# Paleogenomics/pss-bam

Measured on AMD Instinct MI355X. Metric: aligned reads/s (whole node) + HBM GB/s fraction, 200M x 150bp BAM, higher is better.
Workload: dtype u64

## Files before the change

### pss-bam_amd/csrc/engine.hip

```cpp
#include "../../include/pssbam_hip.h"
#include "../../include/fasta-genome-io.h"

#include <hip/hip_runtime.h>

#include <algorithm>
#include <condition_variable>
#include <cstdarg>
#include <cstdio>
#include <cstdlib>
#include <cstring>
#include <ctime>
#include <map>
#include <string>
#include <thread>
#include <unordered_map>
#include <atomic>
#include <memory>
#include <mutex>
#include <vector>

#include "tally_kernels.h"

using namespace pssbam;

static thread_local char g_err[512] = "";
static double feed_now() {
    timespec ts;
    clock_gettime(CLOCK_MONOTONIC, &ts);
    return ts.tv_sec + ts.tv_nsec * 1e-9;
}

static int fail(int code, const char *fmt, ...) {
    va_list ap;
    va_start(ap, fmt);
    vsnprintf(g_err, sizeof g_err, fmt, ap);
    va_end(ap);
    return code;
}

#define HIP_TRY(expr)                                                                          \
    do {                                                                                       \
        hipError_t _e = (expr);                                                                \
        if (_e != hipSuccess)                                                                  \
            return fail(PSSBAM_EHIP, "%s failed: %s (%s:%d)", #expr, hipGetErrorString(_e), __FILE__, __LINE__); \
    } while (0)

extern "C" const char *pssbam_last_error(void) { return g_err; }

static bool device_is_gfx950(int dev) {
    hipDeviceProp_t pr;
    if (hipGetDeviceProperties(&pr, dev) != hipSuccess) return false;
    return strncmp(pr.gcnArchName, "gfx950", 6) == 0;
}

extern "C" int pssbam_device_count(void) {
    int n = 0;
    if (hipGetDeviceCount(&n) != hipSuccess) return 0;
    int ok = 0;
    for (int d = 0; d < n; d++) ok += device_is_gfx950(d) ? 1 : 0;
    return ok;
}

extern "C" int pssbam_warmup(int device) {
    HIP_TRY(hipSetDevice(device));
    HIP_TRY(hipFree(nullptr));
    return PSSBAM_OK;
}

struct Slot {
    uint8_t *d_recs = nullptr;
    size_t recs_cap = 0;
    uint32_t *d_offs = nullptr;
    size_t offs_cap = 0;
    hipEvent_t copy_begin = nullptr, copied = nullptr, consumed = nullptr;
    bool busy = false;
    bool timed = false;
    uint64_t ticket = 0;
};

static constexpr uint64_t FEED_OUT_TARGET = 4400ull << 20, FEED_COMP_CAP = 2ull << 30, FEED_OUT_SLACK = 160ull << 20,
                          FEED_OVERSHOOT = 64ull << 20,
                          FEED_GAP = 16ull << 20;
static constexpr int FEED_SLOTS_READY = 3, FEED_SLOTS_MAX = 40;

struct FeedAcc {
    uint8_t *d_comp = nullptr;
    size_t comp_cap = 0;
    uint64_t comp_used = 0;
    std::vector<pssbam_bgzf_block> blocks;
    std::vector<uint32_t> sub_first;
    uint64_t out_used = 0, sub_bytes = 0;
    void *d_blocks = nullptr;
    pssbam_bgzf_block *h_blocks = nullptr;
    size_t h_blocks_cap = 0;
    uint64_t *d_a = nullptr, *d_e = nullptr, *d_last = nullptr, *d_nexta = nullptr;
    uint32_t *d_n = nullptr, *d_counts = nullptr, *d_base = nullptr;
    size_t blocks_cap = 0;
    uint8_t *d_out = nullptr;
    size_t out_cap = 0;
    uint32_t *d_offs = nullptr;
    size_t offs_cap = 0;
    uint32_t *d_nrecs = nullptr;
    size_t nrecs_cap = 0;
    uint64_t *d_chain = nullptr;
    hipEvent_t consumed = nullptr, copies_done = nullptr, copies_done2 = nullptr, inflated = nullptr, inflate_done = nullptr;
    bool busy = false;
    bool held = false;
    uint64_t flush_seq = 0;
};

struct DeferredTally {
    int slot;
    uint64_t sub_base, sub_len, offs_at;
    uint32_t n_bound, k;
    uint64_t sample_off;
    bool last_of_slot;
};

namespace {
struct PinEntry { size_t len; int refs; };
std::map<const void *, PinEntry> g_pins;
std::mutex g_pins_mu;
bool pin_acquire(const void *p, size_t len) {
    std::lock_guard<std::mutex> lk(g_pins_mu);
    auto it = g_pins.find(p);
    if (it != g_pins.end()) { it->second.refs++; return true; }
    if (hipHostRegister((void *)p, len, hipHostRegisterPortable) != hipSuccess) { (void)hipGetLastError(); return false; }
    g_pins[p] = PinEntry{len, 1};
    return true;
}
void pin_release(const void *p) {
    std::lock_guard<std::mutex> lk(g_pins_mu);
    auto it = g_pins.find(p);
    if (it == g_pins.end()) return;
    if (--it->second.refs == 0) { (void)hipHostUnregister((void *)p); g_pins.erase(it); }
}
}

enum PrepSlot : int {
    PREP_TILED_PSS, PREP_TILED_PSS_LATER, PREP_TILED_PSS_KMER, PREP_TILED_PSS_KMER_LDS, PREP_TILED_KMER, PREP_TILED_KMER_LDS,
    PREP_COMPACT, PREP_COMPACT_KMER, PREP_COMPACT_KMER_LDS,
    PREP_COMPACT_ONCE, PREP_COMPACT_ONCE_KMER, PREP_COMPACT_ONCE_KMER_LDS, PREP_COMPACT_DECODE_TWICE,
    PREP_PLANES_RG, PREP_PLANES_RG_LATER, PREP_PLANES_LEN, PREP_PLANES_LEN_LATER, PREP_PLANES_REF, PREP_PLANES_REF_LATER,
    PREP_KPLANES_RG, PREP_KPLANES_RG_LDS, PREP_KPLANES_LEN, PREP_KPLANES_LEN_LDS, PREP_KPLANES_REF, PREP_KPLANES_REF_LDS,
    PREP_TILED_PSS_BQ, PREP_TILED_PSS_LATER_BQ, PREP_TILED_PSS_KMER_BQ, PREP_TILED_PSS_KMER_LDS_BQ,
    PREP_PLANES_RG_BQ, PREP_PLANES_RG_LATER_BQ, PREP_PLANES_LEN_BQ, PREP_PLANES_LEN_LATER_BQ, PREP_PLANES_REF_BQ, PREP_PLANES_REF_LATER_BQ,
    PREP_TILED_PSS_H, PREP_TILED_PSS_KMER_H, PREP_TILED_PSS_KMER_LDS_H, PREP_TILED_PSS_H_BQ, PREP_TILED_PSS_KMER_H_BQ, PREP_TILED_PSS_KMER_LDS_H_BQ,
    PREP_TILED_SITE, PREP_TILED_SITE_LATER, PREP_TILED_SITE_BQ, PREP_TILED_SITE_LATER_BQ,
    PREP_N
};

struct pssbam_engine {
    pssbam_config cfg{};
    std::string up_ctx, down_ctx, rg;
    bool has_rg = false;
    int device = 0;
    int n_cu = 0;
    hipStream_t stream = nullptr, copy_stream = nullptr, copy_stream2 = nullptr;
    hipStream_t inflate_stream[2] = {nullptr, nullptr};
    hipEvent_t feed_base_ev = nullptr;
    hipStream_t genome_stream = nullptr;
    std::thread late_thread;
    std::atomic<int> late_ready{0};
    std::mutex late_mu;
    hipStream_t late_copy1 = nullptr, late_copy2 = nullptr, late_genome = nullptr;
    bool late_adopted = false;
    hipEvent_t genome_ready = nullptr;
    bool genome_wait_pending = false;
    std::vector<const void *> genome_pins;
    std::vector<void *> retired;
    hipEvent_t copied2 = nullptr;
    bool own_stream = false;

    uint8_t *d_genome = nullptr;
    uint32_t *d_genome4 = nullptr;
    uint32_t acgt_ctx = 0;
    uint64_t genome_bytes = 0;
    std::vector<uint64_t> contig_start;
    std::vector<uint32_t> contig_len;
    std::vector<std::string> contig_ids;
    int32_t star_contig = -1;
    uint4 *d_ref_info = nullptr;
    uint4 *h_ref_info = nullptr;
    size_t h_ref_cap = 0;
    int32_t n_ref = 0;
    bool have_refs = false;
    uint8_t *d_rg = nullptr;
    PlaneSel planes = PLANES_NONE;
    uint32_t n_planes = 0, off_groups = 0, plane_words = 0;
    uint64_t kplane_words = 0;
    uint8_t *d_grp_ids = nullptr;
    uint32_t *d_grp_offs = nullptr, *d_grp_hash = nullptr;
    uint32_t grp_hash_mask = 0;
    std::vector<uint32_t> len_edges;
    std::unordered_map<std::string, uint32_t> ctg_plane;
    std::vector<std::string> ref_names;
    bool tallied = false;
    uint32_t min_bq = 0;
    uint32_t hist_max = 0, off_hist = 0;
    uint32_t site_mode = 0, off_site = 0;
    int env_hist_lds_bins = -1;
    std::unordered_map<std::string, std::vector<uint2>> regions;
    bool has_regions = false;
    uint32_t region_shift = 10;
    std::vector<uint4> ref_info_host;
    uint4 *d_region_info = nullptr;
    uint32_t *d_region_grid = nullptr;
    uint2 *d_region_iv = nullptr;
    unsigned long long *d_counters = nullptr;
    unsigned long long *d_counters_own = nullptr;
    size_t n_counters = 0;
    uint32_t rows = 0, off_rev = 0, off_k5 = 0, off_k3 = 0, off_stats = 0;
    uint64_t n_bins = 0;
    Slot slots[2];
    int next_slot = 0;
    uint64_t ticket_seq = 0;
    double h2d_ms = 0.0;
    uint64_t h2d_bytes = 0;
    std::vector<FeedAcc *> feed;
    int cur_feed = -1, spare_feed = -1;
    uint64_t flush_seq = 0;
    bool feed_opened = false;
    int32_t feed_n_ref = 0;
    uint64_t feed_mem_budget = 0;
    std::vector<DeferredTally> deferred;
    uint8_t *d_carry = nullptr;
    uint8_t *h_handoff = nullptr;
    hipEvent_t handoff_ev = nullptr;
    uint64_t feed_out_target = FEED_OUT_TARGET, feed_comp_cap = FEED_COMP_CAP;
    double feed_t_alloc = 0, feed_t_wait_busy = 0, feed_t_flush = 0;
    double feed_t0 = 0, feed_t_first_flush = -1;
    uint64_t feed_slots_allocated = 0, feed_deferred_launches = 0, feed_early_flushes = 0;
    uint64_t feed_blocks_launched = 0, feed_lanes_launched = 0;
    uint64_t feed_idle_min_blocks = 8192;
    uint64_t feed_block_target = 0;
    std::vector<std::pair<uint64_t, hipEvent_t>> feed_copies;
    std::vector<hipEvent_t> feed_event_pool;
    uint32_t *d_feed_flags = nullptr;
    uint64_t *d_feed_tail = nullptr;
    bool feed_fresh = true;
    uint32_t feed_skip = 0;
    double inflate_ms = 0.0;
    uint64_t inflated_bytes = 0;
    std::vector<std::pair<hipEvent_t, hipEvent_t>> inflate_events;
    hipEvent_t t_begin = nullptr, t_end = nullptr;
    std::vector<std::pair<hipEvent_t, hipEvent_t>> launch_events;
    std::vector<hipEvent_t> event_pool;
    double kernel_ms = 0.0;
    uint64_t kernel_launches = 0;
    int env_tile_reads = 0, env_grid_mult = 0, env_simple_blocks = 0, env_grid_wgs = 0, env_pieces = 0;
    int env_group_slots = 0;
    bool warned_ablate = false;
    bool compact_plan_once = false;
    uint32_t prep_lds[2 * PREP_N] = {0};
    int prep_occ[2 * PREP_N] = {0};
    bool use_compact = true;
    uint32_t *d_scratch = nullptr;
    size_t scratch_slots = 0;
    uint32_t dev_pieces = 0;
    uint64_t dev_pieces_avg = 0;
};

static void ctx_mask(const char *set, uint32_t (&m)[8]) {
    memset(m, 0, sizeof m);
    for (const unsigned char *p = (const unsigned char *)set;; p++) {
        const uint32_t st = enc_byte(*p);
        m[st >> 5] |= 1u << (st & 31);
        if (!*p) break;
    }
}

static int env_int(const char *name) {
    const char *v = getenv(name);
    return v ? atoi(v) : 0;
}

static void late_streams(pssbam_engine *e, bool wait) {
    std::lock_guard<std::mutex> lk(e->late_mu);
    if (e->late_adopted) return;
    if (!wait && !e->late_ready.load(std::memory_order_acquire)) return;
    if (e->late_thread.joinable()) e->late_thread.join();
    e->copy_stream = e->late_copy1;
    e->copy_stream2 = e->late_copy2;
    e->genome_stream = e->late_genome;
    e->late_adopted = true;
}

extern "C" int pssbam_engine_create(const pssbam_config *cfg, pssbam_engine **out) {
    if (!cfg || !out) return fail(PSSBAM_EINVAL, "null argument");
    *out = nullptr;
    if (cfg->abi_version != PSSBAM_ABI_VERSION)
        return fail(PSSBAM_EINVAL, "abi_version %u != %u", cfg->abi_version, PSSBAM_ABI_VERSION);
    if (!(cfg->tally_mask & (PSSBAM_TALLY_PSS | PSSBAM_TALLY_KMER)) ||
        (cfg->tally_mask & ~(PSSBAM_TALLY_PSS | PSSBAM_TALLY_KMER)))
        return fail(PSSBAM_EINVAL, "tally_mask must be a non-empty subset of PSS|KMER");
    if ((cfg->tally_mask & PSSBAM_TALLY_PSS)) {
        if (cfg->pss.region_len < 0 || cfg->pss.region_len > 1000000)
            return fail(PSSBAM_EINVAL, "region_len %d out of range", cfg->pss.region_len);
        if (!cfg->pss.up_ctx || !cfg->pss.down_ctx) return fail(PSSBAM_EINVAL, "up_ctx/down_ctx must be set");
    }
    if ((cfg->tally_mask & PSSBAM_TALLY_KMER) && (cfg->kmer.klen < 1 || cfg->kmer.klen > PSSBAM_MAX_KLEN))
        return fail(PSSBAM_EINVAL, "klen %d outside the device range 1..%d", cfg->kmer.klen, PSSBAM_MAX_KLEN);

    int n_dev = 0;
    if (hipGetDeviceCount(&n_dev) != hipSuccess || n_dev == 0)
        return fail(PSSBAM_ENODEV, "no HIP device available (this engine has no CPU path)");
    int dev = cfg->device;
    if (dev < 0) HIP_TRY(hipGetDevice(&dev));
    if (dev >= n_dev) return fail(PSSBAM_ENODEV, "device %d does not exist (%d present)", dev, n_dev);
    if (!device_is_gfx950(dev) && !getenv("PSSBAM_ALLOW_OTHER_ARCH"))
        return fail(PSSBAM_ENODEV, "device %d is not gfx950", dev);
    HIP_TRY(hipSetDevice(dev));

    pssbam_engine *e = new pssbam_engine();
    std::unique_ptr<pssbam_engine, void (*)(pssbam_engine *)> guard(e, pssbam_engine_destroy);
    e->cfg = *cfg;
    e->device = dev;
    if (cfg->tally_mask & PSSBAM_TALLY_PSS) {
        e->up_ctx = cfg->pss.up_ctx;
        e->down_ctx = cfg->pss.down_ctx;
    }
    if (cfg->read_group) {
        e->rg = cfg->read_group;
        e->has_rg = true;
    }
    e->cfg.pss.up_ctx = e->cfg.pss.down_ctx = e->cfg.read_group = nullptr;
    const bool tstat = getenv("PSSBAM_STATS") != nullptr;
    const double tc0 = tstat ? feed_now() : 0.0;
    hipDeviceProp_t pr;
    HIP_TRY(hipGetDeviceProperties(&pr, dev));
    e->n_cu = pr.multiProcessorCount;
    const double tc1 = tstat ? feed_now() : 0.0;
    HIP_TRY(hipStreamCreateWithFlags(&e->stream, hipStreamNonBlocking));
    if (getenv("PSSBAM_STREAMS_UP_FRONT")) {
        HIP_TRY(hipStreamCreateWithFlags(&e->copy_stream, hipStreamNonBlocking));
        HIP_TRY(hipStreamCreateWithFlags(&e->copy_stream2, hipStreamNonBlocking));
        HIP_TRY(hipStreamCreateWithFlags(&e->genome_stream, hipStreamNonBlocking));
        e->late_adopted = true;
    } else {
        e->late_thread = std::thread([e, dev]() {
            if (hipSetDevice(dev) == hipSuccess) {
                if (hipStreamCreateWithFlags(&e->late_copy1, hipStreamNonBlocking) != hipSuccess) e->late_copy1 = nullptr;
                if (hipStreamCreateWithFlags(&e->late_copy2, hipStreamNonBlocking) != hipSuccess) e->late_copy2 = nullptr;
                if (hipStreamCreateWithFlags(&e->late_genome, hipStreamNonBlocking) != hipSuccess) e->late_genome = nullptr;
            }
            (void)hipGetLastError();
            e->late_ready.store(1, std::memory_order_release);
        });
    }
    HIP_TRY(hipEventCreateWithFlags(&e->genome_ready, hipEventDisableTiming));
    HIP_TRY(hipEventCreateWithFlags(&e->copied2, hipEventDisableTiming));
    e->own_stream = true;
    HIP_TRY(hipEventCreate(&e->t_begin));
    HIP_TRY(hipEventCreate(&e->t_end));
    const double tc2 = tstat ? feed_now() : 0.0;

    e->rows = (cfg->tally_mask & PSSBAM_TALLY_PSS) ? (uint32_t)cfg->pss.region_len + 2u : 0u;
    e->n_bins = (cfg->tally_mask & PSSBAM_TALLY_KMER) ? (1ull << (2 * cfg->kmer.klen)) : 0ull;
    e->off_rev = e->rows * 16u;
    e->off_k5 = 2u * e->rows * 16u;
    e->off_k3 = (uint32_t)(e->off_k5 + e->n_bins);
    e->off_stats = (uint32_t)(e->off_k3 + e->n_bins);
    e->n_counters = (size_t)e->off_stats + PSSBAM_ST_N;
    e->plane_words = 2u * e->rows * 16u;
    e->off_groups = (uint32_t)e->n_counters;
    e->kplane_words = cfg->tally_mask == PSSBAM_TALLY_KMER ? 2ull * e->n_bins : 0ull;
    HIP_TRY(hipMalloc(&e->d_counters_own, e->n_counters * sizeof(unsigned long long)));
    e->d_counters = e->d_counters_own;
    HIP_TRY(hipMemsetAsync(e->d_counters, 0, e->n_counters * sizeof(unsigned long long), e->stream));
    if (e->has_rg) {
        HIP_TRY(hipMalloc(&e->d_rg, e->rg.size() + 16));
        HIP_TRY(hipMemcpy(e->d_rg, e->rg.data(), e->rg.size(), hipMemcpyHostToDevice));
    }
    for (Slot &s : e->slots) {
        HIP_TRY(hipEventCreate(&s.copy_begin));
        HIP_TRY(hipEventCreate(&s.copied));
        HIP_TRY(hipEventCreateWithFlags(&s.consumed, hipEventDisableTiming));
    }
    e->scratch_slots = (size_t)e->n_cu * 8;
    HIP_TRY(hipMalloc(&e->d_scratch, e->scratch_slots * SCRATCH_WORDS * sizeof(uint32_t)));
    e->env_tile_reads = env_int("PSSBAM_TILE_READS");
    e->env_grid_mult = env_int("PSSBAM_GRID_MULT");
    e->env_simple_blocks = env_int("PSSBAM_SIMPLE_BLOCKS");
    e->env_grid_wgs = env_int("PSSBAM_GRID_WGS");
    e->env_pieces = env_int("PSSBAM_PIECES");
    e->env_group_slots = env_int("PSSBAM_GROUP_SLOTS");
    if (getenv("PSSBAM_HIST_LDS_BINS")) e->env_hist_lds_bins = std::max(env_int("PSSBAM_HIST_LDS_BINS"), 0);
    if (const int g = env_int("PSSBAM_REGION_GRID_SHIFT")) e->region_shift = (uint32_t)std::min(std::max(g, 2), 20);
    if (getenv("PSSBAM_COMPACT")) e->use_compact = env_int("PSSBAM_COMPACT") != 0;
    if (getenv("PSSBAM_COMPACT_PLAN_ONCE")) e->compact_plan_once = env_int("PSSBAM_COMPACT_PLAN_ONCE") != 0;
    if (tstat)
        fprintf(stderr, "[pssbam] engine on device %d: device properties %.3f, its stream + events %.3f, counters + scratch (first allocations, first "
                        "enqueue) %.3f s\n", dev, tc1 - tc0, tc2 - tc1, feed_now() - tc2);
    *out = guard.release();
    return PSSBAM_OK;
}

extern "C" void pssbam_engine_destroy(pssbam_engine *e) {
    if (!e) return;
    (void)hipSetDevice(e->device);
    late_streams(e, true);
    for (hipStream_t is : e->inflate_stream)
        if (is) (void)hipStreamSynchronize(is);
    if (e->stream) (void)hipStreamSynchronize(e->stream);
    if (e->copy_stream) (void)hipStreamSynchronize(e->copy_stream);
    if (e->copy_stream2) (void)hipStreamSynchronize(e->copy_stream2);
    for (Slot &s : e->slots) {
        if (s.d_recs) (void)hipFree(s.d_recs);
        if (s.d_offs) (void)hipFree(s.d_offs);
        if (s.copied) (void)hipEventDestroy(s.copied);
        if (s.copy_begin) (void)hipEventDestroy(s.copy_begin);
        if (s.consumed) (void)hipEventDestroy(s.consumed);
    }
    if (e->genome_stream) (void)hipStreamSynchronize(e->genome_stream);
    for (const void *p : e->genome_pins) pin_release(p);
    e->genome_pins.clear();
    for (FeedAcc *sp : e->feed) {
        FeedAcc &s = *sp;
        void *ptrs[] = {s.d_comp, s.d_blocks, s.d_a, s.d_e, s.d_last, s.d_nexta, s.d_n, s.d_counts, s.d_base, s.d_out, s.d_offs, s.d_nrecs, s.d_chain};
        for (void *q : ptrs)
            if (q) (void)hipFree(q);
        if (s.h_blocks) (void)hipHostFree(s.h_blocks);
        if (s.consumed) (void)hipEventDestroy(s.consumed);
        if (s.copies_done) (void)hipEventDestroy(s.copies_done);
        if (s.copies_done2) (void)hipEventDestroy(s.copies_done2);
        if (s.inflated) (void)hipEventDestroy(s.inflated);
        if (s.inflate_done) (void)hipEventDestroy(s.inflate_done);
        delete sp;
    }
    e->feed.clear();
    if (e->d_carry) (void)hipFree(e->d_carry);
    if (e->h_handoff) (void)hipHostFree(e->h_handoff);
    if (e->handoff_ev) (void)hipEventDestroy(e->handoff_ev);
    for (void *q : e->retired) (void)hipFree(q);
    if (e->d_feed_tail) (void)hipFree(e->d_feed_tail);
    for (auto &p : e->feed_copies) (void)hipEventDestroy(p.second);
    for (hipEvent_t ev : e->feed_event_pool) (void)hipEventDestroy(ev);
    if (e->d_feed_flags) (void)hipFree(e->d_feed_flags);
    for (auto &p : e->inflate_events) { (void)hipEventDestroy(p.first); (void)hipEventDestroy(p.second); }
    for (auto &p : e->launch_events) { (void)hipEventDestroy(p.first); (void)hipEventDestroy(p.second); }
    for (hipEvent_t ev : e->event_pool) (void)hipEventDestroy(ev);
    if (e->t_begin) (void)hipEventDestroy(e->t_begin);
    if (e->t_end) (void)hipEventDestroy(e->t_end);
    if (e->d_scratch) (void)hipFree(e->d_scratch);
    if (e->d_genome) (void)hipFree(e->d_genome);
    if (e->d_genome4) (void)hipFree(e->d_genome4);
    if (e->d_ref_info) (void)hipFree(e->d_ref_info);
    if (e->h_ref_info) (void)hipHostFree(e->h_ref_info);
    if (e->d_rg) (void)hipFree(e->d_rg);
    for (void *q : {(void *)e->d_region_info, (void *)e->d_region_grid, (void *)e->d_region_iv})
        if (q) (void)hipFree(q);
    if (e->d_grp_ids) (void)hipFree(e->d_grp_ids);
    if (e->d_grp_offs) (void)hipFree(e->d_grp_offs);
    if (e->d_grp_hash) (void)hipFree(e->d_grp_hash);
    if (e->d_counters_own) (void)hipFree(e->d_counters_own);
    if (e->own_stream && e->stream) (void)hipStreamDestroy(e->stream);
    if (e->copy_stream) (void)hipStreamDestroy(e->copy_stream);
    if (e->copy_stream2) (void)hipStreamDestroy(e->copy_stream2);
    for (hipStream_t is : e->inflate_stream)
        if (is) (void)hipStreamDestroy(is);
    if (e->feed_base_ev) (void)hipEventDestroy(e->feed_base_ev);
    if (e->genome_stream) (void)hipStreamDestroy(e->genome_stream);
    if (e->genome_ready) (void)hipEventDestroy(e->genome_ready);
    if (e->copied2) (void)hipEventDestroy(e->copied2);
    delete e;
}

extern "C" int pssbam_engine_set_stream(pssbam_engine *e, void *hip_stream) {
    if (!e) return fail(PSSBAM_EINVAL, "null engine");
    HIP_TRY(hipSetDevice(e->device));
    HIP_TRY(hipStreamSynchronize(e->stream));
    if (e->own_stream) HIP_TRY(hipStreamDestroy(e->stream));
    e->stream = (hipStream_t)hip_stream;
    e->own_stream = false;
    return PSSBAM_OK;
}

static constexpr uint64_t CONTIG_ALIGN = 256, CONTIG_PAD = 256;

static hipEvent_t take_event(pssbam_engine *e);
static int feed_resume(pssbam_engine *e);

static int genome_settle(pssbam_engine *e) {
    if (e->genome_pins.empty()) return PSSBAM_OK;
    HIP_TRY(hipSetDevice(e->device));
    HIP_TRY(hipEventSynchronize(e->genome_ready));
    for (const void *p : e->genome_pins) pin_release(p);
    e->genome_pins.clear();
    return PSSBAM_OK;
}

static int genome_upload(pssbam_engine *e, size_t n, const char *const *ids, const uint8_t *const *seqs, const uint64_t *lens,
                         int seqs_on_device) {
    if (!e || (n && (!ids || !seqs || !lens))) return fail(PSSBAM_EINVAL, "null argument");
    HIP_TRY(hipSetDevice(e->device));
    int rc = genome_settle(e);
    if (rc) return rc;
    std::vector<size_t> order(n);
    for (size_t i = 0; i < n; i++) order[i] = i;
    std::stable_sort(order.begin(), order.end(), [&](size_t a, size_t b) { return strcmp(ids[a], ids[b]) < 0; });
    std::vector<uint64_t> start(n + 1, 0);
    std::vector<uint32_t> len(n + 1, 0);
    uint64_t total = CONTIG_PAD;
    for (size_t k = 0; k < n; k++) {
        if (lens[order[k]] > 0xFFFFFF00ull)
            return fail(PSSBAM_EINVAL, "contig %s has %llu bases; the engine addresses contigs below 4 Gi bases", ids[order[k]],
                        (unsigned long long)lens[order[k]]);
        start[k] = total;
        len[k] = (uint32_t)lens[order[k]];
        total += ((uint64_t)len[k] + CONTIG_PAD + CONTIG_ALIGN - 1) / CONTIG_ALIGN * CONTIG_ALIGN;
    }
    if (e->d_genome) {
        HIP_TRY(hipStreamSynchronize(e->stream));
        HIP_TRY(hipFree(e->d_genome));
        e->d_genome = nullptr;
        if (e->d_genome4) { HIP_TRY(hipFree(e->d_genome4)); e->d_genome4 = nullptr; }
    }
    HIP_TRY(hipMalloc(&e->d_genome, total));
    late_streams(e, true);
    if (!e->genome_stream) HIP_TRY(hipStreamCreateWithFlags(&e->genome_stream, hipStreamNonBlocking));
    hipStream_t gs = e->genome_stream;
    if (seqs_on_device) {
        hipEvent_t ev = take_event(e);
        if (!ev) return fail(PSSBAM_EHIP, "hipEventCreate failed");
        HIP_TRY(hipEventRecord(ev, e->stream));
        HIP_TRY(hipStreamWaitEvent(gs, ev, 0));
        e->event_pool.push_back(ev);
    }
    HIP_TRY(hipMemsetAsync(e->d_genome, 0, total, gs));
    const bool try_lock = !seqs_on_device && !getenv("PSSBAM_NO_PIN");
    for (size_t k = 0; k < n; k++) {
        if (!len[k]) continue;
        const void *src = seqs[order[k]];
        if (try_lock && len[k] >= (32u << 20) && pin_acquire(src, len[k])) e->genome_pins.push_back(src);
        HIP_TRY(hipMemcpyAsync(e->d_genome + start[k], src, len[k],
                               seqs_on_device ? hipMemcpyDeviceToDevice : hipMemcpyHostToDevice, gs));
    }
    hipLaunchKernelGGL(encode_genome_kernel, dim3(4096), dim3(256), 0, gs, e->d_genome, total / 16);
    HIP_TRY(hipGetLastError());
    {
        CtxSets sets;
        ctx_mask(e->up_ctx.c_str(), sets.up);
        ctx_mask(e->down_ctx.c_str(), sets.down);
        e->acgt_ctx = 0;
        for (uint32_t v = 0; v < 4; v++)
            e->acgt_ctx |= (((sets.up[0] >> v) & 1u) << (2 * v)) | (((sets.down[0] >> v) & 1u) << (2 * v + 1));
        const uint64_t n_out = total / 8, slack = 16;
        HIP_TRY(hipMalloc(&e->d_genome4, (n_out + slack) * sizeof(uint32_t)));
        HIP_TRY(hipMemsetAsync(e->d_genome4 + n_out, 0x44, slack * sizeof(uint32_t), gs));
        hipLaunchKernelGGL(pack_genome4_kernel, dim3(4096), dim3(256), 0, gs, e->d_genome, e->d_genome4, n_out, sets);
        HIP_TRY(hipGetLastError());
    }
    HIP_TRY(hipEventRecord(e->genome_ready, gs));
    e->genome_wait_pending = true;
    e->contig_start.assign(start.begin(), start.begin() + n);
    e->contig_len.assign(len.begin(), len.begin() + n);
    e->genome_bytes = total;
    e->contig_ids.clear();
    for (size_t k = 0; k < n; k++) e->contig_ids.emplace_back(ids[order[k]]);
    e->star_contig = -1;
    if (e->have_refs) e->have_refs = false;
    {
        auto it = std::lower_bound(e->contig_ids.begin(), e->contig_ids.end(), std::string("*"),
                                   [](const std::string &a, const std::string &b) { return strcmp(a.c_str(), b.c_str()) < 0; });
        if (it != e->contig_ids.end() && *it == "*") e->star_contig = (int32_t)(it - e->contig_ids.begin());
    }
    return PSSBAM_OK;
}

extern "C" int pssbam_engine_set_genome_arrays(pssbam_engine *e, size_t n, const char *const *ids,
                                               const uint8_t *const *seqs, const uint64_t *lens,
                                               int seqs_on_device) {
    int rc = genome_upload(e, n, ids, seqs, lens, seqs_on_device);
    if (rc) return rc;
    if (e->genome_stream) HIP_TRY(hipStreamSynchronize(e->genome_stream));
    return genome_settle(e);
}

static int genome_from_struct(pssbam_engine *e, const struct genome *g, bool wait) {
    if (!e || !g) return fail(PSSBAM_EINVAL, "null argument");
    std::vector<const char *> ids(g->n_seqs);
    std::vector<const uint8_t *> seqs(g->n_seqs);
    std::vector<uint64_t> lens(g->n_seqs);
    for (size_t i = 0; i < g->n_seqs; i++) {
        ids[i] = g->seqs[i]->id;
        seqs[i] = (const uint8_t *)g->seqs[i]->seq;
        lens[i] = g->seqs[i]->len;
    }
    return wait ? pssbam_engine_set_genome_arrays(e, g->n_seqs, ids.data(), seqs.data(), lens.data(), 0)
                : genome_upload(e, g->n_seqs, ids.data(), seqs.data(), lens.data(), 0);
}

extern "C" int pssbam_engine_set_genome(pssbam_engine *e, const struct genome *g) { return genome_from_struct(e, g, true); }

extern "C" int pssbam_engine_set_genome_async(pssbam_engine *e, const struct genome *g) { return genome_from_struct(e, g, false); }

extern "C" int pssbam_engine_genome_wait(pssbam_engine *e) {
    if (!e) return fail(PSSBAM_EINVAL, "null engine");
    HIP_TRY(hipSetDevice(e->device));
    if (e->genome_stream) HIP_TRY(hipStreamSynchronize(e->genome_stream));
    return genome_settle(e);
}

static int pack_regions(pssbam_engine *e, bool in_use) {
    if (!e->has_regions) return PSSBAM_OK;
    const size_t n_ent = (size_t)e->n_ref + 1;
    const uint32_t g = e->region_shift;
    std::vector<uint4> desc(n_ent, make_uint4(0, 0, 0, 0));
    uint64_t n_iv = 0, n_grid = 0;
    std::vector<const std::vector<uint2> *> src(n_ent, nullptr);
    for (size_t i = 0; i < n_ent; i++) {
        const uint4 ri = e->ref_info_host[i];
        if (!ri.w) continue;
        const auto it = e->regions.find(i < (size_t)e->n_ref ? e->ref_names[i] : std::string("*"));
        if (it == e->regions.end()) continue;
        uint64_t cnt = 0;
        for (const uint2 &v : it->second) cnt += v.x < ri.z ? 1u : 0u;
        if (!cnt) continue;
        src[i] = &it->second;
        desc[i] = make_uint4(0, (uint32_t)cnt, 0, 0);
        n_iv += cnt;
        n_grid += ((uint64_t)ri.z >> g) + 2;
    }
    if (n_iv >= (1ull << 32) || n_grid >= (1ull << 32)) return fail(PSSBAM_ENOMEM, "the region table has too many intervals or grid words for 32-bit indices");
    const uint64_t bytes = n_ent * sizeof(uint4) + (n_iv + 1) * sizeof(uint2) + (n_grid + 2) * sizeof(uint32_t);
    HIP_TRY(hipSetDevice(e->device));
    if (in_use && e->d_region_info) HIP_TRY(hipStreamSynchronize(e->stream));
    for (void **q : {(void **)&e->d_region_info, (void **)&e->d_region_grid, (void **)&e->d_region_iv})
        if (*q) { HIP_TRY(hipFree(*q)); *q = nullptr; }
    size_t free_b = 0, total_b = 0;
    HIP_TRY(hipMemGetInfo(&free_b, &total_b));
    if (bytes > (uint64_t)free_b)
        return fail(PSSBAM_ENOMEM, "the region table (%llu intervals, grid shift %u) needs %llu bytes; the device has %llu free",
                    (unsigned long long)n_iv, g, (unsigned long long)bytes, (unsigned long long)free_b);
    std::vector<uint2> iv((size_t)n_iv + 1, make_uint2(0, 0));
    std::vector<uint32_t> grid((size_t)n_grid + 2, 0u);
    uint64_t at_iv = 0, at_grid = 0;
    for (size_t i = 0; i < n_ent; i++) {
        if (!src[i]) continue;
        const uint32_t len = e->ref_info_host[i].z, cnt = desc[i].y;
        desc[i].x = (uint32_t)at_iv;
        desc[i].z = (uint32_t)at_grid;
        uint2 *out = iv.data() + at_iv;
        for (uint32_t k = 0; k < cnt; k++) out[k] = make_uint2((*src[i])[k].x, std::min((*src[i])[k].y, len));
        const uint64_t n_bins = ((uint64_t)len >> g) + 1;
        uint32_t j = 0;
        for (uint64_t b = 0; b < n_bins; b++) {
            while (j < cnt && (uint64_t)out[j].y <= (b << g)) j++;
            grid[at_grid + b] = j;
        }
        grid[at_grid + n_bins] = cnt;
        at_iv += cnt;
        at_grid += n_bins + 1;
    }
    HIP_TRY(hipMalloc(&e->d_region_info, n_ent * sizeof(uint4)));
    HIP_TRY(hipMalloc(&e->d_region_iv, iv.size() * sizeof(uint2)));
    HIP_TRY(hipMalloc(&e->d_region_grid, grid.size() * sizeof(uint32_t)));
    HIP_TRY(hipMemcpy(e->d_region_info, desc.data(), n_ent * sizeof(uint4), hipMemcpyHostToDevice));
    HIP_TRY(hipMemcpy(e->d_region_iv, iv.data(), iv.size() * sizeof(uint2), hipMemcpyHostToDevice));
    HIP_TRY(hipMemcpy(e->d_region_grid, grid.data(), grid.size() * sizeof(uint32_t), hipMemcpyHostToDevice));
    return PSSBAM_OK;
}

extern "C" int pssbam_engine_set_regions(pssbam_engine *e, int32_t n_names, const char *const *names, int64_t n_regions,
                                         const int32_t *name_of, const uint32_t *starts, const uint32_t *ends) {
    if (!e) return fail(PSSBAM_EINVAL, "null engine");
    if (n_names < 0 || n_regions < 0 || n_regions > PSSBAM_MAX_REGIONS) return fail(PSSBAM_EINVAL, "region count outside 0..%d", PSSBAM_MAX_REGIONS);
    if ((n_names && !names) || (n_regions && (!name_of || !starts || !ends))) return fail(PSSBAM_EINVAL, "null region list");
    if (e->tallied) return fail(PSSBAM_ESTATE, "records have been tallied already: set the regions after create or reset, before the first tally");
    std::unordered_map<std::string, std::vector<uint2>> map;
    for (int32_t k = 0; k < n_names; k++) {
        if (!names[k]) return fail(PSSBAM_EINVAL, "region contig name %d is NULL", k);
        if (n_regions) map[names[k]];
    }
    for (int64_t i = 0; i < n_regions; i++) {
        if (name_of[i] < 0 || name_of[i] >= n_names) return fail(PSSBAM_EINVAL, "region %lld: contig index %d outside 0..%d", (long long)i, name_of[i], n_names - 1);
        if (starts[i] > ends[i])
            return fail(PSSBAM_EINVAL, "region %lld on %s: start %u lies behind end %u", (long long)i, names[name_of[i]], starts[i], ends[i]);
        if (starts[i] < ends[i]) map[names[name_of[i]]].push_back(make_uint2(starts[i], ends[i]));
    }
    for (auto &kv : map) {
        std::vector<uint2> &v = kv.second;
        std::sort(v.begin(), v.end(), [](const uint2 &a, const uint2 &b) { return a.x != b.x ? a.x < b.x : a.y < b.y; });
        size_t n = 0;
        for (const uint2 &r : v) {
            if (n && r.x <= v[n - 1].y) v[n - 1].y = std::max(v[n - 1].y, r.y);
            else v[n++] = r;
        }
        v.resize(n);
    }
    HIP_TRY(hipSetDevice(e->device));
    e->regions.swap(map);
    e->has_regions = n_regions > 0;
// ... 123 lines not shown
static int launch_tiled(pssbam_engine *e, PrepSlot slot, TallyParams &P, uint32_t lds, uint32_t n_tiles) {
    if (P.region_info)
        return launch_flat(e, (PrepSlot)(slot + PREP_N), tally_tiled<DO_PSS, DO_KMER, LDS_KMER, LATER, MASKQ, true, HIST>, P, lds, n_tiles, LDS_KMER);
    return launch_flat(e, slot, tally_tiled<DO_PSS, DO_KMER, LDS_KMER, LATER, MASKQ, false, HIST>, P, lds, n_tiles, LDS_KMER);
}

template <bool LATER, bool MASKQ>
static int launch_tiled_site(pssbam_engine *e, TallyParams &P, uint32_t lds, uint32_t n_tiles) {
    constexpr PrepSlot slot = MASKQ ? (LATER ? PREP_TILED_SITE_LATER_BQ : PREP_TILED_SITE_BQ) : (LATER ? PREP_TILED_SITE_LATER : PREP_TILED_SITE);
    if (P.region_info)
        return launch_flat<true>(e, (PrepSlot)(slot + PREP_N), tally_tiled<true, false, false, LATER, MASKQ, true, false, true>, P, lds, n_tiles, false);
    return launch_flat<true>(e, slot, tally_tiled<true, false, false, LATER, MASKQ, false, false, true>, P, lds, n_tiles, false);
}

template <bool MASKQ>
static int launch_tiled_hist(pssbam_engine *e, TallyParams &P, bool do_kmer, bool kmer_lds, uint32_t lds, uint32_t n_tiles) {
    constexpr int bq = MASKQ ? PREP_TILED_PSS_H_BQ - PREP_TILED_PSS_H : 0;
    if (!do_kmer) return launch_tiled<true, false, false, false, MASKQ, true>(e, (PrepSlot)(PREP_TILED_PSS_H + bq), P, lds, n_tiles);
    return kmer_lds ? launch_tiled<true, true, true, false, MASKQ, true>(e, (PrepSlot)(PREP_TILED_PSS_KMER_LDS_H + bq), P, lds, n_tiles)
                    : launch_tiled<true, true, false, false, MASKQ, true>(e, (PrepSlot)(PREP_TILED_PSS_KMER_H + bq), P, lds, n_tiles);
}

template <PlaneSel SEL, bool LATER, bool MASKQ, bool REGIONS>
static int launch_planes(pssbam_engine *e, TallyParams &P, const PlaneParams &G, uint32_t lds, uint32_t n_tiles) {
    constexpr PrepSlot plain = SEL == PLANES_RG  ? (LATER ? PREP_PLANES_RG_LATER : PREP_PLANES_RG)
                             : SEL == PLANES_LEN ? (LATER ? PREP_PLANES_LEN_LATER : PREP_PLANES_LEN)
                                                 : (LATER ? PREP_PLANES_REF_LATER : PREP_PLANES_REF);
    constexpr PrepSlot unfiltered = MASKQ ? (PrepSlot)(PREP_PLANES_RG_BQ + (plain - PREP_PLANES_RG)) : plain;
    constexpr PrepSlot slot = (PrepSlot)(unfiltered + (REGIONS ? PREP_N : 0));
    uint32_t grid = 0;
    const int rc = tiled_grid(e, slot, tally_tiled_planes<SEL, LATER, MASKQ, REGIONS>, lds, n_tiles, G.scratch_words, &grid);
    if (rc != PSSBAM_OK) return rc;
    P.scratch = e->d_scratch;
    hipLaunchKernelGGL((tally_tiled_planes<SEL, LATER, MASKQ, REGIONS>), dim3(grid), dim3(TILED_THREADS), lds, e->stream, P, G);
    hipLaunchKernelGGL(reduce_partials_grouped, dim3((G.scratch_words * REDUCE_GROUPS + 255) / 256), dim3(256), 0, e->stream, P, G, grid);
    return PSSBAM_OK;
}

template <PlaneSel SEL, bool LDS_KMER, bool REGIONS>
static int launch_kmer_planes(pssbam_engine *e, TallyParams &P, const PlaneParams &G, uint32_t lds, uint32_t n_tiles) {
    constexpr PrepSlot unfiltered = SEL == PLANES_RG  ? (LDS_KMER ? PREP_KPLANES_RG_LDS : PREP_KPLANES_RG)
                                  : SEL == PLANES_LEN ? (LDS_KMER ? PREP_KPLANES_LEN_LDS : PREP_KPLANES_LEN)
                                                      : (LDS_KMER ? PREP_KPLANES_REF_LDS : PREP_KPLANES_REF);
    constexpr PrepSlot slot = (PrepSlot)(unfiltered + (REGIONS ? PREP_N : 0));
    uint32_t grid = 0;
    const int rc = tiled_grid(e, slot, tally_tiled_kmer_planes<SEL, LDS_KMER, REGIONS>, lds, n_tiles, G.scratch_words, &grid);
    if (rc != PSSBAM_OK) return rc;
    P.scratch = e->d_scratch;
    hipLaunchKernelGGL((tally_tiled_kmer_planes<SEL, LDS_KMER, REGIONS>), dim3(grid), dim3(TILED_THREADS), lds, e->stream, P, G);
    hipLaunchKernelGGL(reduce_partials_kmer_planes, dim3((G.scratch_words * REDUCE_GROUPS + 255) / 256), dim3(256), 0, e->stream, P, G, grid,
                       (uint32_t)(LDS_KMER ? 1 : 0));
    return PSSBAM_OK;
}

static uint64_t sample_prefix_need(const uint8_t *bytes, uint64_t nbytes, bool whole_record, int max_records = 4096) {
    uint64_t o = 0, need_max = 64;
    for (int n = 0; n < max_records && o + 36 <= nbytes; n++) {
        uint32_t bs, l_seq;
        memcpy(&bs, bytes + o, 4);
        if (bs < 32 || o + 4 + (uint64_t)bs > nbytes) break;
        const uint32_t l_name = bytes[o + 12];
        uint16_t n_cig;
        memcpy(&n_cig, bytes + o + 16, 2);
        memcpy(&l_seq, bytes + o + 20, 4);
        const uint64_t qual_off = 36ull + l_name + 4ull * n_cig + ((uint64_t)l_seq + 1) / 2;
        const uint64_t need = whole_record ? 4ull + bs : std::min<uint64_t>(qual_off + 1, 4ull + bs);
        need_max = std::max(need_max, need);
        o += 4 + (uint64_t)bs;
    }
    return need_max;
}

static bool whole_records(const pssbam_engine *e) { return e->has_rg || e->planes == PLANES_RG || e->min_bq > 0; }

static PlaneParams plane_params(const pssbam_engine *e) {
    PlaneParams G{};
    G.ids = e->d_grp_ids;
    G.id_offs = e->d_grp_offs;
    G.hash = e->d_grp_hash;
    G.hash_mask = e->grp_hash_mask;
    G.n_groups = e->n_planes;
    G.n_slots = e->n_planes + 1u;
    G.plane_words = e->plane_words;
    G.off_groups = e->off_groups;
    G.koff_planes = e->off_groups;
    G.kplane_words = e->kplane_words;
    G.n_edges = (uint32_t)e->len_edges.size();
    std::copy(e->len_edges.begin(), e->len_edges.end(), G.edges);
    return G;
}

static uint32_t pieces_for(uint64_t need_max) {
    uint64_t pieces = (need_max + 15 + 15) / 16;
    pieces |= 1;
    return (uint32_t)std::min<uint64_t>(std::max<uint64_t>(pieces, 5), 41);
}

static int launch_tally(pssbam_engine *e, const uint8_t *d_recs, uint64_t nbytes, const uint32_t *d_offs,
                        uint32_t n_records, const uint8_t *host_sample, uint64_t host_sample_bytes,
                        const uint32_t *d_n_recs = nullptr, uint64_t sample_off = 0, const uint32_t *host_offsets = nullptr) {
    if (!n_records) return PSSBAM_OK;
    e->tallied = true;
    const pssbam_config &c = e->cfg;
    TallyParams P{};
    P.recs = d_recs;
    P.offs = d_offs;
    P.n_recs = n_records;
    P.n_recs_dev = d_n_recs;
    P.recs_bytes = nbytes;
    P.tally_mask = c.tally_mask;
    P.genome = e->d_genome;
    P.genome4 = e->d_genome4;
    P.acgt_ctx = e->acgt_ctx;
    P.ref_info = e->d_ref_info;
    P.n_ref = e->n_ref;
    const bool do_pss = (c.tally_mask & PSSBAM_TALLY_PSS) != 0, do_kmer = (c.tally_mask & PSSBAM_TALLY_KMER) != 0;
    if (do_pss) {
        P.N = c.pss.region_len;
        P.pss_min_mq = (uint32_t)c.pss.min_mq;
        P.pss_len_never = c.pss.min_read_len > 0xFFFFFFFFull ? 1u : 0u;
        P.pss_min_len = (uint32_t)std::min<uint64_t>(c.pss.min_read_len, 0xFFFFFFFFull);
        P.pss_max_len = (uint32_t)std::min<uint64_t>(c.pss.max_read_len, 0xFFFFFFFFull);
        P.pss_merged_only = c.pss.merged_only ? 1u : 0u;
        ctx_mask(e->up_ctx.c_str(), P.up_mask);
        ctx_mask(e->down_ctx.c_str(), P.down_mask);
    }
    if (do_kmer) {
        P.K = c.kmer.klen;
        P.fk_min_mq = (uint32_t)c.kmer.min_mq;
        P.fk_len_never = c.kmer.min_read_len > 0xFFFFFFFFull ? 1u : 0u;
        P.fk_min_len = (uint32_t)std::min<uint64_t>(c.kmer.min_read_len, 0xFFFFFFFFull);
        P.fk_max_len = (uint32_t)std::min<uint64_t>(c.kmer.max_read_len, 0xFFFFFFFFull);
        P.fk_merged_only = c.kmer.merged_only ? 1u : 0u;
    }
    P.rg = e->has_rg ? e->d_rg : nullptr;
    P.rg_len = (uint32_t)e->rg.size();
    P.counters = e->d_counters;
    P.off_rev = e->off_rev;
    P.off_k5 = e->off_k5;
    P.off_k3 = e->off_k3;
    P.off_stats = e->off_stats;
    P.min_bq = do_pss ? e->min_bq : 0u;
    const bool maskq = P.min_bq > 0;
    const bool regions = e->has_regions;
    const bool hist = do_pss && e->hist_max > 0;
    if (hist) {
        P.hist_max = e->hist_max;
        P.off_hist = e->off_hist;
    }
    const bool site = do_pss && e->site_mode != PSSBAM_SITE_NONE;
    if (site) P.off_site = e->off_site;
    if (regions) {
        P.region_info = e->d_region_info;
        P.region_grid = e->d_region_grid;
        P.region_iv = e->d_region_iv;
        P.region_shift = e->region_shift;
    }
    PlaneParams G = plane_params(e);

    int kernel = c.kernel;
    if (d_n_recs && kernel == PSSBAM_KERNEL_SIMPLE) return fail(PSSBAM_EINVAL, "device-indexed blocks need the tiled kernels");
    const uint32_t n_passes = do_pss ? (e->rows + TILED_ROWS - 1) / TILED_ROWS : 1u;
    if (kernel == PSSBAM_KERNEL_AUTO) kernel = PSSBAM_KERNEL_TILED;

    if (e->genome_wait_pending) {
        HIP_TRY(hipStreamWaitEvent(e->stream, e->genome_ready, 0));
        e->genome_wait_pending = false;
    }
    hipEvent_t ev0 = take_event(e), ev1 = take_event(e);
    if (!ev0 || !ev1) return fail(PSSBAM_EHIP, "hipEventCreate failed");
    HIP_TRY(hipEventRecord(ev0, e->stream));

    if (kernel == PSSBAM_KERNEL_SIMPLE) {
        const uint32_t tab_bytes = do_pss ? 2u * e->rows * 16u * 4u : 0u;
        const bool lds_tab = do_pss && tab_bytes <= 60u * 1024u;
        uint32_t blocks = (uint32_t)std::min<uint64_t>(((uint64_t)n_records + 255) / 256, (uint64_t)e->n_cu * 8);
        if (e->env_simple_blocks > 0) blocks = (uint32_t)e->env_simple_blocks;
        if (e->planes != PLANES_NONE && !do_pss) {
            if (e->planes == PLANES_RG) hipLaunchKernelGGL(tally_simple_kmer_planes<PLANES_RG>, dim3(blocks), dim3(256), 0, e->stream, P, G);
            else if (e->planes == PLANES_LEN) hipLaunchKernelGGL(tally_simple_kmer_planes<PLANES_LEN>, dim3(blocks), dim3(256), 0, e->stream, P, G);
            else hipLaunchKernelGGL(tally_simple_kmer_planes<PLANES_REF>, dim3(blocks), dim3(256), 0, e->stream, P, G);
        } else if (e->planes == PLANES_RG) hipLaunchKernelGGL(tally_simple_planes<PLANES_RG>, dim3(blocks), dim3(256), 0, e->stream, P, G);
        else if (e->planes == PLANES_LEN) hipLaunchKernelGGL(tally_simple_planes<PLANES_LEN>, dim3(blocks), dim3(256), 0, e->stream, P, G);
        else if (e->planes == PLANES_REF) hipLaunchKernelGGL(tally_simple_planes<PLANES_REF>, dim3(blocks), dim3(256), 0, e->stream, P, G);
        else if (lds_tab) hipLaunchKernelGGL(tally_simple<true>, dim3(blocks), dim3(256), tab_bytes, e->stream, P);
        else hipLaunchKernelGGL(tally_simple<false>, dim3(blocks), dim3(256), 0, e->stream, P);
    } else {
        const uint64_t avg = std::max<uint64_t>(40, nbytes / n_records);
        uint32_t pieces;
        if (host_sample) {
            uint64_t need = sample_prefix_need(host_sample, host_sample_bytes, whole_records(e), 1400);
            if (host_offsets && n_records > 4200u) {
                const uint32_t mid = host_offsets[n_records / 2], late = host_offsets[n_records - 1400u];
                need = std::max(need, sample_prefix_need(host_sample + mid, host_sample_bytes - mid, whole_records(e), 1400));
                need = std::max(need, sample_prefix_need(host_sample + late, host_sample_bytes - late, whole_records(e), 1400));
            }
            pieces = pieces_for(need);
        } else {
            if (!e->dev_pieces || (!d_n_recs && (avg * 8 < e->dev_pieces_avg * 7 || avg * 7 > e->dev_pieces_avg * 8))) {
                sample_off = std::min<uint64_t>(sample_off, nbytes);
                std::vector<uint8_t> head((size_t)std::min<uint64_t>(nbytes - sample_off, 1024 * 1024));
                HIP_TRY(hipMemcpyAsync(head.data(), d_recs + sample_off, head.size(), hipMemcpyDeviceToHost, e->stream));
                HIP_TRY(hipStreamSynchronize(e->stream));
                uint64_t need = sample_prefix_need(head.data(), head.size(), whole_records(e));
                if (!d_n_recs && n_records > 8192u) {
                    uint32_t at[2] = {0, 0};
                    HIP_TRY(hipMemcpyAsync(&at[0], d_offs + n_records / 2, 4, hipMemcpyDeviceToHost, e->stream));
                    HIP_TRY(hipMemcpyAsync(&at[1], d_offs + (n_records - 2048u), 4, hipMemcpyDeviceToHost, e->stream));
                    HIP_TRY(hipStreamSynchronize(e->stream));
                    for (int k = 0; k < 2; k++) {
                        if ((uint64_t)at[k] >= nbytes) continue;
                        head.resize((size_t)std::min<uint64_t>(nbytes - at[k], 512 * 1024));
                        HIP_TRY(hipMemcpyAsync(head.data(), d_recs + at[k], head.size(), hipMemcpyDeviceToHost, e->stream));
                        HIP_TRY(hipStreamSynchronize(e->stream));
                        need = std::max(need, sample_prefix_need(head.data(), head.size(), whole_records(e), 2048));
                    }
                }
                e->dev_pieces = pieces_for(need);
                e->dev_pieces_avg = avg;
            }
            pieces = e->dev_pieces;
        }
        if (e->env_pieces > 0) pieces = (uint32_t)std::min(std::max(e->env_pieces, 4), 64);
        uint32_t T = TILED_MAX_T;
        if (e->env_tile_reads > 0) T = std::min<uint32_t>(TILED_MAX_T, (uint32_t)(e->env_tile_reads + 15) / 16 * 16);
        P.reads_per_tile = T;
        P.prefix_pieces = pieces;
        P.xcd_map = (uint32_t)env_int("PSSBAM_XCD_MAP");
        P.ablate = (uint32_t)env_int("PSSBAM_ABLATE");
        if (P.ablate && !e->warned_ablate) {
            fprintf(stderr, "[pssbam] PSSBAM_ABLATE=%u: kernel phases are switched off, the tables are WRONG (profiling only)\n", P.ablate);
            e->warned_ablate = true;
        }
        const bool kmer_lds = do_kmer && c.kmer.klen <= KMER_LDS_MAX_K;
        const uint32_t n_tiles = (n_records + T - 1) / T;
        const uint32_t lds = tiled_lds_bytes(T, pieces);
        int rc = PSSBAM_OK;
        P.row_base = 0;
        if (e->planes != PLANES_NONE && !do_pss) {
            using LaunchK = int (*)(pssbam_engine *, TallyParams &, const PlaneParams &, uint32_t, uint32_t);
            static constexpr LaunchK launch_kr[2][3][2] = {
                {{launch_kmer_planes<PLANES_RG, false, false>, launch_kmer_planes<PLANES_RG, true, false>},
                 {launch_kmer_planes<PLANES_LEN, false, false>, launch_kmer_planes<PLANES_LEN, true, false>},
                 {launch_kmer_planes<PLANES_REF, false, false>, launch_kmer_planes<PLANES_REF, true, false>}},
                {{launch_kmer_planes<PLANES_RG, false, true>, launch_kmer_planes<PLANES_RG, true, true>},
                 {launch_kmer_planes<PLANES_LEN, false, true>, launch_kmer_planes<PLANES_LEN, true, true>},
                 {launch_kmer_planes<PLANES_REF, false, true>, launch_kmer_planes<PLANES_REF, true, true>}}};
            const auto &launch_k = launch_kr[regions];
            const uint32_t n_planes = G.n_groups + 1u;
            if (kmer_lds) {
                const uint32_t hist = 2u * (1u << (2 * c.kmer.klen)) * 4u;
                const uint32_t fit = lds + 2u * hist <= KMER_PLANES_LDS_BUDGET ? (KMER_PLANES_LDS_BUDGET - lds) / hist - 1u : 1u;
                uint32_t per_pass = std::min(n_planes, fit);
                if (e->env_group_slots > 0) per_pass = std::min(per_pass, (uint32_t)e->env_group_slots);
                for (uint32_t plane0 = 0; plane0 < n_planes && rc == PSSBAM_OK; plane0 += per_pass) {
                    G.plane0 = plane0;
                    G.n_slots = std::min(per_pass, n_planes - plane0);
                    G.scratch_words = GROUP_SCRATCH_DELTA + G.n_slots * (hist / 4u);
                    rc = launch_k[e->planes - PLANES_RG][1](e, P, G, tiled_kmer_planes_lds_bytes(T, pieces, G.n_slots, c.kmer.klen, true), n_tiles);
                }
            } else {
                G.plane0 = 0;
                G.n_slots = n_planes;
                G.scratch_words = GROUP_SCRATCH_DELTA;
                rc = launch_k[e->planes - PLANES_RG][0](e, P, G, lds, n_tiles);
            }
        } else if (e->planes != PLANES_NONE) {
            using LaunchPlanes = int (*)(pssbam_engine *, TallyParams &, const PlaneParams &, uint32_t, uint32_t);
            static constexpr LaunchPlanes launch_pass_r[2][2][3][2] = {
                {{{launch_planes<PLANES_RG, false, false, false>, launch_planes<PLANES_RG, true, false, false>},
                  {launch_planes<PLANES_LEN, false, false, false>, launch_planes<PLANES_LEN, true, false, false>},
                  {launch_planes<PLANES_REF, false, false, false>, launch_planes<PLANES_REF, true, false, false>}},
                 {{launch_planes<PLANES_RG, false, true, false>, launch_planes<PLANES_RG, true, true, false>},
                  {launch_planes<PLANES_LEN, false, true, false>, launch_planes<PLANES_LEN, true, true, false>},
                  {launch_planes<PLANES_REF, false, true, false>, launch_planes<PLANES_REF, true, true, false>}}},
                {{{launch_planes<PLANES_RG, false, false, true>, launch_planes<PLANES_RG, true, false, true>},
                  {launch_planes<PLANES_LEN, false, false, true>, launch_planes<PLANES_LEN, true, false, true>},
                  {launch_planes<PLANES_REF, false, false, true>, launch_planes<PLANES_REF, true, false, true>}},
                 {{launch_planes<PLANES_RG, false, true, true>, launch_planes<PLANES_RG, true, true, true>},
                  {launch_planes<PLANES_LEN, false, true, true>, launch_planes<PLANES_LEN, true, true, true>},
                  {launch_planes<PLANES_REF, false, true, true>, launch_planes<PLANES_REF, true, true, true>}}}};
            const auto &launch_pass = launch_pass_r[regions];
            const uint32_t n_planes = G.n_groups + 1u;
            const uint32_t fit = lds + 2u * GROUP_PLANE_WORDS * 4u <= GROUPED_LDS_BUDGET
                                     ? (GROUPED_LDS_BUDGET - lds) / (GROUP_PLANE_WORDS * 4u) - 1u : 1u;
            uint32_t per_pass = std::min(n_planes, fit);
            if (e->env_group_slots > 0) per_pass = std::min(per_pass, (uint32_t)e->env_group_slots);
            for (uint32_t pass = 0; pass < n_passes && rc == PSSBAM_OK; pass++) {
                P.row_base = pass * TILED_ROWS;
                for (uint32_t plane0 = 0; plane0 < n_planes && rc == PSSBAM_OK; plane0 += per_pass) {
                    G.plane0 = plane0;
                    G.n_slots = std::min(per_pass, n_planes - plane0);
                    G.scratch_words = GROUP_SCRATCH_DELTA + G.n_slots * GROUP_PLANE_WORDS;
                    rc = launch_pass[maskq][e->planes - PLANES_RG][pass > 0](e, P, G, tiled_grouped_lds_bytes(T, pieces, G.n_slots), n_tiles);
                }
            }
        } else if (site) {
            rc = maskq ? launch_tiled_site<false, true>(e, P, lds, n_tiles) : launch_tiled_site<false, false>(e, P, lds, n_tiles);
            for (uint32_t pass = 1; pass < n_passes && rc == PSSBAM_OK; pass++) {
                P.row_base = pass * TILED_ROWS;
                rc = maskq ? launch_tiled_site<true, true>(e, P, lds, n_tiles) : launch_tiled_site<true, false>(e, P, lds, n_tiles);
            }
        } else if (do_pss && e->rows <= COMPACT_MAX_ROWS && e->use_compact && !e->has_rg && !maskq && !regions && !hist) {
            if (!do_kmer && getenv("PSSBAM_COMPACT_DECODE_TWICE"))
                rc = launch_flat(e, PREP_COMPACT_DECODE_TWICE, tally_compact_decode_twice, P, lds, n_tiles, false);
            else if (e->compact_plan_once)
                rc = !do_kmer  ? launch_flat(e, PREP_COMPACT_ONCE, tally_compact<false, false, true>, P, lds, n_tiles, false)
                     : kmer_lds ? launch_flat(e, PREP_COMPACT_ONCE_KMER_LDS, tally_compact<true, true, true>, P, lds, n_tiles, true)
                                : launch_flat(e, PREP_COMPACT_ONCE_KMER, tally_compact<true, false, true>, P, lds, n_tiles, false);
            else
                rc = !do_kmer  ? launch_flat(e, PREP_COMPACT, tally_compact<false, false, false>, P, lds, n_tiles, false)
                     : kmer_lds ? launch_flat(e, PREP_COMPACT_KMER_LDS, tally_compact<true, true, false>, P, lds, n_tiles, true)
                                : launch_flat(e, PREP_COMPACT_KMER, tally_compact<true, false, false>, P, lds, n_tiles, false);
        } else if (hist) {
            P.hist_lds_bins = std::min(e->hist_max + 2u, HIST_LDS_MAX_BINS);
            if (e->env_hist_lds_bins >= 0) P.hist_lds_bins = std::min(P.hist_lds_bins, (uint32_t)e->env_hist_lds_bins);
            const uint32_t lds_h = lds + hist_lds_bytes(P.hist_lds_bins);
            rc = maskq ? launch_tiled_hist<true>(e, P, do_kmer, kmer_lds, lds_h, n_tiles) : launch_tiled_hist<false>(e, P, do_kmer, kmer_lds, lds_h, n_tiles);
            for (uint32_t pass = 1; pass < n_passes && rc == PSSBAM_OK; pass++) {
                P.row_base = pass * TILED_ROWS;
                rc = maskq ? launch_tiled<true, false, false, true, true>(e, PREP_TILED_PSS_LATER_BQ, P, lds, n_tiles)
                           : launch_tiled<true, false, false, true, false>(e, PREP_TILED_PSS_LATER, P, lds, n_tiles);
            }
        } else if (maskq) {
            if (do_kmer)
                rc = kmer_lds ? launch_tiled<true, true, true, false, true>(e, PREP_TILED_PSS_KMER_LDS_BQ, P, lds, n_tiles)
                              : launch_tiled<true, true, false, false, true>(e, PREP_TILED_PSS_KMER_BQ, P, lds, n_tiles);
            else
                rc = launch_tiled<true, false, false, false, true>(e, PREP_TILED_PSS_BQ, P, lds, n_tiles);
            for (uint32_t pass = 1; pass < n_passes && rc == PSSBAM_OK; pass++) {
                P.row_base = pass * TILED_ROWS;
                rc = launch_tiled<true, false, false, true, true>(e, PREP_TILED_PSS_LATER_BQ, P, lds, n_tiles);
            }
        } else {
            if (do_pss && do_kmer)
                rc = kmer_lds ? launch_tiled<true, true, true, false, false>(e, PREP_TILED_PSS_KMER_LDS, P, lds, n_tiles)
                              : launch_tiled<true, true, false, false, false>(e, PREP_TILED_PSS_KMER, P, lds, n_tiles);
            else if (do_pss)
                rc = launch_tiled<true, false, false, false, false>(e, PREP_TILED_PSS, P, lds, n_tiles);
            else
                rc = kmer_lds ? launch_tiled<false, true, true, false, false>(e, PREP_TILED_KMER_LDS, P, lds, n_tiles)
                              : launch_tiled<false, true, false, false, false>(e, PREP_TILED_KMER, P, lds, n_tiles);
            for (uint32_t pass = 1; pass < n_passes && rc == PSSBAM_OK; pass++) {
                P.row_base = pass * TILED_ROWS;
                rc = launch_tiled<true, false, false, true, false>(e, PREP_TILED_PSS_LATER, P, lds, n_tiles);
            }
        }
        if (rc != PSSBAM_OK) return rc;
    }
    HIP_TRY(hipGetLastError());
    HIP_TRY(hipEventRecord(ev1, e->stream));
    e->launch_events.emplace_back(ev0, ev1);
    if (e->launch_events.size() > 4096) return resolve_launch_events(e);
    return PSSBAM_OK;
}

extern "C" int pssbam_engine_hint_records(pssbam_engine *e, const void *records, uint64_t nbytes) {
    if (!e || (!records && nbytes)) return fail(PSSBAM_EINVAL, "null argument");
    if (nbytes < 36) return PSSBAM_OK;
    e->dev_pieces = pieces_for(sample_prefix_need((const uint8_t *)records, nbytes, whole_records(e), 1 << 16));
    e->dev_pieces_avg = 40;
    return PSSBAM_OK;
}

static int check_ready(pssbam_engine *e) {
    if (!e) return fail(PSSBAM_EINVAL, "null engine");
    if (!e->d_genome) return fail(PSSBAM_ESTATE, "set_genome has not been called");
    if (!e->have_refs) return fail(PSSBAM_ESTATE, "set_references has not been called");
    return PSSBAM_OK;
}

extern "C" int pssbam_engine_submit_device(pssbam_engine *e, const void *d_records, uint64_t nbytes,
                                           const uint32_t *d_offsets, uint32_t n_records) {
    int rc = check_ready(e);
    if (rc) return rc;
    if (n_records && (!d_records || !d_offsets)) return fail(PSSBAM_EINVAL, "null buffer");
    if (nbytes >= (1ull << 32)) return fail(PSSBAM_EINVAL, "record block must be < 4 GiB (got %llu)", (unsigned long long)nbytes);
    if (((uintptr_t)d_records & 15u) || ((uintptr_t)d_offsets & 3u))
        return fail(PSSBAM_EINVAL, "d_records must be 16-byte aligned, d_offsets 4-byte aligned");
    HIP_TRY(hipSetDevice(e->device));
    return launch_tally(e, (const uint8_t *)d_records, nbytes, d_offsets, n_records, nullptr, 0);
}

static void book_copy_time(pssbam_engine *e, Slot &s) {
    if (!s.timed) return;
    float ms = 0.f;
    if (hipEventElapsedTime(&ms, s.copy_begin, s.copied) == hipSuccess) e->h2d_ms += ms;
    s.timed = false;
}

extern "C" int pssbam_engine_submit_async(pssbam_engine *e, const void *records, uint64_t nbytes, const uint32_t *offsets,
                                          uint32_t n_records, uint64_t *ticket) {
    int rc = check_ready(e);
    if (rc) return rc;
    if (ticket) *ticket = 0;
    if (!n_records) return PSSBAM_OK;
    if (!records || !offsets) return fail(PSSBAM_EINVAL, "null buffer");
    if (nbytes >= (1ull << 32)) return fail(PSSBAM_EINVAL, "record block must be < 4 GiB (got %llu)", (unsigned long long)nbytes);
    if (offsets[n_records] != nbytes) return fail(PSSBAM_EFORMAT, "offsets[n_records] must equal nbytes");
    HIP_TRY(hipSetDevice(e->device));
    Slot &s = e->slots[e->next_slot];
    e->next_slot ^= 1;
    if (s.busy) HIP_TRY(hipEventSynchronize(s.consumed));
    s.busy = false;
    book_copy_time(e, s);
    if (s.recs_cap < nbytes + 64) {
        if (s.d_recs) HIP_TRY(hipFree(s.d_recs));
        s.d_recs = nullptr;
        s.recs_cap = (size_t)(nbytes + nbytes / 4 + 4096);
        HIP_TRY(hipMalloc(&s.d_recs, s.recs_cap));
    }
    if (s.offs_cap < (size_t)n_records + 1) {
        if (s.d_offs) HIP_TRY(hipFree(s.d_offs));
        s.d_offs = nullptr;
        s.offs_cap = (size_t)n_records + n_records / 4 + 1024;
        HIP_TRY(hipMalloc(&s.d_offs, s.offs_cap * sizeof(uint32_t)));
    }
    late_streams(e, true);
    if (!e->copy_stream) HIP_TRY(hipStreamCreateWithFlags(&e->copy_stream, hipStreamNonBlocking));
    const uint64_t half = (nbytes >= (64ull << 20) && e->copy_stream2 && !getenv("PSSBAM_ONE_COPY_STREAM")) ? (nbytes / 2) & ~4095ull : 0;
    HIP_TRY(hipEventRecord(s.copy_begin, e->copy_stream));
    if (half) {
        HIP_TRY(hipStreamWaitEvent(e->copy_stream2, s.copy_begin, 0));
        HIP_TRY(hipMemcpyAsync(s.d_recs + half, (const uint8_t *)records + half, nbytes - half, hipMemcpyHostToDevice, e->copy_stream2));
        HIP_TRY(hipEventRecord(e->copied2, e->copy_stream2));
    }
    HIP_TRY(hipMemcpyAsync(s.d_recs, records, half ? half : nbytes, hipMemcpyHostToDevice, e->copy_stream));
    HIP_TRY(hipMemcpyAsync(s.d_offs, offsets, ((size_t)n_records + 1) * sizeof(uint32_t), hipMemcpyHostToDevice,
                           e->copy_stream));
    if (half) HIP_TRY(hipStreamWaitEvent(e->copy_stream, e->copied2, 0));
    HIP_TRY(hipEventRecord(s.copied, e->copy_stream));
    s.timed = true;
    e->h2d_bytes += nbytes + ((uint64_t)n_records + 1) * sizeof(uint32_t);
    HIP_TRY(hipStreamWaitEvent(e->stream, s.copied, 0));
    rc = launch_tally(e, s.d_recs, nbytes, s.d_offs, n_records, (const uint8_t *)records, nbytes, nullptr, 0, offsets);
    if (rc) return rc;
    HIP_TRY(hipEventRecord(s.consumed, e->stream));
    s.busy = true;
    s.ticket = ++e->ticket_seq;
    if (ticket) *ticket = s.ticket;
    return PSSBAM_OK;
}

extern "C" int pssbam_engine_copy_done(pssbam_engine *e, uint64_t ticket) {
    if (!e) return fail(PSSBAM_EINVAL, "null engine");
    if (!ticket) return 1;
    for (Slot &s : e->slots)
        if (s.ticket == ticket) {
            HIP_TRY(hipSetDevice(e->device));
            const hipError_t q = hipEventQuery(s.copied);
            if (q == hipSuccess) return 1;
            if (q == hipErrorNotReady) return 0;
            return fail(PSSBAM_EHIP, "hipEventQuery failed: %s", hipGetErrorString(q));
        }
    return 1;
}

extern "C" int pssbam_engine_wait_copied(pssbam_engine *e, uint64_t ticket) {
    if (!e) return fail(PSSBAM_EINVAL, "null engine");
    if (!ticket) return PSSBAM_OK;
    for (Slot &s : e->slots)
        if (s.ticket == ticket) {
            HIP_TRY(hipSetDevice(e->device));
            HIP_TRY(hipEventSynchronize(s.copied));
            return PSSBAM_OK;
        }
    return PSSBAM_OK;
}

extern "C" int pssbam_engine_submit(pssbam_engine *e, const void *records, uint64_t nbytes, const uint32_t *offsets,
                                    uint32_t n_records) {
    uint64_t ticket = 0;
    int rc = pssbam_engine_submit_async(e, records, nbytes, offsets, n_records, &ticket);
    if (rc) return rc;
    return pssbam_engine_wait_copied(e, ticket);
}

extern "C" int pssbam_engine_phase_times(pssbam_engine *e, double *h2d_ms, uint64_t *h2d_bytes, double *kernel_ms,
                                         uint64_t *n_launches) {
    if (!e) return fail(PSSBAM_EINVAL, "null engine");
    int rc = pssbam_engine_sync(e);
    if (rc) return rc;
    for (Slot &s : e->slots) book_copy_time(e, s);
    rc = resolve_launch_events(e);
    if (rc) return rc;
    if (h2d_ms) *h2d_ms = e->h2d_ms;
    if (h2d_bytes) *h2d_bytes = e->h2d_bytes;
    if (kernel_ms) *kernel_ms = e->kernel_ms;
    if (n_launches) *n_launches = e->kernel_launches;
    return PSSBAM_OK;
}

static int feed_flush(pssbam_engine *e);

extern "C" int pssbam_engine_sync(pssbam_engine *e) {
    if (!e) return fail(PSSBAM_EINVAL, "null engine");
    HIP_TRY(hipSetDevice(e->device));
    {
        const int rc = feed_flush(e);
        if (rc) return rc;
    }
    if (e->copy_stream2) HIP_TRY(hipStreamSynchronize(e->copy_stream2));
    if (e->copy_stream) HIP_TRY(hipStreamSynchronize(e->copy_stream));
    if (e->genome_stream) HIP_TRY(hipStreamSynchronize(e->genome_stream));
    for (hipStream_t q : e->inflate_stream)
        if (q) HIP_TRY(hipStreamSynchronize(q));
    HIP_TRY(hipStreamSynchronize(e->stream));
    const int rc = genome_settle(e);
    if (rc) return rc;
    if (!e->deferred.empty())
        return fail(PSSBAM_ESTATE, "compressed blocks were fed (pssbam_engine_feed_open) but set_genome / set_references never followed");
    return PSSBAM_OK;
}

extern "C" int pssbam_engine_finish(pssbam_engine *e, unsigned long *fwd, unsigned long *rev, uint64_t *k5,
                                    uint64_t *k3, uint64_t stats[PSSBAM_ST_N]) {
    int rc = pssbam_engine_sync(e);
    if (rc) return rc;
    std::vector<unsigned long long> h(e->n_counters);
    HIP_TRY(hipMemcpy(h.data(), e->d_counters, e->n_counters * sizeof(unsigned long long), hipMemcpyDeviceToHost));
    static_assert(sizeof(unsigned long) == 8, "LP64 expected");
    const size_t tab = (size_t)e->rows * 16;
    for (size_t g = 0; g < e->n_planes; g++)
        for (size_t i = 0; i < 2 * tab; i++) h[i] += h[e->off_groups + g * e->plane_words + i];
    for (size_t g = 0; g < e->n_planes && e->kplane_words; g++)
        for (uint64_t i = 0; i < e->kplane_words; i++) h[e->off_k5 + i] += h[(uint64_t)e->off_groups + g * e->kplane_words + i];
    if (fwd) for (size_t i = 0; i < tab; i++) fwd[i] = (unsigned long)h[i];
    if (rev) for (size_t i = 0; i < tab; i++) rev[i] = (unsigned long)h[e->off_rev + i];
    if (k5) for (uint64_t i = 0; i < e->n_bins; i++) k5[i] = h[e->off_k5 + i];
    if (k3) for (uint64_t i = 0; i < e->n_bins; i++) k3[i] = h[e->off_k3 + i];
    if (stats) for (int i = 0; i < PSSBAM_ST_N; i++) stats[i] = h[e->off_stats + i];
    return PSSBAM_OK;
}

extern "C" int pssbam_engine_finish_groups(pssbam_engine *e, int32_t group, unsigned long *fwd, unsigned long *rev) {
    if (!e) return fail(PSSBAM_EINVAL, "null engine");
    if (e->cfg.tally_mask == PSSBAM_TALLY_KMER) return fail(PSSBAM_EINVAL, "a k-mer engine's planes are read with pssbam_engine_finish_kmer_groups");
    const int32_t n_planes = (int32_t)e->n_planes;
    if (!n_planes) return fail(PSSBAM_ESTATE, "none of pssbam_engine_set_read_groups / _set_length_bins / _set_contig_sets has been called");
    if (group < -1 || group >= n_planes) return fail(PSSBAM_EINVAL, "group %d outside -1..%d", group, n_planes - 1);
    int rc = pssbam_engine_sync(e);
    if (rc) return rc;
    const size_t tab = (size_t)e->rows * 16;
    const size_t at = group < 0 ? 0 : e->off_groups + (size_t)group * e->plane_words;
    std::vector<unsigned long long> h(2 * tab);
    HIP_TRY(hipMemcpy(h.data(), e->d_counters + at, 2 * tab * sizeof(unsigned long long), hipMemcpyDeviceToHost));
    if (fwd) for (size_t i = 0; i < tab; i++) fwd[i] = (unsigned long)h[i];
    if (rev) for (size_t i = 0; i < tab; i++) rev[i] = (unsigned long)h[tab + i];
    return PSSBAM_OK;
}

extern "C" int pssbam_engine_finish_kmer_groups(pssbam_engine *e, int32_t group, uint64_t *k5, uint64_t *k3) {
    if (!e) return fail(PSSBAM_EINVAL, "null engine");
    if (e->cfg.tally_mask != PSSBAM_TALLY_KMER) return fail(PSSBAM_EINVAL, "only a k-mer engine (PSSBAM_TALLY_KMER alone) has k-mer planes");
    const int32_t n_planes = (int32_t)e->n_planes;
    if (!n_planes) return fail(PSSBAM_ESTATE, "none of pssbam_engine_set_read_groups / _set_length_bins / _set_contig_sets has been called");
    if (group < -1 || group >= n_planes) return fail(PSSBAM_EINVAL, "group %d outside -1..%d", group, n_planes - 1);
    int rc = pssbam_engine_sync(e);
    if (rc) return rc;
    const uint64_t at = group < 0 ? (uint64_t)e->off_k5 : (uint64_t)e->off_groups + (uint64_t)group * e->kplane_words;
    if (k5) HIP_TRY(hipMemcpy(k5, e->d_counters + at, e->n_bins * sizeof(uint64_t), hipMemcpyDeviceToHost));
    if (k3) HIP_TRY(hipMemcpy(k3, e->d_counters + at + e->n_bins, e->n_bins * sizeof(uint64_t), hipMemcpyDeviceToHost));
    return PSSBAM_OK;
}

static int set_planes(pssbam_engine *e, PlaneSel sel, uint32_t n_planes, const char *what) {
    if (e->hist_max) return fail(PSSBAM_EINVAL, "%s and the length histogram exclude each other", what);
    if (e->site_mode) return fail(PSSBAM_EINVAL, "%s and site context exclude each other", what);
    const bool kmer = e->cfg.tally_mask == PSSBAM_TALLY_KMER;
    if (e->cfg.tally_mask != PSSBAM_TALLY_PSS && !kmer)
        return fail(PSSBAM_EINVAL, "%s split the substitution tables or the k-mer tables, not both (PSSBAM_TALLY_PSS | PSSBAM_TALLY_KMER)", what);
    if (e->tallied) return fail(PSSBAM_ESTATE, "records have been tallied already: set %s after create or reset, before the first tally", what);
    if (e->d_counters != e->d_counters_own) return fail(PSSBAM_ESTATE, "a caller-bound counter block cannot grow: set %s before bind_counters", what);
    HIP_TRY(hipSetDevice(e->device));
    const uint64_t n_counters = (uint64_t)e->off_groups + (uint64_t)n_planes * (kmer ? e->kplane_words : (uint64_t)e->plane_words);
    if (kmer) {
        size_t free_b = 0, total_b = 0;
        HIP_TRY(hipMemGetInfo(&free_b, &total_b));
        if (n_counters * sizeof(unsigned long long) > (uint64_t)free_b)
            return fail(PSSBAM_ENOMEM, "k = %d with %u planes (plane 0 and %u %s) needs a counter block of %llu bytes; the device has %llu free",
                        e->cfg.kmer.klen, n_planes + 1u, n_planes, what, (unsigned long long)(n_counters * sizeof(unsigned long long)),
                        (unsigned long long)free_b);
    }
    unsigned long long *d_counters = nullptr;
    HIP_TRY(hipMalloc(&d_counters, n_counters * sizeof(unsigned long long)));
    HIP_TRY(hipMemsetAsync(d_counters, 0, n_counters * sizeof(unsigned long long), e->stream));
    if (e->d_counters_own) e->retired.push_back(e->d_counters_own);
    e->d_counters = e->d_counters_own = d_counters;
    e->n_counters = n_counters;
    e->planes = sel;
    e->n_planes = n_planes;
    return PSSBAM_OK;
}

extern "C" int pssbam_engine_set_read_groups(pssbam_engine *e, int32_t n, const char *const *ids) {
    if (!e) return fail(PSSBAM_EINVAL, "null engine");
    if (n < 1 || n > PSSBAM_MAX_READ_GROUPS || !ids) return fail(PSSBAM_EINVAL, "read group count %d outside 1..%d", n, PSSBAM_MAX_READ_GROUPS);
    if (e->has_rg) return fail(PSSBAM_EINVAL, "read groups and a -R read group filter exclude each other");
    if (e->planes == PLANES_LEN) return fail(PSSBAM_EINVAL, "read groups and length bins exclude each other");
    if (e->planes == PLANES_REF) return fail(PSSBAM_EINVAL, "read groups and contig sets exclude each other");
    for (int32_t i = 0; i < n; i++)
        if (!ids[i]) return fail(PSSBAM_EINVAL, "read group %d is NULL", i);
    std::vector<std::string> groups(ids, ids + n);
    std::string cat;
    std::vector<uint32_t> offs(1, 0u);
    for (const std::string &g : groups) {
        cat += g;
        offs.push_back((uint32_t)cat.size());
    }
    uint32_t hsize = 16;
    while (hsize < 2u * (uint32_t)n) hsize <<= 1;
    std::vector<uint32_t> hash(hsize, 0u);
    for (int32_t g = 0; g < n; g++) {
        uint32_t hv = FNV1A_SEED;
        for (unsigned char ch : groups[g]) hv = fnv1a_step(hv, ch);
        for (uint32_t k = 0;; k++) {
// ... 402 lines not shown
```

### pss-bam_amd/csrc/tally_kernels.h

```cpp
#pragma once

#include "record_decode.h"

namespace pssbam {

constexpr int TILED_THREADS = 256;
constexpr int TILED_WAVES = TILED_THREADS / 64;
constexpr int TILED_ROWS = 32;
constexpr int KMER_LDS_MAX_K = 4;
constexpr uint32_t STAGE_SLACK = 64;
constexpr uint32_t CODE_NONE = 32;
constexpr uint32_t TABLE_WORDS = 64 * 32;
constexpr uint32_t SCRATCH_KMER = 1024, SCRATCH_DELTA = 1536, SCRATCH_WORDS = 1552;
constexpr uint32_t SITE_WORDS = 16 * 32, SITE_SCRATCH_WORDS = SCRATCH_WORDS + SITE_WORDS;
constexpr uint32_t CODE_SITE = 64;
constexpr uint32_t REF_LDS_ENTRIES = 64;

struct LdsTableRowMajor {
    uint32_t *t;
    uint32_t rows;
    __device__ __forceinline__ void add(uint32_t table, uint32_t row, uint32_t cell) const {
        atomicAdd(&t[(table * rows + row) * 16u + cell], 1u);
    }
};
struct LdsTableColumnMajor {
    uint32_t *t;
    uint32_t row_base;
    __device__ __forceinline__ void add(uint32_t table, uint32_t row, uint32_t cell) const {
        const uint32_t r = row - row_base;
        if (r < 32u) atomicAdd(&t[(((cell << 1) | table) << 5) + r], 1u);
    }
};
struct GlobalTable {
    unsigned long long *c;
    uint32_t off_rev;
    __device__ __forceinline__ void add(uint32_t table, uint32_t row, uint32_t cell) const {
        atomicAdd(&c[(table ? off_rev : 0u) + row * 16u + cell], 1ull);
    }
};

struct NoSite {
    __device__ __forceinline__ void add(uint32_t, uint32_t, uint32_t) const {}
};
__device__ __forceinline__ uint32_t site_half_code(uint32_t table, uint32_t cell) {
    return ((cell >> 2) << 2) | (cell & 2u) | table;
}
struct LdsSiteColumnMajor {
    uint32_t *t;
    uint32_t row_base;
    __device__ __forceinline__ void add(uint32_t table, uint32_t row, uint32_t cell) const {
        const uint32_t r = row - row_base;
        if (r < 32u) atomicAdd(&t[(site_half_code(table, cell) << 5) + r], 1u);
    }
};
struct GlobalSite {
    unsigned long long *c;
    uint32_t off_rev;
    __device__ __forceinline__ void add(uint32_t table, uint32_t row, uint32_t cell) const {
        atomicAdd(&c[(table ? off_rev : 0u) + row * 16u + cell], 1ull);
    }
};
__device__ __forceinline__ bool site_in_cpg(const uint8_t *G, int64_t p) {
    const uint32_t b = G[p];
    return (b == 1u && G[p + 1] == 2u) || (b == 2u && G[p - 1] == 1u);
}

template <bool MASKQ, bool SITE, class Src, class Tab, class Site>
__device__ void tally_end(const Tab &tab, const Site &site, uint32_t table, const Src &src, const RecHdr &h, const uint8_t *G,
                          int64_t s, uint32_t L, int N, bool left, bool comp, uint32_t min_bq) {
    const uint32_t c0 = ref_code(left ? G[s - 2] : G[s + L + 1]);
    const uint32_t c1 = ref_code(left ? G[s - 1] : G[s + L]);
    if (c0 < 4u) tab.add(table, 0, comp ? 15u - 5u * c0 : 5u * c0);
    if (c1 < 4u) tab.add(table, 1, comp ? 15u - 5u * c1 : 5u * c1);
    for (int i = 0; i < N; i++) {
        const uint32_t ri = left ? (uint32_t)i : L - 1u - (uint32_t)i;
        if (MASKQ && ri < h.l_seq && src.u8(h.qual_off + ri) < min_bq) continue;
        const uint32_t rd = nib_code(read_nibble(src, h, ri));
        const uint32_t rf = ref_code(G[s + (int64_t)ri]);
        if (rd < 4u && rf < 4u) {
            const uint32_t cell = 4u * rd + rf;
            tab.add(table, (uint32_t)i + 2u, comp ? 15u - cell : cell);
            if constexpr (SITE) {
                if (site_in_cpg(G, s + (int64_t)ri)) site.add(table, (uint32_t)i + 2u, comp ? 15u - cell : cell);
            }
        }
    }
}

template <bool MASKQ = false, bool SITE = false, class Src, class Tab, class Site>
__device__ __forceinline__ void tally_pss_record(const TallyParams &P, const Tab &tab, const Site &site, const Src &src,
                                                 const RecHdr &h, const Plan &pl) {
    const uint32_t min_bq = MASKQ ? P.min_bq : 0u;
    const uint8_t *G = P.genome + pl.gbase;
    if (pl.pss_fwd) tally_end<MASKQ, SITE>(tab, site, 0u, src, h, G, pl.s, pl.L, P.N, !pl.rev, pl.rev, min_bq);
    if (pl.pss_rev) tally_end<MASKQ, SITE>(tab, site, 1u, src, h, G, pl.s, pl.L, P.N, pl.rev, pl.rev, min_bq);
}
template <bool MASKQ = false, class Src, class Tab>
__device__ __forceinline__ void tally_pss_record(const TallyParams &P, const Tab &tab, const Src &src,
                                                 const RecHdr &h, const Plan &pl) {
    tally_pss_record<MASKQ, false>(P, tab, NoSite{}, src, h, pl);
}

template <bool LDS_KMER>
__device__ __forceinline__ bool tally_one_kmer(const TallyParams &P, const Plan &pl, uint32_t which, uint32_t *lds_kmer) {
    const uint8_t *G = P.genome + pl.gbase;
    int64_t w5, w3;
    kmer_windows(pl, P.K, w5, w3);
    uint32_t bin;
    if (!kmer_bin(G, which ? w3 : w5, P.K, pl.rev, bin)) return false;
    if (LDS_KMER) atomicAdd(&lds_kmer[(which ? (1u << (2 * P.K)) : 0u) + bin], 1u);
    else atomicAdd(&P.counters[(which ? P.off_k3 : P.off_k5) + bin], 1ull);
    return true;
}

template <bool LDS_KMER>
__device__ __forceinline__ bool tally_kmer_record(const TallyParams &P, const Plan &pl, uint32_t *lds_kmer) {
    bool good = true;
    if (pl.fk5) good = tally_one_kmer<LDS_KMER>(P, pl, 0u, lds_kmer) && good;
    if (pl.fk3) good = tally_one_kmer<LDS_KMER>(P, pl, 1u, lds_kmer) && good;
    return !good;
}

constexpr uint32_t HIST_LDS_MAX_BINS = 1024;
__host__ __device__ inline uint32_t hist_lds_bytes(uint32_t lds_bins) { return 2u * lds_bins * 4u; }

__device__ __forceinline__ void hist_add(const TallyParams &P, uint32_t *hist_lds, uint32_t b, bool fwd, bool rev, uint32_t n) {
    if (b < P.hist_lds_bins) {
        if (fwd) atomicAdd(&hist_lds[b], n);
        if (rev) atomicAdd(&hist_lds[P.hist_lds_bins + b], n);
    } else {
        if (fwd) atomicAdd(&P.counters[P.off_hist + b], (unsigned long long)n);
        if (rev) atomicAdd(&P.counters[P.off_hist + P.hist_max + 2u + b], (unsigned long long)n);
    }
}
__device__ __forceinline__ uint32_t hist_bin(const TallyParams &P, uint32_t L) { return min(L, P.hist_max + 1u); }

__device__ __forceinline__ void hist_wave_add(const TallyParams &P, uint32_t *hist_lds, bool on, uint32_t L, bool fwd, bool rev) {
    const uint32_t b = hist_bin(P, L);
    const uint32_t key = (b << 2) | (fwd ? 2u : 0u) | (rev ? 1u : 0u);
    const uint32_t lane = threadIdx.x & 63u;
    bool pending = on && (fwd || rev);
    for (uint32_t round = 0; __any(pending); round++) {
        if (pending) {
            if (round >= 2u && b < P.hist_lds_bins) {
                hist_add(P, hist_lds, b, fwd, rev, 1u);
                pending = false;
            } else {
                const uint32_t v = __builtin_amdgcn_readfirstlane(key);
                const bool same = key == v;
                const unsigned long long m = __ballot(same);
                if (same) {
                    pending = false;
                    if (lane == (uint32_t)__ffsll((long long)m) - 1u) hist_add(P, hist_lds, b, fwd, rev, (uint32_t)__popcll(m));
                }
            }
        }
    }
}

template <bool LDS_TABLE>
__global__ void __launch_bounds__(256) tally_simple(const TallyParams P) {
    extern __shared__ __attribute__((aligned(16))) uint32_t dyn_lds[];
    __shared__ int32_t lds_delta[ST_USED];
    const uint32_t rows = (uint32_t)P.N + 2u;
    const uint32_t tab_words = LDS_TABLE ? 2u * rows * 16u : 0u;
    const bool do_pss = (P.tally_mask & 1u) != 0, do_kmer = (P.tally_mask & 2u) != 0;
    for (uint32_t i = threadIdx.x; i < tab_words; i += blockDim.x) dyn_lds[i] = 0u;
    if (threadIdx.x < ST_USED) lds_delta[threadIdx.x] = 0;
    __syncthreads();

    const uint32_t stride = gridDim.x * blockDim.x;
    for (uint32_t r = blockIdx.x * blockDim.x + threadIdx.x; r < P.n_recs; r += stride) {
        const uint32_t o0 = P.offs[r], o1 = P.offs[r + 1];
        GlobalBytes src{P.recs + o0};
        const RecHdr h = decode_hdr(src, o1 - o0);
        Plan pl = make_plan<true, true>(P, src, h);
        if (!do_pss) pl.pss_fwd = pl.pss_rev = false;
        if (!do_kmer) pl.fk5 = pl.fk3 = false;
        if (pl.pss_fwd || pl.pss_rev) {
            if (P.off_site) {
                const GlobalSite site{P.counters + P.off_site, rows * 16u};
                if (LDS_TABLE) tally_pss_record<true, true>(P, LdsTableRowMajor{dyn_lds, rows}, site, src, h, pl);
                else tally_pss_record<true, true>(P, GlobalTable{P.counters, P.off_rev}, site, src, h, pl);
            } else if (LDS_TABLE) tally_pss_record<true>(P, LdsTableRowMajor{dyn_lds, rows}, src, h, pl);
            else tally_pss_record<true>(P, GlobalTable{P.counters, P.off_rev}, src, h, pl);
            if (P.hist_max) hist_add(P, nullptr, hist_bin(P, pl.L), pl.pss_fwd, pl.pss_rev, 1u);
        }
        bool kfail = false;
        if (pl.fk5 || pl.fk3) kfail = tally_kmer_record<false>(P, pl, nullptr);
        book_events(do_pss, do_kmer, record_events(do_pss, do_kmer, pl, kfail), lds_delta);
    }
    __syncthreads();
    if (LDS_TABLE) {
        for (uint32_t i = threadIdx.x; i < tab_words; i += blockDim.x) {
            const uint32_t v = dyn_lds[i];
            if (v) {
                const uint32_t table = i / (rows * 16u), rest = i % (rows * 16u);
                atomicAdd(&P.counters[(table ? P.off_rev : 0u) + rest], (unsigned long long)v);
            }
        }
    }
    flush_events(do_pss, do_kmer, P, lds_delta);
}

__host__ __device__ inline uint32_t tiled_lds_bytes(uint32_t T, uint32_t pieces) { return T * pieces * 16u + STAGE_SLACK; }

struct __attribute__((packed, aligned(4))) Quad { uint32_t v[4]; };
struct __attribute__((packed, aligned(4))) Tri { uint32_t v[3]; };

constexpr uint32_t TILED_MAX_T = 128;
static_assert(TILED_MAX_T * 2 == TILED_THREADS, "CODES maps one (read, end) pair to each thread");

__device__ __forceinline__ void stage_tile_dma(const uint8_t *recs, uint64_t recs_limit, const uint32_t *tile_offs,
                                               uint32_t count, uint32_t pieces, uint8_t *stage, uint32_t tid) {
    const uint32_t n_pieces = count * pieces;
    const uint32_t lds0 = (uint32_t)(uintptr_t)stage;
    const uint32_t magic = ((1u << 20) + pieces - 1u) / pieces;
    for (uint32_t q0 = (tid & ~63u); q0 < n_pieces; q0 += TILED_THREADS) {
        const uint32_t q = q0 + (tid & 63u);
        const uint32_t jq = (q * magic) >> 20;
        const uint32_t j = min(jq, count - 1u), pc = q - jq * pieces;
        const uint64_t a = (uint64_t)(tile_offs[j] & ~15u) + 16u * pc;
        if (q < n_pieces && a + 16u <= recs_limit) {
            const uint8_t *src = recs + a;
            const uint32_t m0v = __builtin_amdgcn_readfirstlane(lds0 + (q0 << 4));
            uint32_t keep;
            asm volatile("s_mov_b32 %0, m0\n\ts_mov_b32 m0, %2\n\ts_nop 0\n\tglobal_load_lds_dwordx4 %1, off nt\n\ts_mov_b32 m0, %0"
                         : "=&s"(keep) : "v"(src), "s"(m0v) : "memory");
        }
    }
}

template <bool DO_PSS, bool DO_KMER, bool LDS_KMER, bool MASKQ = false, bool REGIONS = false, bool HIST = false, bool SITE = false>
__device__ __attribute__((noinline)) uint32_t tally_overflow_record(const TallyParams *kernarg, uint32_t o0,
                                                                    uint32_t o1, uint32_t *table, uint32_t *lds_kmer,
                                                                    uint32_t *hist_lds = nullptr, uint32_t *site_lds = nullptr) {
    const TallyParams &P = *kernarg;
    GlobalBytes gsrc{P.recs + o0};
    const RecHdr gh = decode_hdr(gsrc, o1 - o0);
    const Plan gpl = make_plan<DO_PSS, DO_KMER, REGIONS>(P, gsrc, gh);
    if constexpr (SITE) {
        if (gpl.pss_fwd || gpl.pss_rev)
            tally_pss_record<MASKQ, true>(P, LdsTableColumnMajor{table, P.row_base}, LdsSiteColumnMajor{site_lds, P.row_base}, gsrc, gh, gpl);
    } else if (DO_PSS && (gpl.pss_fwd || gpl.pss_rev)) tally_pss_record<MASKQ>(P, LdsTableColumnMajor{table, P.row_base}, gsrc, gh, gpl);
    if constexpr (HIST) {
        if (gpl.pss_fwd || gpl.pss_rev) hist_add(P, hist_lds, hist_bin(P, gpl.L), gpl.pss_fwd, gpl.pss_rev, 1u);
    }
    bool kfail = false;
    if (DO_KMER && (gpl.fk5 || gpl.fk3)) kfail = tally_kmer_record<LDS_KMER>(P, gpl, lds_kmer);
    return record_events(DO_PSS, DO_KMER, gpl, kfail);
}

enum PlaneSel { PLANES_NONE = 0, PLANES_RG, PLANES_LEN, PLANES_REF };

template <PlaneSel PLANES, bool KMER = false, class Src>
__device__ __forceinline__ uint32_t record_plane(const Src &src, const RecHdr &h, const Plan &pl, const PlaneParams &G) {
    if constexpr (PLANES == PLANES_RG) return read_group_plane(src, h, G);
    else if constexpr (PLANES == PLANES_REF) return pl.ref_plane;
    else return length_bin_plane(G, KMER ? pl.Lk : pl.L);
}

__device__ __forceinline__ uint64_t kmer_plane_base(const TallyParams &P, const PlaneParams &G, uint32_t plane) {
    return plane ? G.koff_planes + (uint64_t)(plane - 1u) * G.kplane_words : (uint64_t)P.off_k5;
}
template <bool LDS_KMER>
__device__ __forceinline__ void kmer_plane_add(const TallyParams &P, const PlaneParams &G, uint32_t plane, uint32_t which,
                                               uint32_t bin, uint32_t *lds_kmer) {
    const uint32_t nb = 1u << (2 * P.K);
    if (LDS_KMER) {
        const uint32_t slot = min(plane - G.plane0, G.n_slots);
        atomicAdd(&lds_kmer[slot * 2u * nb + (which ? nb : 0u) + bin], 1u);
    } else {
        atomicAdd(&P.counters[kmer_plane_base(P, G, plane) + (which ? nb : 0u) + bin], 1ull);
    }
}
template <bool LDS_KMER>
__device__ __forceinline__ bool tally_kmer_record_plane(const TallyParams &P, const PlaneParams &G, const Plan &pl, uint32_t plane,
                                                        uint32_t *lds_kmer) {
    const uint8_t *Gn = P.genome + pl.gbase;
    int64_t w5, w3;
    kmer_windows(pl, P.K, w5, w3);
    bool good = true;
    for (uint32_t which = 0; which < 2u; which++) {
        if (!(which ? pl.fk3 : pl.fk5)) continue;
        uint32_t bin;
        if (kmer_bin(Gn, which ? w3 : w5, P.K, pl.rev, bin)) kmer_plane_add<LDS_KMER>(P, G, plane, which, bin, lds_kmer);
        else good = false;
    }
    return !good;
}
template <PlaneSel PLANES, bool LDS_KMER, bool REGIONS = false>
__device__ __attribute__((noinline)) uint32_t tally_overflow_record_kmer_planes(const TallyParams *kernarg, const PlaneParams *gk,
                                                                                uint32_t o0, uint32_t o1, uint32_t *lds_kmer) {
    const TallyParams &P = *kernarg;
    GlobalBytes gsrc{P.recs + o0};
    const RecHdr gh = decode_hdr(gsrc, o1 - o0);
    const Plan gpl = make_plan<false, true, REGIONS>(P, gsrc, gh);
    bool kfail = false;
    if (gpl.fk5 || gpl.fk3) kfail = tally_kmer_record_plane<LDS_KMER>(P, *gk, gpl, record_plane<PLANES, true>(gsrc, gh, gpl, *gk), lds_kmer);
    return record_events(false, true, gpl, kfail);
}

template <PlaneSel PLANES, bool MASKQ = false, bool REGIONS = false>
__device__ __attribute__((noinline)) uint32_t tally_overflow_record_planes(const TallyParams *kernarg, const PlaneParams *gk,
                                                                           uint32_t o0, uint32_t o1, uint32_t *table) {
    const TallyParams &P = *kernarg;
    GlobalBytes gsrc{P.recs + o0};
    const RecHdr gh = decode_hdr(gsrc, o1 - o0);
    const Plan gpl = make_plan<true, false, REGIONS>(P, gsrc, gh);
    if (gpl.pss_fwd || gpl.pss_rev) {
        const uint32_t slot = record_plane<PLANES>(gsrc, gh, gpl, *gk) - gk->plane0;
        if (slot < gk->n_slots) tally_pss_record<MASKQ>(P, LdsTableColumnMajor{table + slot * GROUP_PLANE_WORDS, P.row_base}, gsrc, gh, gpl);
    }
    return record_events(true, false, gpl, false);
}

__device__ __forceinline__ uint32_t base_quality_mask(uint32_t x, uint32_t q4) {
    const uint32_t lt = ~((x | 0x80808080u) - q4) & ~x & 0x80808080u;
    return (lt - (lt >> 7)) | lt;
}

template <bool DO_PSS, bool DO_KMER, bool LDS_KMER, bool LATER_PASS, PlaneSel PLANES = PLANES_NONE, bool MASKQ = false,
          bool REGIONS = false, bool HIST = false, bool SITE = false>
__device__ __forceinline__ void tally_tiled_body(const TallyParams &P, const TallyParams *kernarg,
                                                 uint8_t *__restrict__ stage, uint8_t *__restrict__ sheet,
                                                 uint32_t *__restrict__ table,
                                                 uint32_t *__restrict__ toffs,
                                                 uint32_t *__restrict__ lds_kmer,
                                                 int32_t *__restrict__ lds_delta, uint4 *__restrict__ refs_lds,
                                                 const PlaneParams *gk = nullptr, uint32_t *__restrict__ grp_lds = nullptr,
                                                 uint32_t *__restrict__ hist_lds = nullptr, uint32_t *__restrict__ site_lds = nullptr) {
    constexpr bool GROUPED = PLANES != PLANES_NONE;
    static_assert(!SITE || (DO_PSS && !DO_KMER && PLANES == PLANES_NONE && !HIST), "site context belongs to the one-plane substitution tally without the length histogram");
    static_assert(!HIST || (DO_PSS && !LATER_PASS && PLANES == PLANES_NONE), "the length histogram belongs to pass 0 of the one-plane substitution tally");
    constexpr bool KPLANES = GROUPED && DO_KMER;
    static_assert(!KPLANES || !DO_PSS, "planes split either the substitution tables or the k-mer tables");
    static_assert(!MASKQ || DO_PSS, "base qualities mask the substitution tables only");
    const uint32_t T = P.reads_per_tile;
    const uint32_t n_recs = P.n_recs_dev ? *P.n_recs_dev : P.n_recs;
    const uint32_t pieces = P.prefix_pieces;
    const uint64_t recs_limit = (P.recs_bytes + 15ull) & ~15ull;
    const uint32_t ablate = P.ablate;

    const uint32_t tid = threadIdx.x;
    const uint32_t lane = tid & 63u, wave = tid >> 6;
    const int N = P.N;
    const uint32_t n_pos = (uint32_t)N + 2u;
    const uint32_t row_base = LATER_PASS ? P.row_base : 0u;
    const bool pass0 = !LATER_PASS;
    const uint32_t n_live = n_pos > row_base ? min(n_pos - row_base, 32u) : 0u;

    const uint32_t table_words = KPLANES ? 0u : GROUPED ? (gk->n_slots + 1u) * GROUP_PLANE_WORDS : TABLE_WORDS;
    for (uint32_t i = tid; i < table_words; i += TILED_THREADS) table[i] = 0u;
    uint32_t kmer_words = 2u * (1u << (2 * P.K));
    if constexpr (KPLANES) kmer_words *= gk->n_slots + 1u;
    if (LDS_KMER)
        for (uint32_t i = tid; i < kmer_words; i += TILED_THREADS) lds_kmer[i] = 0u;
    if (tid < ST_USED) lds_delta[tid] = 0;
    if constexpr (HIST)
        for (uint32_t i = tid; i < 2u * P.hist_lds_bins; i += TILED_THREADS) hist_lds[i] = 0u;
    if constexpr (SITE)
        for (uint32_t i = tid; i < SITE_WORDS; i += TILED_THREADS) site_lds[i] = 0u;
    const uint32_t n_ref_cached = min((uint32_t)P.n_ref, REF_LDS_ENTRIES);
    if (tid < n_ref_cached) refs_lds[tid] = P.ref_info[tid];
    if (tid == n_ref_cached) refs_lds[tid] = P.ref_info[P.n_ref];
    const uint32_t all_tiles = (n_recs + T - 1u) / T;
    uint32_t tile0 = blockIdx.x, tstride = gridDim.x, n_tiles = all_tiles;
    if (P.xcd_map && (gridDim.x & 7u) == 0u && all_tiles >= 64u) {
        const uint32_t per = (all_tiles + 7u) >> 3, xcd = blockIdx.x & 7u;
        tile0 = xcd * per + (blockIdx.x >> 3);
        tstride = gridDim.x >> 3;
        n_tiles = min(all_tiles, (xcd + 1u) * per);
    }
    uint32_t tile = tile0;
    uint32_t off_a = 0;
    const uint32_t TOFF = TILED_MAX_T + 4u;
    auto load_offsets = [&](uint32_t t) {
        const uint32_t r0 = t * T;
        if (tid <= T && r0 + tid <= n_recs) off_a = P.offs[r0 + tid];
    };
    auto tile_count = [&](uint32_t t) { return min(T, n_recs - t * T); };
    __syncthreads();
    if (tile < n_tiles) {
        load_offsets(tile);
        if (tid <= T) toffs[tid] = off_a;
        __syncthreads();
        stage_tile_dma(P.recs, recs_limit, toffs, tile_count(tile), pieces, stage, tid);
        if (tile + tstride < n_tiles) load_offsets(tile + tstride);
    }

    for (uint32_t it = 0; tile < n_tiles; tile += tstride, it++) {
        const uint32_t par = it & 1u;
        const uint32_t *cur_offs = toffs + par * TOFF;
        const uint32_t r0 = tile * T;
        const uint32_t count = min(T, n_recs - r0);
        const uint32_t next = tile + tstride;

        asm volatile("s_waitcnt vmcnt(0)" ::: "memory");
        if (next < n_tiles && tid <= T) toffs[(par ^ 1u) * TOFF + tid] = off_a;
        __syncthreads();

        const uint32_t j = tid >> 1, e = tid & 1u;
        const bool lane_on = tid < 2u * T && !(ablate & 4u);
        const bool in_tile = lane_on && j < count;
        uint32_t o0 = 0, o1 = 0;
        if (in_tile) { o0 = cur_offs[j]; o1 = cur_offs[j + 1]; }
        const uint32_t avail = pieces * 16u - (o0 & 15u);
        const bool hdr_ok = in_tile && o1 - o0 >= 36u && avail >= 48u;
        LdsBytes src{stage, hdr_ok ? j * pieces * 16u + (o0 & 15u) : 0u};
        const RecHdr h = decode_hdr_lds(src, hdr_ok ? o1 - o0 : 0u);
        const uint32_t needed = (PLANES == PLANES_RG || P.rg) ? o1 - o0 : MASKQ ? h.aux_off : h.qual_off + 1u;
        const bool in_stage = hdr_ok && needed <= avail;
        Plan pl = plan_head<DO_PSS, DO_KMER>(P, src, h, RefsLdsCached{refs_lds, P.ref_info, n_ref_cached, (uint32_t)P.n_ref});
        if (!in_stage) { pl.status = RS_LIVE; pl.live = pl.pss_cand = pl.fk5 = pl.fk3 = false; }
        const bool cand = DO_PSS && pl.pss_cand;
        const bool rcand = REGIONS && (pl.pss_cand || pl.fk5 || pl.fk3);
        uint4 rdesc = make_uint4(0u, 0u, 0u, 0u);
        if constexpr (REGIONS) {
            if (rcand) rdesc = P.region_info[region_ref_index(P, h)];
        }
        uint32_t gq[5] = {0u, 0u, 0u, 0u, 0u};
        uint32_t gsh = 0u;
        uint32_t nb_front = 4u, nb_behind = 4u;
        if (cand) {
            const uint64_t ga = pl.gbase + (uint64_t)pl.s + (e ? (uint64_t)pl.L - 30ull - row_base : (uint64_t)row_base - 2ull);
            const uint32_t *pg = P.genome4 + (ga >> 3);
            if (!(ablate & 128u)) {
                const Quad q0 = *(const Quad *)pg;
#pragma unroll
                for (int k = 0; k < 4; k++) gq[k] = q0.v[k];
                gq[4] = pg[4];
                if constexpr (SITE) nb_front = P.genome4[(ga - 1ull) >> 3] >> (4u * (uint32_t)((ga - 1ull) & 7ull));
            }
            gsh = 4u * (uint32_t)(ga & 7ull);
        }
        uint32_t cx = 0u;
        if (cand && !pass0) {
            const uint64_t pc = pl.gbase + (uint64_t)pl.s + (e ? (uint64_t)pl.L : (uint64_t)-1ll);
            cx = (P.genome4[pc >> 3] >> (4u * (uint32_t)(pc & 7ull))) & 15u;
        }
        const int32_t n0 = e ? (int32_t)pl.L - 30 - (int32_t)row_base : (int32_t)row_base - 2;
        uint32_t rr[6];
#pragma unroll
        for (int k = 0; k < 6; k++) rr[k] = 0u;
        uint32_t ssh = 0u;
        if (cand) {
            const int32_t n0a = min(n0, (int32_t)h.l_seq);
            const uint32_t sa = src.off + (uint32_t)((int32_t)h.seq_off + (n0a >> 1));
            const uint32_t *qs = (const uint32_t *)(stage + (sa & ~3u));
            ssh = sa & 3u;
#pragma unroll
            for (int k = 0; k < 6; k++) rr[k] = qs[k];
        }
        uint32_t qq[MASKQ ? 9 : 1];
        uint32_t qsh = 0u;
        if constexpr (MASKQ) {
#pragma unroll
            for (int k = 0; k < 9; k++) qq[k] = 0u;
            if (cand) {
                const int32_t n0q = min(n0, (int32_t)h.l_seq);
                const uint32_t qa = src.off + (uint32_t)((int32_t)h.qual_off + n0q);
                const uint32_t *qp = (const uint32_t *)(stage + (qa & ~3u));
                qsh = qa & 3u;
#pragma unroll
                for (int k = 0; k < 9; k++) qq[k] = qp[k];
            }
        }
        const uint32_t kwhich = e ^ (pl.rev ? 1u : 0u);
        bool kmer_try = DO_KMER && (kwhich ? pl.fk3 : pl.fk5) && !(ablate & 16u);
        uint32_t kw[3] = {0u, 0u, 0u};
        uint32_t ksh = 0u;
        if (kmer_try) {
            int64_t w5, w3;
            kmer_windows(pl, P.K, w5, w3);
            const uint64_t ka = pl.gbase + (uint64_t)(kwhich ? w3 : w5);
            const Tri kq = *(const Tri *)(P.genome4 + (ka >> 3));
#pragma unroll
            for (int k = 0; k < 3; k++) kw[k] = kq.v[k];
            ksh = 4u * (uint32_t)(ka & 7ull);
        }
        RegionQuery rq{};
        if constexpr (REGIONS) {
            if (rcand) region_grid_load(P, h, rdesc, rq);
        }
        uint32_t kplane = 0u;
        if constexpr (KPLANES) {
            if (e == 0u && (pl.fk5 || pl.fk3)) kplane = record_plane<PLANES, true>(src, h, pl, *gk);
            const uint32_t left = (uint32_t)__shfl_xor((int)kplane, 1);
            if (e) kplane = left;
        }
        if constexpr (GROUPED && !KPLANES) {
            if (in_tile && e == 0u) {
                const uint32_t slot = cand ? record_plane<PLANES>(src, h, pl, *gk) - gk->plane0 : gk->n_slots;
                grp_lds[j] = slot < gk->n_slots ? slot : gk->n_slots;
            }
        }
        uint32_t ev_over = 0u;
        if (in_tile && !in_stage && e == 0u) {
            if constexpr (KPLANES) ev_over = tally_overflow_record_kmer_planes<PLANES, LDS_KMER, REGIONS>(kernarg, gk, o0, o1, lds_kmer);
            else if constexpr (GROUPED) ev_over = tally_overflow_record_planes<PLANES, MASKQ, REGIONS>(kernarg, gk, o0, o1, table);
            else ev_over = tally_overflow_record<DO_PSS, DO_KMER, LDS_KMER, MASKQ, REGIONS, HIST, SITE>(kernarg, o0, o1, table, lds_kmer, hist_lds, site_lds);
            if (pass0) atomicAdd(&lds_delta[ST_SLOW_PATH], 1);
        }
        uint32_t W[4];
#pragma unroll
        for (int m = 0; m < 4; m++) W[m] = __builtin_amdgcn_alignbit(gq[m + 1], gq[m], gsh);
#pragma unroll
        for (int k = 0; k < 2; k++) kw[k] = __builtin_amdgcn_alignbit(kw[k + 1], kw[k], ksh);
#pragma unroll
        for (int m = 0; m < 4; m++) asm volatile("" : "+v"(W[m]));
        asm volatile("" : "+v"(cx));
        if constexpr (SITE) {
            nb_front &= 15u;
            nb_behind = (gq[4] >> gsh) & 15u;
            asm volatile("" : "+v"(nb_front));
            asm volatile("" : "+v"(nb_behind));
        }
        if (DO_KMER) {
#pragma unroll
            for (int k = 0; k < 2; k++) asm volatile("" : "+v"(kw[k]));
        }
        if constexpr (MASKQ) {
#pragma unroll
            for (int k = 0; k < 9; k++) asm volatile("" : "+v"(qq[k]));
        }
        if constexpr (REGIONS) {
            if (rcand && !region_resolve(P, rq)) {
                pl.pss_cand = pl.fk5 = pl.fk3 = false;
                kmer_try = false;
            }
        }
        __syncthreads();

        if (next < n_tiles) {
            stage_tile_dma(P.recs, recs_limit, toffs + (par ^ 1u) * TOFF, tile_count(next), pieces, stage, tid);
            if (next + tstride < n_tiles) load_offsets(next + tstride);
        }

        {
            const uint32_t own1 = !pass0 ? cx : e ? (W[3] >> 24) & 15u : (W[0] >> 4) & 15u;
            const uint32_t other1 = (uint32_t)__shfl_xor((int)own1, 1);
            if (DO_PSS) plan_finish_pss_packed(P.acgt_ctx, pl, e ? other1 : own1, e ? own1 : other1);
            uint32_t code_w[8];
#pragma unroll
            for (int k = 0; k < 8; k++) code_w[k] = CODE_NONE * 0x01010101u;
            const uint32_t tsel = e ^ (pl.rev ? 1u : 0u);
            if (cand && (tsel ? pl.pss_rev : pl.pss_fwd) && !(ablate & 2u)) {
                uint32_t S[5];
#pragma unroll
                for (int k = 0; k < 5; k++) S[k] = __builtin_amdgcn_alignbyte(rr[k + 1], rr[k], ssh);
                const bool odd = (n0 & 1) != 0;
                const uint32_t M = 0x0F0F0F0Fu;
                const uint32_t sx = pl.rev ? 0u : 0x1E1E1E1Eu;
                const uint32_t tsel4 = tsel * 0x01010101u;
                uint32_t RE[4], RO[4], GE[4], GO[4];
#pragma unroll
                for (int m = 0; m < 4; m++) {
                    const uint32_t S1 = __builtin_amdgcn_alignbyte(S[m + 1], S[m], 1);
                    const uint32_t A = odd ? S1 : S[m];
                    const uint32_t hiA = (A >> 4) & M, loS = S[m] & M;
                    const uint32_t E = odd ? loS : hiA, O = odd ? hiA : loS;
                    RE[m] = __builtin_amdgcn_perm(0xFF1098FFu, 0xFFFFFF08u, E ^ 0x04040404u);
                    RO[m] = __builtin_amdgcn_perm(0xFF1098FFu, 0xFFFFFF08u, O ^ 0x04040404u);
                    GE[m] = __builtin_amdgcn_perm(0xFFFFFFFFu, 0x00020406u, W[m] & M);
                    GO[m] = __builtin_amdgcn_perm(0xFFFFFFFFu, 0x00020406u, (W[m] >> 4) & M);
                }
                if constexpr (MASKQ) {
                    const uint32_t q4 = P.min_bq * 0x01010101u;
                    uint32_t Qb[8];
#pragma unroll
                    for (int k = 0; k < 8; k++) Qb[k] = __builtin_amdgcn_alignbyte(qq[k + 1], qq[k], qsh);
#pragma unroll
                    for (int m = 0; m < 4; m++) {
                        RE[m] |= base_quality_mask(__builtin_amdgcn_perm(Qb[2 * m + 1], Qb[2 * m], 0x06040200u), q4);
                        RO[m] |= base_quality_mask(__builtin_amdgcn_perm(Qb[2 * m + 1], Qb[2 * m], 0x07050301u), q4);
                    }
                }
                const int32_t have_s = (int32_t)h.l_seq - n0;
                const uint32_t have = have_s <= 0 ? 0u : have_s >= 32 ? 32u : (uint32_t)have_s;
                if (__any(have < (e && pass0 ? 30u : 32u))) {
#pragma unroll
                    for (int m = 0; m < 4; m++) {
                        const uint32_t left = have > 8u * m ? have - 8u * m : 0u;
                        const uint32_t ne = min((left + 1u) >> 1, 4u), no = min(left >> 1, 4u);
                        RE[m] |= ne >= 4u ? 0u : ~((1u << (8u * ne)) - 1u);
                        RO[m] |= no >= 4u ? 0u : ~((1u << (8u * no)) - 1u);
                    }
                }
                {
                    const uint32_t ml = (e || !pass0) ? 0u : 0x000000FFu, mr = (e && pass0) ? 0xFF000000u : 0u;
                    RE[0] = (RE[0] & ~ml) | ((GE[0] << 2) & ml & 0x18181818u);
                    RO[0] = (RO[0] & ~ml) | ((GO[0] << 2) & ml & 0x18181818u);
                    RE[3] = (RE[3] & ~mr) | ((GE[3] << 2) & mr & 0x18181818u);
                    RO[3] = (RO[3] & ~mr) | ((GO[3] << 2) & mr & 0x18181818u);
                }
#pragma unroll
                for (int m = 0; m < 4; m++) {
                    code_w[2 * m] = ((RE[m] | GE[m] | tsel4) ^ sx) & 0x3F3F3F3Fu;
                    code_w[2 * m + 1] = ((RO[m] | GO[m] | tsel4) ^ sx) & 0x3F3F3F3Fu;
                }
                if constexpr (SITE) {
                    const uint32_t B = 0x02020202u;
                    uint32_t cE[4], gE[5], cO[5], gO[4];
                    cO[0] = nb_front == 1u ? 0x02000000u : 0u;
                    gE[4] = nb_behind == 2u ? 0x00000002u : 0u;
#pragma unroll
                    for (int m = 0; m < 4; m++) {
                        const uint32_t yE = GE[m] & 0x06060606u, yO = GO[m] & 0x06060606u;
                        cE[m] = (yE >> 1) & ~yE & B;
                        gE[m] = yE & ~(yE >> 1) & B;
                        cO[m + 1] = (yO >> 1) & ~yO & B;
                        gO[m] = yO & ~(yO >> 1) & B;
                    }
                    const uint32_t ml = (e || !pass0) ? 0u : 0x000000FFu, mr = (e && pass0) ? 0xFF000000u : 0u;
#pragma unroll
                    for (int m = 0; m < 4; m++) {
                        const uint32_t keep = ~((m == 0 ? ml : 0u) | (m == 3 ? mr : 0u));
                        const uint32_t inE = (cE[m] & gO[m]) | (gE[m] & __builtin_amdgcn_alignbyte(cO[m + 1], cO[m], 3));
                        const uint32_t inO = (cO[m + 1] & __builtin_amdgcn_alignbyte(gE[m + 1], gE[m], 1)) | (gO[m] & cE[m]);
                        code_w[2 * m] |= (inE << 5) & keep;
                        code_w[2 * m + 1] |= (inO << 5) & keep;
                    }
                }
            }
            bool kmer_ok = true;
            if (kmer_try) {
                uint32_t bin = 0u, bad = 0u;
#pragma unroll
                for (int t = 0; t < 16; t++) {
                    if (t < P.K) {
                        const uint32_t c = (kw[t >> 3] >> (4 * (t & 7))) & 0xFu;
                        bad |= c & ~3u;
                        bin = pl.rev ? (bin | ((3u - (c & 3u)) << (2 * t))) : ((bin << 2) | (c & 3u));
                    }
                }
                kmer_ok = bad == 0u;
                if (kmer_ok && !(ablate & 8u)) {
                    if constexpr (KPLANES) kmer_plane_add<LDS_KMER>(P, *gk, kplane, kwhich, bin, lds_kmer);
                    else if (LDS_KMER) atomicAdd(&lds_kmer[(kwhich ? (1u << (2 * P.K)) : 0u) + bin], 1u);
                    else atomicAdd(&P.counters[(kwhich ? P.off_k3 : P.off_k5) + bin], 1ull);
                }
            }
            if (lane_on && !KPLANES) {
                uint4 *dst = (uint4 *)(sheet + j * 64u + e * 32u);
                dst[0] = make_uint4(code_w[0], code_w[1], code_w[2], code_w[3]);
                dst[1] = make_uint4(code_w[4], code_w[5], code_w[6], code_w[7]);
            }
            bool kfail = false;
            if (DO_KMER) {
                const int bad = (kmer_try && !kmer_ok) ? 1 : 0;
                const int bad_other = __shfl_xor(bad, 1);
                kfail = (bad | bad_other) != 0;
            }
            if (e == 0u && pass0) book_events(DO_PSS, DO_KMER, in_stage ? record_events(DO_PSS, DO_KMER, pl, kfail) : ev_over, lds_delta);
            if constexpr (HIST) hist_wave_add(P, hist_lds, e == 0u, pl.L, pl.pss_fwd, pl.pss_rev);
        }

        if (DO_PSS && !(ablate & 1u)) {
            const uint32_t e = lane >> 5, b = lane & 31u;
            const uint32_t wpos = (b & 24u) + 2u * (b & 3u) + ((b >> 2) & 1u);
            const uint32_t row = e ? 31u - wpos : wpos;
            const uint32_t j0 = min(count, wave * 32u), j1 = min(count, j0 + 32u);
            if (GROUPED && row < n_live) {
                const uint32_t trash_off = (gk->n_slots - 1u) * GROUP_PLANE_WORDS;
                uint32_t j = j0;
                for (; j + 8u <= j1; j += 8u) {
                    uint32_t c[8], po[8];
#pragma unroll
                    for (int u = 0; u < 8; u++) {
                        c[u] = sheet[(j + u) * 64u + lane];
                        po[u] = __builtin_amdgcn_readfirstlane(grp_lds[j + u]) * GROUP_PLANE_WORDS;
                    }
#pragma unroll
                    for (int u = 0; u < 8; u++) atomicAdd(&table[(c[u] << 5) + row + (c[u] < 32u ? po[u] : trash_off)], 1u);
                }
                for (; j < j1; j++) {
                    const uint32_t c = sheet[j * 64u + lane];
                    const uint32_t po = __builtin_amdgcn_readfirstlane(grp_lds[j]) * GROUP_PLANE_WORDS;
                    atomicAdd(&table[(c << 5) + row + (c < 32u ? po : trash_off)], 1u);
                }
            } else if (SITE && row < n_live) {
                auto add = [&](uint32_t c) {
                    atomicAdd(&table[((c & 63u) << 5) + row], 1u);
                    if ((c & (CODE_SITE | CODE_NONE)) == CODE_SITE) atomicAdd(&site_lds[((((c >> 1) & 14u) | (c & 1u)) << 5) + row], 1u);
                };
                uint32_t j = j0;
                for (; j + 8u <= j1; j += 8u) {
                    uint32_t c[8];
#pragma unroll
                    for (int u = 0; u < 8; u++) c[u] = sheet[(j + u) * 64u + lane];
#pragma unroll
                    for (int u = 0; u < 8; u++) add(c[u]);
                }
                for (; j < j1; j++) add(sheet[j * 64u + lane]);
            } else if (row < n_live) {
                uint32_t j = j0;
                for (; j + 8u <= j1; j += 8u) {
                    uint32_t c[8];
#pragma unroll
                    for (int u = 0; u < 8; u++) c[u] = sheet[(j + u) * 64u + lane];
#pragma unroll
                    for (int u = 0; u < 8; u++) atomicAdd(&table[(c[u] << 5) + row], 1u);
                }
                for (; j < j1; j++) atomicAdd(&table[((uint32_t)sheet[j * 64u + lane] << 5) + row], 1u);
            }
        }
    }

    __syncthreads();
    if constexpr (KPLANES) {
        uint32_t *mine = P.scratch + (size_t)blockIdx.x * gk->scratch_words;
        const uint32_t n_words = LDS_KMER ? gk->n_slots * 2u * (1u << (2 * P.K)) : 0u;
        for (uint32_t i = tid; i < n_words; i += TILED_THREADS) mine[GROUP_SCRATCH_DELTA + i] = lds_kmer[i];
        if (tid < 16u) mine[tid] = tid < (uint32_t)ST_USED ? (uint32_t)lds_delta[tid] : 0u;
    } else if constexpr (GROUPED) {
        uint32_t *mine = P.scratch + (size_t)blockIdx.x * gk->scratch_words;
        const uint32_t n_words = gk->n_slots * GROUP_PLANE_WORDS;
        for (uint32_t i = tid; i < n_words; i += TILED_THREADS) mine[GROUP_SCRATCH_DELTA + i] = table[i];
        if (tid < 16u) mine[tid] = tid < (uint32_t)ST_USED ? (uint32_t)lds_delta[tid] : 0u;
    } else {
    uint32_t *mine = P.scratch + (size_t)blockIdx.x * (SITE ? SITE_SCRATCH_WORDS : SCRATCH_WORDS);
    if constexpr (SITE)
        for (uint32_t i = tid; i < SITE_WORDS; i += TILED_THREADS) mine[SCRATCH_WORDS + i] = site_lds[i];
    for (uint32_t i = tid; i < 32u * 32u; i += TILED_THREADS) mine[i] = DO_PSS ? table[i] : 0u;
    for (uint32_t i = tid; i < 512u; i += TILED_THREADS)
        mine[SCRATCH_KMER + i] = (LDS_KMER && i < 2u * (1u << (2 * P.K))) ? lds_kmer[i] : 0u;
    if (tid < 16u) mine[SCRATCH_DELTA + tid] = tid < (uint32_t)ST_USED ? (uint32_t)lds_delta[tid] : 0u;
    }
    if constexpr (HIST) {
        for (uint32_t i = tid; i < 2u * P.hist_lds_bins; i += TILED_THREADS) {
            const uint32_t v = hist_lds[i];
            if (v) atomicAdd(&P.counters[P.off_hist + (i < P.hist_lds_bins ? i : P.hist_max + 2u + (i - P.hist_lds_bins))], (unsigned long long)v);
        }
    }
}


constexpr uint32_t COMPACT_MAX_ROWS = 18;
constexpr uint32_t CTX_REP = 16;
constexpr uint32_t CTX_WORDS = 16 * CTX_REP;
constexpr uint32_t COMPACT_TABLE_WORDS = 33 * 32;

__device__ __forceinline__ void stage_tile_dma32(const uint8_t *recs, uint32_t recs_limit32, const uint32_t *tile_offs,
                                                 uint32_t count, uint32_t pieces, uint8_t *stage, uint32_t tid) {
    const uint32_t n_pieces = count * pieces;
    const uint32_t lds0 = (uint32_t)(uintptr_t)stage;
    const uint32_t magic = ((1u << 20) + pieces - 1u) / pieces;
    for (uint32_t q0 = (tid & ~63u); q0 < n_pieces; q0 += TILED_THREADS) {
        const uint32_t q = q0 + (tid & 63u);
        const uint32_t jq = (q * magic) >> 20;
        const uint32_t j = min(jq, count - 1u), pc = q - jq * pieces;
        const uint32_t a = (tile_offs[j] & ~15u) + 16u * pc;
        if (q < n_pieces && a <= recs_limit32) {
            const uint32_t m0v = __builtin_amdgcn_readfirstlane(lds0 + (q0 << 4));
            uint32_t keep;
            asm volatile("s_mov_b32 %0, m0\n\ts_mov_b32 m0, %3\n\ts_nop 0\n\tglobal_load_lds_dwordx4 %1, %2\n\ts_mov_b32 m0, %0"
                         : "=&s"(keep) : "v"(a), "s"(recs), "s"(m0v) : "memory");
        }
    }
}

struct LdsTableCompact {
    uint32_t *t;
    uint32_t *ctx;
    __device__ __forceinline__ void add(uint32_t table, uint32_t row, uint32_t cell) const {
        if (row >= 2u) { if (row < COMPACT_MAX_ROWS) atomicAdd(&t[(((cell << 1) | table) << 5) + (row - 2u)], 1u); }
        else atomicAdd(&ctx[((table * 2u + row) * 4u + cell / 5u) * CTX_REP], 1u);
    }
};

template <bool DO_KMER, bool LDS_KMER>
__device__ __attribute__((noinline)) uint32_t tally_overflow_record_compact(const TallyParams *kernarg, uint32_t o0, uint32_t o1,
                                                                            uint32_t *table, uint32_t *ctx, uint32_t *lds_kmer) {
    const TallyParams &P = *kernarg;
    GlobalBytes gsrc{P.recs + o0};
    const RecHdr gh = decode_hdr(gsrc, o1 - o0);
    const Plan gpl = make_plan<true, DO_KMER, false>(P, gsrc, gh);
    if (gpl.pss_fwd || gpl.pss_rev) tally_pss_record(P, LdsTableCompact{table, ctx}, gsrc, gh, gpl);
    bool kfail = false;
    if (DO_KMER && (gpl.fk5 || gpl.fk3)) kfail = tally_kmer_record<LDS_KMER>(P, gpl, lds_kmer);
    return record_events(true, DO_KMER, gpl, kfail);
}

template <bool DO_KMER, bool LDS_KMER, int DECODE_REPS = 1, bool PLAN_ONCE = false>
__device__ __forceinline__ void tally_compact_body(const TallyParams &P, const TallyParams *kernarg,
                                                   uint8_t *__restrict__ stage, uint8_t *__restrict__ sheet,
                                                   uint32_t *__restrict__ table, uint32_t *__restrict__ toffs,
                                                   uint32_t *__restrict__ lds_kmer, int32_t *__restrict__ lds_delta,
                                                   uint4 *__restrict__ refs_lds, uint32_t *__restrict__ ctx_rep,
                                                   uint32_t *__restrict__ ovf_list, uint32_t *__restrict__ ovf_n) {
    const uint32_t T = P.reads_per_tile;
    const uint32_t n_recs = P.n_recs_dev ? *P.n_recs_dev : P.n_recs;
    const uint32_t pieces = P.prefix_pieces;
    const uint32_t recs_limit32 = (uint32_t)(((P.recs_bytes + 15ull) & ~15ull) - 16ull);
    const uint32_t tid = threadIdx.x;
    const uint32_t lane = tid & 63u, wave = tid >> 6;

    uint32_t up_tab = 0u, dn_tab = 0u;
#pragma unroll
    for (uint32_t n = 0; n < 8u; n++) {
        const uint32_t c = n < 4u ? 3u - n : n;
        const uint32_t u = n < 4u ? (P.acgt_ctx >> (2u * n)) & 1u : n & 1u, uc = c < 4u ? (P.acgt_ctx >> (2u * c)) & 1u : c & 1u;
        const uint32_t d = n < 4u ? (P.acgt_ctx >> (2u * n + 1u)) & 1u : (n >> 1) & 1u, dc = c < 4u ? (P.acgt_ctx >> (2u * c + 1u)) & 1u : (c >> 1) & 1u;
        up_tab |= (u << n) | (uc << (16u + n));
        dn_tab |= (d << n) | (dc << (16u + n));
    }

    for (uint32_t i = tid; i < COMPACT_TABLE_WORDS; i += TILED_THREADS) table[i] = 0u;
    if (tid < CTX_WORDS) ctx_rep[tid] = 0u;
    if (LDS_KMER)
        for (uint32_t i = tid; i < 2u * (1u << (2 * P.K)); i += TILED_THREADS) lds_kmer[i] = 0u;
    if (tid < ST_USED) lds_delta[tid] = 0;
    if (tid == 0u) *ovf_n = 0u;
    const uint32_t n_ref_cached = min((uint32_t)P.n_ref, REF_LDS_ENTRIES);
    if (tid < n_ref_cached) refs_lds[tid] = P.ref_info[tid];
    if (tid == n_ref_cached) refs_lds[tid] = P.ref_info[P.n_ref];
    const uint32_t all_tiles = (n_recs + T - 1u) / T;
    uint32_t tile = blockIdx.x;
    const uint32_t tstride = gridDim.x, n_tiles = all_tiles;
    uint32_t off_a = 0;
    const uint32_t TOFF = TILED_MAX_T + 4u;
    auto load_offsets = [&](uint32_t t) {
        const uint32_t r0 = t * T;
        if (tid <= T && r0 + tid <= n_recs) off_a = P.offs[r0 + tid];
    };
    auto tile_count = [&](uint32_t t) { return min(T, n_recs - t * T); };
    __syncthreads();
    if (tile < n_tiles) {
        load_offsets(tile);
        if (tid <= T) toffs[tid] = off_a;
        __syncthreads();
        stage_tile_dma32(P.recs, recs_limit32, toffs, tile_count(tile), pieces, stage, tid);
        if (tile + tstride < n_tiles) load_offsets(tile + tstride);
    }

    for (uint32_t it = 0; tile < n_tiles; tile += tstride, it++) {
        const uint32_t par = it & 1u;
        const uint32_t *cur_offs = toffs + par * TOFF;
        const uint32_t r0 = tile * T;
        const uint32_t count = min(T, n_recs - r0);
        const uint32_t next = tile + tstride;

        asm volatile("s_waitcnt vmcnt(0)" ::: "memory");
        if (next < n_tiles && tid <= T) toffs[(par ^ 1u) * TOFF + tid] = off_a;
        __syncthreads();

        const uint32_t j = tid >> 1, e = tid & 1u;
        const bool lane_on = tid < 2u * T;
        Plan pl;
        uint32_t l_seq = 0, soff = 0;
        bool in_stage = false;
        if constexpr (PLAN_ONCE) {
            uint4 *plan_lds = (uint4 *)sheet;
            if (tid < T) {
                const bool in_t = tid < count;
                uint32_t o0 = 0, o1 = 0;
                if (in_t) { o0 = cur_offs[tid]; o1 = cur_offs[tid + 1]; }
                const uint32_t avail = pieces * 16u - (o0 & 15u);
                const bool hdr_ok = in_t && o1 - o0 >= 36u && avail >= 48u;
                LdsBytes src{stage, hdr_ok ? tid * pieces * 16u + (o0 & 15u) : 0u};
                const RecHdr h = decode_hdr_lds32(src, hdr_ok ? o1 - o0 : 0u);
                const bool staged = hdr_ok && h.qual_off + 1u <= avail;
                Plan p1 = plan_head<true, DO_KMER, false>(P, src, h, RefsLdsCached{refs_lds, P.ref_info, n_ref_cached, (uint32_t)P.n_ref});
                if (!staged) { p1.status = RS_LIVE; p1.live = p1.pss_cand = p1.fk5 = p1.fk3 = false; }
                if (in_t && !staged) ovf_list[atomicAdd(ovf_n, 1u)] = tid;
                const uint32_t bits = (p1.flag & 0xFFFFu) | (p1.status << 16) | (p1.live ? 1u << 18 : 0u) | (p1.pss_cand ? 1u << 19 : 0u) |
                                      (p1.fk5 ? 1u << 20 : 0u) | (p1.fk3 ? 1u << 21 : 0u) | (staged ? 1u << 22 : 0u);
                plan_lds[2u * tid] = make_uint4((uint32_t)p1.gbase, (uint32_t)(p1.gbase >> 32), (uint32_t)p1.s, p1.L);
                plan_lds[2u * tid + 1u] = make_uint4(h.l_seq, src.off + h.seq_off, bits, p1.Lk);
            }
            __syncthreads();
            const uint4 qa = plan_lds[2u * j], qb = plan_lds[2u * j + 1u];
            pl.gbase = (uint64_t)qa.x | ((uint64_t)qa.y << 32);
            pl.s = (int32_t)qa.z;
            pl.L = qa.w;
            l_seq = qb.x;
            soff = qb.y;
            pl.flag = qb.z & 0xFFFFu;
            pl.status = (qb.z >> 16) & 3u;
            pl.live = lane_on && ((qb.z >> 18) & 1u);
            pl.pss_cand = lane_on && ((qb.z >> 19) & 1u);
            pl.fk5 = lane_on && ((qb.z >> 20) & 1u);
            pl.fk3 = lane_on && ((qb.z >> 21) & 1u);
            in_stage = lane_on && ((qb.z >> 22) & 1u);
            pl.Lk = qb.w;
            pl.rev = (pl.flag & FL_REVERSE) != 0;
            pl.pss_fwd = pl.pss_rev = false;
        } else {
        const bool in_tile = lane_on && j < count;
        uint32_t o0 = 0, o1 = 0;
        if (in_tile) { o0 = cur_offs[j]; o1 = cur_offs[j + 1]; }
        const uint32_t avail = pieces * 16u - (o0 & 15u);
        const bool hdr_ok = in_tile && o1 - o0 >= 36u && avail >= 48u;
        LdsBytes src{stage, hdr_ok ? j * pieces * 16u + (o0 & 15u) : 0u};
        const RecHdr h = decode_hdr_lds32(src, hdr_ok ? o1 - o0 : 0u);
        const uint32_t needed = h.qual_off + 1u;
        in_stage = hdr_ok && needed <= avail;
        pl = plan_head<true, DO_KMER, false>(P, src, h, RefsLdsCached{refs_lds, P.ref_info, n_ref_cached, (uint32_t)P.n_ref});
        if constexpr (DECODE_REPS > 1) {
            uint32_t off2 = src.off;
            asm volatile("" : "+v"(off2));
            const LdsBytes src2{stage, off2};
            const RecHdr h2 = decode_hdr_lds32(src2, hdr_ok ? o1 - o0 : 0u);
            const Plan p2 = plan_head<true, DO_KMER, false>(P, src2, h2, RefsLdsCached{refs_lds, P.ref_info, n_ref_cached, (uint32_t)P.n_ref});
            const uint32_t sink = (uint32_t)p2.s ^ p2.L ^ p2.flag ^ (uint32_t)p2.gbase ^ (uint32_t)(p2.gbase >> 32) ^ p2.status ^ (p2.pss_cand ? 1u : 0u) ^
                                  (p2.rev ? 2u : 0u) ^ (p2.fk5 ? 4u : 0u) ^ (p2.fk3 ? 8u : 0u) ^ h2.seq_off ^ h2.qual_off;
            asm volatile("" ::"v"(sink));
        }
        if (!in_stage) { pl.status = RS_LIVE; pl.live = pl.pss_cand = pl.fk5 = pl.fk3 = false; }
        l_seq = h.l_seq;
        soff = src.off + h.seq_off;
        if (in_tile && !in_stage && e == 0u) ovf_list[atomicAdd(ovf_n, 1u)] = j;
        }
        const bool cand = pl.pss_cand;
        uint32_t gq[4] = {0u, 0u, 0u, 0u};
        uint32_t gsh = 0u;
        if (cand) {
            const uint64_t ga = pl.gbase + (uint64_t)(int64_t)((int32_t)pl.s + (e ? (int32_t)pl.L - 16 : -2));
            const Quad q0 = *(const Quad *)(P.genome4 + (ga >> 3));
#pragma unroll
            for (int k = 0; k < 4; k++) gq[k] = q0.v[k];
            gsh = 4u * (uint32_t)(ga & 7ull);
        }
        const int32_t n0 = e ? (int32_t)pl.L - 16 : 0;
        uint32_t rr[3] = {0u, 0u, 0u};
        uint32_t ssh = 0u;
        if (cand) {
            const int32_t n0a = min(n0, (int32_t)l_seq);
            const uint32_t sa = soff + (uint32_t)(n0a >> 1);
            const uint32_t *qs = (const uint32_t *)(stage + (sa & ~3u));
            ssh = sa & 3u;
#pragma unroll
            for (int k = 0; k < 3; k++) rr[k] = qs[k];
        }
        const uint32_t kwhich = e ^ (pl.rev ? 1u : 0u);
        const bool kmer_try = DO_KMER && (kwhich ? pl.fk3 : pl.fk5);
        uint32_t kw[3] = {0u, 0u, 0u};
        uint32_t ksh = 0u;
        if (kmer_try) {
            int64_t w5, w3;
            kmer_windows(pl, P.K, w5, w3);
            const uint64_t ka = pl.gbase + (uint64_t)(kwhich ? w3 : w5);
            const Tri kq = *(const Tri *)(P.genome4 + (ka >> 3));
#pragma unroll
            for (int k = 0; k < 3; k++) kw[k] = kq.v[k];
            ksh = 4u * (uint32_t)(ka & 7ull);
        }
        uint32_t A[3];
#pragma unroll
        for (int m = 0; m < 3; m++) A[m] = __builtin_amdgcn_alignbit(gq[m + 1], gq[m], gsh);
#pragma unroll
        for (int k = 0; k < 2; k++) kw[k] = __builtin_amdgcn_alignbit(kw[k + 1], kw[k], ksh);
#pragma unroll
        for (int m = 0; m < 3; m++) asm volatile("" : "+v"(A[m]));
        if (DO_KMER) {
#pragma unroll
            for (int k = 0; k < 2; k++) asm volatile("" : "+v"(kw[k]));
        }
        __syncthreads();

        if (next < n_tiles) {
            stage_tile_dma32(P.recs, recs_limit32, toffs + (par ^ 1u) * TOFF, tile_count(next), pieces, stage, tid);
            if (next + tstride < n_tiles) load_offsets(next + tstride);
        }

        {
            const uint32_t cx = e ? A[2] : A[0];
            const uint32_t c_lo = cx & 15u, c_hi = (cx >> 4) & 15u;
            const uint32_t own1 = e ? c_lo : c_hi, own2 = e ? c_hi : c_lo;
            const uint32_t other1 = (uint32_t)__shfl_xor((int)own1, 1);
            {
                const uint32_t left1 = e ? other1 : own1, right1 = e ? own1 : other1;
                const uint32_t rsh = pl.rev ? 16u : 0u;
                const bool up_ok = ((up_tab >> ((pl.rev ? right1 : left1) + rsh)) & 1u) != 0;
                const bool dn_ok = ((dn_tab >> ((pl.rev ? left1 : right1) + rsh)) & 1u) != 0;
                const bool paired = (pl.flag & FL_PAIRED) != 0;
                const bool r1 = (pl.flag & FL_READ1) != 0, r2 = (pl.flag & FL_READ2) != 0;
                pl.pss_fwd = pl.pss_cand && (paired ? (r1 && up_ok) : (up_ok && dn_ok));
                pl.pss_rev = pl.pss_cand && (paired ? (!(r1 && up_ok) && r2 && dn_ok) : (up_ok && dn_ok));
            }
            const uint32_t G0 = e ? A[0] : __builtin_amdgcn_alignbit(A[1], A[0], 8);
            const uint32_t G1 = e ? A[1] : __builtin_amdgcn_alignbit(A[2], A[1], 8);
            uint32_t code_w[4];
#pragma unroll
            for (int k = 0; k < 4; k++) code_w[k] = CODE_NONE * 0x01010101u;
            const uint32_t tsel = e ^ (pl.rev ? 1u : 0u);
            const bool tallied = cand && (tsel ? pl.pss_rev : pl.pss_fwd);
            if (tallied) {
                uint32_t S[3];
                S[0] = __builtin_amdgcn_alignbyte(rr[1], rr[0], ssh);
                S[1] = __builtin_amdgcn_alignbyte(rr[2], rr[1], ssh);
                S[2] = __builtin_amdgcn_alignbyte(0u, rr[2], ssh);
                const bool odd = (n0 & 1) != 0;
                const uint32_t M = 0x0F0F0F0Fu;
                const uint32_t sx = pl.rev ? 0u : 0x1E1E1E1Eu;
                const uint32_t tsel4 = tsel * 0x01010101u;
                const uint32_t Gw[2] = {G0, G1};
                uint32_t RE[2], RO[2], GE[2], GO[2];
#pragma unroll
                for (int m = 0; m < 2; m++) {
                    const uint32_t S1 = __builtin_amdgcn_alignbyte(S[m + 1], S[m], 1);
                    const uint32_t Ax = odd ? S1 : S[m];
                    const uint32_t hiA = (Ax >> 4) & M, loS = S[m] & M;
                    const uint32_t E = odd ? loS : hiA, O = odd ? hiA : loS;
                    RE[m] = __builtin_amdgcn_perm(0xFF1098FFu, 0xFFFFFF08u, E ^ 0x04040404u);
                    RO[m] = __builtin_amdgcn_perm(0xFF1098FFu, 0xFFFFFF08u, O ^ 0x04040404u);
                    GE[m] = __builtin_amdgcn_perm(0xFFFFFFFFu, 0x00020406u, Gw[m] & M);
                    GO[m] = __builtin_amdgcn_perm(0xFFFFFFFFu, 0x00020406u, (Gw[m] >> 4) & M);
                }
                const int32_t have_s = (int32_t)l_seq - n0;
                const uint32_t have = have_s <= 0 ? 0u : have_s >= 16 ? 16u : (uint32_t)have_s;
                if (__any(have < 16u)) {
#pragma unroll
                    for (int m = 0; m < 2; m++) {
                        const uint32_t left = have > 8u * m ? have - 8u * m : 0u;
                        const uint32_t ne = min((left + 1u) >> 1, 4u), no = min(left >> 1, 4u);
                        RE[m] |= ne >= 4u ? 0u : ~((1u << (8u * ne)) - 1u);
                        RO[m] |= no >= 4u ? 0u : ~((1u << (8u * no)) - 1u);
                    }
                }
#pragma unroll
                for (int m = 0; m < 2; m++) {
                    code_w[2 * m] = ((RE[m] | GE[m] | tsel4) ^ sx) & 0x3F3F3F3Fu;
                    code_w[2 * m + 1] = ((RO[m] | GO[m] | tsel4) ^ sx) & 0x3F3F3F3Fu;
                }
                const uint32_t rep = lane & (CTX_REP - 1u);
                const uint32_t b1 = pl.rev ? 3u - own1 : own1, b2 = pl.rev ? 3u - own2 : own2;
                if (own1 < 4u) atomicAdd(&ctx_rep[((tsel * 2u + 1u) * 4u + b1) * CTX_REP + rep], 1u);
                if (own2 < 4u) atomicAdd(&ctx_rep[((tsel * 2u + 0u) * 4u + b2) * CTX_REP + rep], 1u);
            }
            bool kmer_ok = true;
            if (kmer_try) {
                uint32_t bin = 0u, bad = 0u;
#pragma unroll
                for (int t = 0; t < 16; t++) {
                    if (t < P.K) {
                        const uint32_t c = (kw[t >> 3] >> (4 * (t & 7))) & 0xFu;
                        bad |= c & ~3u;
                        bin = pl.rev ? (bin | ((3u - (c & 3u)) << (2 * t))) : ((bin << 2) | (c & 3u));
                    }
                }
                kmer_ok = bad == 0u;
                if (kmer_ok) {
                    if (LDS_KMER) atomicAdd(&lds_kmer[(kwhich ? (1u << (2 * P.K)) : 0u) + bin], 1u);
                    else atomicAdd(&P.counters[(kwhich ? P.off_k3 : P.off_k5) + bin], 1ull);
                }
            }
            if (lane_on)
                *(uint4 *)(sheet + j * 32u + e * 16u) = make_uint4(code_w[0], code_w[1], code_w[2], code_w[3]);
            bool kfail = false;
            if (DO_KMER) {
                const int bad = (kmer_try && !kmer_ok) ? 1 : 0;
                const int bad_other = __shfl_xor(bad, 1);
                kfail = (bad | bad_other) != 0;
            }
            if (e == 0u && in_stage) book_events(true, DO_KMER, record_events(true, DO_KMER, pl, kfail), lds_delta);
        }

        {
            const uint32_t ee = (lane >> 4) & 1u, b = lane & 15u;
            const uint32_t w = (b & 8u) + 2u * (b & 3u) + ((b >> 2) & 1u);
            const uint32_t posn = ee ? 15u - w : w;
            const uint32_t slot = ee * 16u + posn;
            const uint32_t j0 = min(count, wave * 32u), j1 = min(count, j0 + 32u);
            if (posn < (uint32_t)P.N) {
                const uint32_t rd = lane >> 5;
                uint32_t jj = j0;
                for (; jj + 16u <= j1; jj += 16u) {
                    uint32_t c[8];
#pragma unroll
                    for (int u = 0; u < 8; u++) c[u] = sheet[(jj + 2u * u) * 32u + lane];
#pragma unroll
                    for (int u = 0; u < 8; u++) atomicAdd(&table[(min(c[u], 32u) << 5) + slot], 1u);
                }
                for (; jj < j1; jj += 2u)
                    if (jj + rd < j1) atomicAdd(&table[(min((uint32_t)sheet[jj * 32u + lane], 32u) << 5) + slot], 1u);
            }
        }
        const uint32_t n_ovf = *ovf_n;
        if (n_ovf) {
            for (uint32_t i = tid; i < n_ovf; i += TILED_THREADS) {
                const uint32_t jo = ovf_list[i];
                const uint32_t ev = tally_overflow_record_compact<DO_KMER, LDS_KMER>(kernarg, cur_offs[jo], cur_offs[jo + 1u], table,
                                                                                    ctx_rep, lds_kmer);
                book_events(true, DO_KMER, ev, lds_delta);
                atomicAdd(&lds_delta[ST_SLOW_PATH], 1);
            }
            __syncthreads();
            if (tid == 0u) *ovf_n = 0u;
        }
    }

    __syncthreads();
    uint32_t *mine = P.scratch + (size_t)blockIdx.x * SCRATCH_WORDS;
    for (uint32_t i = tid; i < 32u * 32u; i += TILED_THREADS) {
        const uint32_t ct = i >> 5, row = i & 31u;
        uint32_t v = 0u;
        if (row >= 2u && row < COMPACT_MAX_ROWS) v = table[(ct << 5) + (row - 2u)] + table[(ct << 5) + 16u + (row - 2u)];
        else if (row < 2u) {
            const uint32_t t = ct & 1u, cell = ct >> 1;
            if (cell % 5u == 0u) {
                const uint32_t *rp = ctx_rep + ((t * 2u + row) * 4u + cell / 5u) * CTX_REP;
                for (uint32_t k = 0; k < CTX_REP; k++) v += rp[k];
            }
        }
        mine[i] = v;
    }
    for (uint32_t i = tid; i < 512u; i += TILED_THREADS)
        mine[SCRATCH_KMER + i] = (LDS_KMER && i < 2u * (1u << (2 * P.K))) ? lds_kmer[i] : 0u;
    if (tid < 16u) mine[SCRATCH_DELTA + tid] = tid < (uint32_t)ST_USED ? (uint32_t)lds_delta[tid] : 0u;
}

template <bool DO_KMER, bool LDS_KMER, bool PLAN_ONCE = false>
__global__ void __launch_bounds__(TILED_THREADS) tally_compact(const TallyParams P) {
    extern __shared__ __attribute__((aligned(16))) uint8_t stage[];
    __shared__ __attribute__((aligned(16))) uint8_t sheet[TILED_MAX_T * 32u];
    __shared__ uint32_t table[COMPACT_TABLE_WORDS];
    __shared__ uint32_t toffs[2u * (TILED_MAX_T + 4u)];
    __shared__ uint32_t lds_kmer[LDS_KMER ? 2u * (1u << (2 * KMER_LDS_MAX_K)) : 1u];
    __shared__ int32_t lds_delta[ST_USED];
    __shared__ uint4 refs_lds[REF_LDS_ENTRIES + 1];
    __shared__ uint32_t ctx_rep[CTX_WORDS];
    __shared__ uint32_t ovf_list[TILED_MAX_T + 1];
    const TallyParams *kernarg = (const TallyParams *)__builtin_amdgcn_kernarg_segment_ptr();
    tally_compact_body<DO_KMER, LDS_KMER, 1, PLAN_ONCE>(P, kernarg, stage, sheet, table, toffs, lds_kmer, lds_delta, refs_lds, ctx_rep, ovf_list,
                                                        ovf_list + TILED_MAX_T);
}

__global__ void __launch_bounds__(TILED_THREADS) tally_compact_decode_twice(const TallyParams P) {
    extern __shared__ __attribute__((aligned(16))) uint8_t stage[];
    __shared__ __attribute__((aligned(16))) uint8_t sheet[TILED_MAX_T * 32u];
    __shared__ uint32_t table[COMPACT_TABLE_WORDS];
    __shared__ uint32_t toffs[2u * (TILED_MAX_T + 4u)];
    __shared__ uint32_t lds_kmer[1u];
    __shared__ int32_t lds_delta[ST_USED];
    __shared__ uint4 refs_lds[REF_LDS_ENTRIES + 1];
    __shared__ uint32_t ctx_rep[CTX_WORDS];
    __shared__ uint32_t ovf_list[TILED_MAX_T + 1];
    const TallyParams *kernarg = (const TallyParams *)__builtin_amdgcn_kernarg_segment_ptr();
    tally_compact_body<false, false, 2>(P, kernarg, stage, sheet, table, toffs, lds_kmer, lds_delta, refs_lds, ctx_rep, ovf_list,
                                        ovf_list + TILED_MAX_T);
}

constexpr uint32_t REDUCE_GROUPS = 32;
template <bool SITE = false>
__global__ void __launch_bounds__(256) reduce_partials(const TallyParams P, uint32_t n_slots, uint32_t lds_kmer_on) {
    constexpr uint32_t SLOT_WORDS = SITE ? SITE_SCRATCH_WORDS : SCRATCH_WORDS;
    const uint32_t gid = blockIdx.x * blockDim.x + threadIdx.x;
    const uint32_t i = gid % SLOT_WORDS, g = gid / SLOT_WORDS;
    if (g >= REDUCE_GROUPS) return;
    const bool do_pss = (P.tally_mask & 1u) != 0, do_kmer = (P.tally_mask & 2u) != 0;
    const uint32_t n_pos = (uint32_t)P.N + 2u;
    unsigned long long *dst = nullptr;
    bool is_delta = false;
    if (i < 1024u) {
        const uint32_t row = P.row_base + (i & 31u), ct = i >> 5, t = ct & 1u, cell = ct >> 1;
        if (do_pss && row < n_pos) dst = &P.counters[(t ? P.off_rev : 0u) + row * 16u + cell];
    } else if (i < SCRATCH_DELTA) {
        const uint32_t k = i - SCRATCH_KMER, nb = do_kmer ? 1u << (2 * P.K) : 0u;
        if (lds_kmer_on && k < 2u * nb) dst = &P.counters[k < nb ? P.off_k5 + k : P.off_k3 + (k - nb)];
    } else if (SITE && i >= SCRATCH_WORDS) {
        const uint32_t k = i - SCRATCH_WORDS, row = P.row_base + (k & 31u), hc = k >> 5;
        const uint32_t cell = ((hc >> 2) << 2) | ((hc & 2u) ? 2u : 1u);
        if (row >= 2u && row < n_pos) dst = &P.counters[P.off_site + ((hc & 1u) ? n_pos * 16u : 0u) + row * 16u + cell];
    } else {
        const uint32_t k = i - SCRATCH_DELTA;
        if (k < (uint32_t)ST_USED && P.row_base == 0u) { dst = &P.counters[P.off_stats + k]; is_delta = true; }
    }
    if (!dst) return;
    long long sum = 0;
    const uint32_t *p = P.scratch + i;
#pragma unroll 8
    for (uint32_t b = g; b < n_slots; b += REDUCE_GROUPS) {
        const uint32_t v = p[(size_t)b * SLOT_WORDS];
        sum += is_delta ? (long long)(int32_t)v : (long long)v;
    }
    if (is_delta && g == 0u) {
        const uint32_t k = i - SCRATCH_DELTA;
        if (k == ST_RECORDS || (do_pss && k == ST_PSS_OK) || (do_kmer && k == ST_KMER_OK)) sum += P.n_recs_dev ? *P.n_recs_dev : P.n_recs;
    }
    if (sum) atomicAdd(dst, (unsigned long long)sum);
}

template <bool DO_PSS, bool DO_KMER, bool LDS_KMER, bool LATER_PASS = false, bool MASKQ = false, bool REGIONS = false, bool HIST = false,
          bool SITE = false>
__global__ void __launch_bounds__(TILED_THREADS) tally_tiled(const TallyParams P) {
    extern __shared__ __attribute__((aligned(16))) uint8_t stage[];
    __shared__ __attribute__((aligned(16))) uint8_t sheet[TILED_MAX_T * 64u];
    __shared__ uint32_t table[TABLE_WORDS];
    __shared__ uint32_t toffs[2u * (TILED_MAX_T + 4u)];
    __shared__ uint32_t lds_kmer[LDS_KMER ? 2u * (1u << (2 * KMER_LDS_MAX_K)) : 1u];
    __shared__ int32_t lds_delta[ST_USED];
    __shared__ uint4 refs_lds[REF_LDS_ENTRIES + 1];
    const TallyParams *kernarg = (const TallyParams *)__builtin_amdgcn_kernarg_segment_ptr();
    uint32_t *hist_lds = HIST ? (uint32_t *)(stage + tiled_lds_bytes(P.reads_per_tile, P.prefix_pieces)) : nullptr;
    if constexpr (SITE) {
        __shared__ uint32_t site_lds[SITE_WORDS];
        tally_tiled_body<DO_PSS, DO_KMER, LDS_KMER, LATER_PASS, PLANES_NONE, MASKQ, REGIONS, HIST, true>(P, kernarg, stage, sheet, table, toffs, lds_kmer,
                                                                                                      lds_delta, refs_lds, nullptr, nullptr, hist_lds, site_lds);
    } else
    tally_tiled_body<DO_PSS, DO_KMER, LDS_KMER, LATER_PASS, PLANES_NONE, MASKQ, REGIONS, HIST>(P, kernarg, stage, sheet, table, toffs, lds_kmer,
                                                                                            lds_delta, refs_lds, nullptr, nullptr, hist_lds);
}

constexpr size_t PLANE_KERNARG_OFFSET = (sizeof(TallyParams) + alignof(PlaneParams) - 1) & ~(alignof(PlaneParams) - 1);

template <PlaneSel PLANES, bool LATER_PASS, bool MASKQ = false, bool REGIONS = false>
__global__ void __launch_bounds__(TILED_THREADS) tally_tiled_planes(const TallyParams P, const PlaneParams G) {
    extern __shared__ __attribute__((aligned(16))) uint8_t stage[];
    __shared__ __attribute__((aligned(16))) uint8_t sheet[TILED_MAX_T * 64u];
    __shared__ uint32_t toffs[2u * (TILED_MAX_T + 4u)];
    __shared__ uint32_t grp_lds[TILED_MAX_T];
    __shared__ uint32_t lds_kmer[1];
    __shared__ int32_t lds_delta[ST_USED];
    __shared__ uint4 refs_lds[REF_LDS_ENTRIES + 1];
    const TallyParams *kernarg = (const TallyParams *)__builtin_amdgcn_kernarg_segment_ptr();
    const PlaneParams *gk = (const PlaneParams *)((const uint8_t *)kernarg + PLANE_KERNARG_OFFSET);
    uint32_t *table = (uint32_t *)(stage + tiled_lds_bytes(P.reads_per_tile, P.prefix_pieces));
    tally_tiled_body<true, false, false, LATER_PASS, PLANES, MASKQ, REGIONS>(P, kernarg, stage, sheet, table, toffs, lds_kmer, lds_delta,
                                                                             refs_lds, gk, grp_lds);
}
constexpr uint32_t GROUPED_LDS_BUDGET = 148u * 1024u;
__host__ __device__ inline uint32_t tiled_grouped_lds_bytes(uint32_t T, uint32_t pieces, uint32_t n_slots) {
    return tiled_lds_bytes(T, pieces) + (n_slots + 1u) * GROUP_PLANE_WORDS * 4u;
}

__global__ void __launch_bounds__(256) reduce_partials_grouped(const TallyParams P, const PlaneParams G, uint32_t n_slots) {
    const uint32_t sw = G.scratch_words;
    const uint32_t gid = blockIdx.x * blockDim.x + threadIdx.x;
    const uint32_t i = gid % sw, g = gid / sw;
    if (g >= REDUCE_GROUPS) return;
    const uint32_t n_pos = (uint32_t)P.N + 2u;
    unsigned long long *dst = nullptr;
    bool is_delta = false;
    if (i < GROUP_SCRATCH_DELTA) {
        if (i < (uint32_t)ST_USED && P.row_base == 0u && G.plane0 == 0u) { dst = &P.counters[P.off_stats + i]; is_delta = true; }
    } else {
        const uint32_t w = (i - GROUP_SCRATCH_DELTA) & (GROUP_PLANE_WORDS - 1u), plane = G.plane0 + (i - GROUP_SCRATCH_DELTA) / GROUP_PLANE_WORDS;
        const uint32_t row = P.row_base + (w & 31u), ct = w >> 5, t = ct & 1u, cell = ct >> 1;
        const uint32_t base = plane ? G.off_groups + (plane - 1u) * G.plane_words : 0u;
        if (plane <= G.n_groups && row < n_pos) dst = &P.counters[base + (t ? P.off_rev : 0u) + row * 16u + cell];
    }
    if (!dst) return;
    long long sum = 0;
    const uint32_t *p = P.scratch + i;
#pragma unroll 8
    for (uint32_t b = g; b < n_slots; b += REDUCE_GROUPS) {
        const uint32_t v = p[(size_t)b * sw];
        sum += is_delta ? (long long)(int32_t)v : (long long)v;
    }
    if (is_delta && g == 0u && (i == ST_RECORDS || i == ST_PSS_OK)) sum += P.n_recs_dev ? *P.n_recs_dev : P.n_recs;
    if (sum) atomicAdd(dst, (unsigned long long)sum);
}

template <PlaneSel PLANES>
__global__ void __launch_bounds__(256) tally_simple_planes(const TallyParams P, const PlaneParams G) {
    __shared__ int32_t lds_delta[ST_USED];
    if (threadIdx.x < ST_USED) lds_delta[threadIdx.x] = 0;
    __syncthreads();
    const uint32_t stride = gridDim.x * blockDim.x;
    for (uint32_t r = blockIdx.x * blockDim.x + threadIdx.x; r < P.n_recs; r += stride) {
        const uint32_t o0 = P.offs[r], o1 = P.offs[r + 1];
        GlobalBytes src{P.recs + o0};
        const RecHdr h = decode_hdr(src, o1 - o0);
        const Plan pl = make_plan<true, false>(P, src, h);
        if (pl.pss_fwd || pl.pss_rev) {
            const uint32_t plane = record_plane<PLANES>(src, h, pl, G);
            unsigned long long *base = P.counters + (plane ? G.off_groups + (plane - 1u) * G.plane_words : 0u);
            tally_pss_record<true>(P, GlobalTable{base, P.off_rev}, src, h, pl);
        }
        book_events(true, false, record_events(true, false, pl, false), lds_delta);
    }
    __syncthreads();
    flush_events(true, false, P, lds_delta);
}

template <PlaneSel PLANES, bool LDS_KMER, bool REGIONS = false>
__global__ void __launch_bounds__(TILED_THREADS) tally_tiled_kmer_planes(const TallyParams P, const PlaneParams G) {
    extern __shared__ __attribute__((aligned(16))) uint8_t stage[];
    __shared__ uint32_t toffs[2u * (TILED_MAX_T + 4u)];
    __shared__ int32_t lds_delta[ST_USED];
    __shared__ uint4 refs_lds[REF_LDS_ENTRIES + 1];
    const TallyParams *kernarg = (const TallyParams *)__builtin_amdgcn_kernarg_segment_ptr();
    const PlaneParams *gk = (const PlaneParams *)((const uint8_t *)kernarg + PLANE_KERNARG_OFFSET);
    uint32_t *lds_kmer = (uint32_t *)(stage + tiled_lds_bytes(P.reads_per_tile, P.prefix_pieces));
    tally_tiled_body<false, true, LDS_KMER, false, PLANES, false, REGIONS>(P, kernarg, stage, nullptr, nullptr, toffs, lds_kmer, lds_delta,
                                                                           refs_lds, gk);
}
constexpr uint32_t KMER_PLANES_LDS_BUDGET = 156u * 1024u;
__host__ __device__ inline uint32_t tiled_kmer_planes_lds_bytes(uint32_t T, uint32_t pieces, uint32_t n_slots, int K, bool lds_kmer) {
    return tiled_lds_bytes(T, pieces) + (lds_kmer ? (n_slots + 1u) * 2u * (1u << (2 * K)) * 4u : 0u);
}

__global__ void __launch_bounds__(256) reduce_partials_kmer_planes(const TallyParams P, const PlaneParams G, uint32_t n_slots,
                                                                   uint32_t lds_kmer_on) {
    const uint32_t sw = G.scratch_words;
    const uint32_t gid = blockIdx.x * blockDim.x + threadIdx.x;
    const uint32_t i = gid % sw, g = gid / sw;
    if (g >= REDUCE_GROUPS) return;
    unsigned long long *dst = nullptr;
    bool is_delta = false;
    if (i < GROUP_SCRATCH_DELTA) {
        if (i < (uint32_t)ST_USED && G.plane0 == 0u) { dst = &P.counters[P.off_stats + i]; is_delta = true; }
    } else if (lds_kmer_on) {
        const uint32_t kw = 2u * (1u << (2 * P.K));
        const uint32_t w = (i - GROUP_SCRATCH_DELTA) % kw, plane = G.plane0 + (i - GROUP_SCRATCH_DELTA) / kw;
        if (plane <= G.n_groups) dst = &P.counters[kmer_plane_base(P, G, plane) + w];
    }
    if (!dst) return;
    long long sum = 0;
    const uint32_t *p = P.scratch + i;
#pragma unroll 8
    for (uint32_t b = g; b < n_slots; b += REDUCE_GROUPS) {
        const uint32_t v = p[(size_t)b * sw];
        sum += is_delta ? (long long)(int32_t)v : (long long)v;
    }
    if (is_delta && g == 0u && (i == ST_RECORDS || i == ST_KMER_OK)) sum += P.n_recs_dev ? *P.n_recs_dev : P.n_recs;
    if (sum) atomicAdd(dst, (unsigned long long)sum);
}

template <PlaneSel PLANES>
__global__ void __launch_bounds__(256) tally_simple_kmer_planes(const TallyParams P, const PlaneParams G) {
    __shared__ int32_t lds_delta[ST_USED];
    if (threadIdx.x < ST_USED) lds_delta[threadIdx.x] = 0;
    __syncthreads();
    const uint32_t stride = gridDim.x * blockDim.x;
    for (uint32_t r = blockIdx.x * blockDim.x + threadIdx.x; r < P.n_recs; r += stride) {
        const uint32_t o0 = P.offs[r], o1 = P.offs[r + 1];
        GlobalBytes src{P.recs + o0};
        const RecHdr h = decode_hdr(src, o1 - o0);
        const Plan pl = make_plan<false, true>(P, src, h);
        bool kfail = false;
        if (pl.fk5 || pl.fk3) kfail = tally_kmer_record_plane<false>(P, G, pl, record_plane<PLANES, true>(src, h, pl, G), nullptr);
        book_events(false, true, record_events(false, true, pl, kfail), lds_delta);
    }
    __syncthreads();
    flush_events(false, true, P, lds_delta);
}

constexpr uint32_t GKC_SPAN = 256;
template <bool LDS_BINS>
__global__ void __launch_bounds__(256) genome_kmer_kernel(const uint8_t *genome, uint64_t n, int K,
                                                          unsigned long long *bins) {
    __shared__ uint32_t lds_bins[LDS_BINS ? 4096 : 1];
    const uint32_t nb = 1u << (2 * K), mask = nb - 1u;
    if (LDS_BINS) {
        for (uint32_t i = threadIdx.x; i < nb; i += blockDim.x) lds_bins[i] = 0u;
        __syncthreads();
    }
    const uint64_t n_spans = (n + GKC_SPAN - 1) / GKC_SPAN;
    for (uint64_t sp = (uint64_t)blockIdx.x * blockDim.x + threadIdx.x; sp < n_spans; sp += (uint64_t)gridDim.x * blockDim.x) {
        const uint64_t p0 = sp * GKC_SPAN, p1 = min(n, p0 + GKC_SPAN);
        uint32_t code = 0u, run = 0u;
        for (uint64_t p = p0 >= (uint64_t)(K - 1) ? p0 - (uint64_t)(K - 1) : 0; p < p0; p++) {
            const uint32_t c = genome[p];
            run = c < 4u ? run + 1u : 0u;
            code = ((code << 2) | (c & 3u)) & mask;
        }
        for (uint64_t p = p0; p < p1; p += 4) {
            const uint32_t w = *(const uint32_t *)(genome + p);
#pragma unroll
            for (int b = 0; b < 4; b++) {
                if (p + b < p1) {
                    const uint32_t c = (w >> (8 * b)) & 0xFFu;
                    run = c < 4u ? run + 1u : 0u;
                    code = ((code << 2) | (c & 3u)) & mask;
                    if (run >= (uint32_t)K) {
                        if (LDS_BINS) atomicAdd(&lds_bins[code], 1u);
                        else atomicAdd(&bins[code], 1ull);
                    }
                }
            }
        }
    }
    if (LDS_BINS) {
        __syncthreads();
        for (uint32_t i = threadIdx.x; i < nb; i += blockDim.x)
            if (lds_bins[i]) atomicAdd(&bins[i], (unsigned long long)lds_bins[i]);
    }
}

constexpr uint32_t GKC4_SPAN = 256;
__global__ void __launch_bounds__(512) genome_kmer_packed_kernel(const uint32_t *g4, uint64_t n_pos, int K, uint32_t bin_lo,
                                                                 uint32_t n_bins, uint32_t rep_log2,
                                                                 unsigned long long *bins) {
    extern __shared__ uint32_t lds_hist[];
    const uint32_t rep = 1u << rep_log2;
    for (uint32_t i = threadIdx.x; i < (n_bins << rep_log2); i += blockDim.x) lds_hist[i] = 0u;
    __syncthreads();
    const uint32_t mask = (1u << (2 * K)) - 1u;
    const uint32_t copy = threadIdx.x & (rep - 1u);
    const uint64_t n_spans = (n_pos + GKC4_SPAN - 1) / GKC4_SPAN;
    for (uint64_t sp = (uint64_t)blockIdx.x * blockDim.x + threadIdx.x; sp < n_spans; sp += (uint64_t)gridDim.x * blockDim.x) {
        const uint64_t p0 = sp * GKC4_SPAN;
        const uint4 *src = (const uint4 *)(g4 + p0 / 8);
        uint32_t code = 0u, run = 0u;
        if (p0) {
            const uint32_t w = g4[p0 / 8 - 1];
#pragma unroll
            for (int b = 1; b < 8; b++) {
                const uint32_t c = (w >> (4 * b)) & 15u;
                run = c < 4u ? run + 1u : 0u;
                code = (code << 2) | (c & 3u);
            }
            run = min(run, (uint32_t)(K - 1));
        }
#pragma unroll 2
        for (int q = 0; q < (int)(GKC4_SPAN / 32); q++) {
            if (p0 + 32ull * q >= n_pos) break;
            const uint4 v = src[q];
            const uint32_t w4[4] = {v.x, v.y, v.z, v.w};
#pragma unroll
            for (int d = 0; d < 4; d++) {
#pragma unroll
                for (int b = 0; b < 8; b++) {
                    const uint32_t c = (w4[d] >> (4 * b)) & 15u;
                    run = c < 4u ? run + 1u : 0u;
                    code = ((code << 2) | (c & 3u)) & mask;
                    const uint32_t slot = code - bin_lo;
                    if (run >= (uint32_t)K && slot < n_bins && p0 + 32ull * q + 8u * d + b < n_pos)
                        atomicAdd(&lds_hist[(slot << rep_log2) + copy], 1u);
                }
            }
        }
    }
    __syncthreads();
    for (uint32_t i = threadIdx.x; i < n_bins; i += blockDim.x) {
        uint32_t sum = 0u;
        for (uint32_t r = 0; r < rep; r++) sum += lds_hist[(i << rep_log2) + r];
        if (sum) atomicAdd(&bins[bin_lo + i], (unsigned long long)sum);
    }
}

__global__ void copy_table_kernel(uint4 *dst, const uint4 *src, uint32_t n) {
    for (uint32_t i = threadIdx.x; i < n; i += blockDim.x) dst[i] = src[i];
}

__global__ void encode_genome_kernel(uint8_t *p, uint64_t n16) {
    const uint64_t stride = (uint64_t)gridDim.x * blockDim.x;
    uint4 *q = (uint4 *)p;
    for (uint64_t i = (uint64_t)blockIdx.x * blockDim.x + threadIdx.x; i < n16; i += stride) {
        uint4 v = q[i];
        uint32_t w[4] = {v.x, v.y, v.z, v.w};
#pragma unroll
// ... 33 lines not shown
```

Baseline: 23.71 billion.

## Decode each read once per thread and share header via lane permutes

```diff
diff --git a/pss-bam_amd/csrc/engine.hip b/pss-bam_amd/csrc/engine.hip
--- a/pss-bam_amd/csrc/engine.hip
+++ b/pss-bam_amd/csrc/engine.hip
@@ -140,7 +140,6 @@
 enum PrepSlot : int {
     PREP_TILED_PSS, PREP_TILED_PSS_LATER, PREP_TILED_PSS_KMER, PREP_TILED_PSS_KMER_LDS, PREP_TILED_KMER, PREP_TILED_KMER_LDS,
     PREP_COMPACT, PREP_COMPACT_KMER, PREP_COMPACT_KMER_LDS,
-    PREP_COMPACT_ONCE, PREP_COMPACT_ONCE_KMER, PREP_COMPACT_ONCE_KMER_LDS, PREP_COMPACT_DECODE_TWICE,
     PREP_PLANES_RG, PREP_PLANES_RG_LATER, PREP_PLANES_LEN, PREP_PLANES_LEN_LATER, PREP_PLANES_REF, PREP_PLANES_REF_LATER,
     PREP_KPLANES_RG, PREP_KPLANES_RG_LDS, PREP_KPLANES_LEN, PREP_KPLANES_LEN_LDS, PREP_KPLANES_REF, PREP_KPLANES_REF_LDS,
     PREP_TILED_PSS_BQ, PREP_TILED_PSS_LATER_BQ, PREP_TILED_PSS_KMER_BQ, PREP_TILED_PSS_KMER_LDS_BQ,
@@ -251,7 +250,6 @@
     int env_tile_reads = 0, env_grid_mult = 0, env_simple_blocks = 0, env_grid_wgs = 0, env_pieces = 0;
     int env_group_slots = 0;
     bool warned_ablate = false;
-    bool compact_plan_once = false;
     uint32_t prep_lds[2 * PREP_N] = {0};
     int prep_occ[2 * PREP_N] = {0};
     bool use_compact = true;
@@ -388,7 +386,6 @@
     if (getenv("PSSBAM_HIST_LDS_BINS")) e->env_hist_lds_bins = std::max(env_int("PSSBAM_HIST_LDS_BINS"), 0);
     if (const int g = env_int("PSSBAM_REGION_GRID_SHIFT")) e->region_shift = (uint32_t)std::min(std::max(g, 2), 20);
     if (getenv("PSSBAM_COMPACT")) e->use_compact = env_int("PSSBAM_COMPACT") != 0;
-    if (getenv("PSSBAM_COMPACT_PLAN_ONCE")) e->compact_plan_once = env_int("PSSBAM_COMPACT_PLAN_ONCE") != 0;
     if (tstat)
         fprintf(stderr, "[pssbam] engine on device %d: device properties %.3f, its stream + events %.3f, counters + scratch (first allocations, first "
                         "enqueue) %.3f s\n", dev, tc1 - tc0, tc2 - tc1, feed_now() - tc2);
@@ -1118,16 +1115,9 @@
                 rc = maskq ? launch_tiled_site<true, true>(e, P, lds, n_tiles) : launch_tiled_site<true, false>(e, P, lds, n_tiles);
             }
         } else if (do_pss && e->rows <= COMPACT_MAX_ROWS && e->use_compact && !e->has_rg && !maskq && !regions && !hist) {
-            if (!do_kmer && getenv("PSSBAM_COMPACT_DECODE_TWICE"))
-                rc = launch_flat(e, PREP_COMPACT_DECODE_TWICE, tally_compact_decode_twice, P, lds, n_tiles, false);
-            else if (e->compact_plan_once)
-                rc = !do_kmer  ? launch_flat(e, PREP_COMPACT_ONCE, tally_compact<false, false, true>, P, lds, n_tiles, false)
-                     : kmer_lds ? launch_flat(e, PREP_COMPACT_ONCE_KMER_LDS, tally_compact<true, true, true>, P, lds, n_tiles, true)
-                                : launch_flat(e, PREP_COMPACT_ONCE_KMER, tally_compact<true, false, true>, P, lds, n_tiles, false);
-            else
-                rc = !do_kmer  ? launch_flat(e, PREP_COMPACT, tally_compact<false, false, false>, P, lds, n_tiles, false)
-                     : kmer_lds ? launch_flat(e, PREP_COMPACT_KMER_LDS, tally_compact<true, true, false>, P, lds, n_tiles, true)
-                                : launch_flat(e, PREP_COMPACT_KMER, tally_compact<true, false, false>, P, lds, n_tiles, false);
+            rc = !do_kmer  ? launch_flat(e, PREP_COMPACT, tally_compact<false, false>, P, lds, n_tiles, false)
+                 : kmer_lds ? launch_flat(e, PREP_COMPACT_KMER_LDS, tally_compact<true, true>, P, lds, n_tiles, true)
+                            : launch_flat(e, PREP_COMPACT_KMER, tally_compact<true, false>, P, lds, n_tiles, false);
         } else if (hist) {
             P.hist_lds_bins = std::min(e->hist_max + 2u, HIST_LDS_MAX_BINS);
             if (e->env_hist_lds_bins >= 0) P.hist_lds_bins = std::min(P.hist_lds_bins, (uint32_t)e->env_hist_lds_bins);
diff --git a/pss-bam_amd/csrc/tally_kernels.h b/pss-bam_amd/csrc/tally_kernels.h
--- a/pss-bam_amd/csrc/tally_kernels.h
+++ b/pss-bam_amd/csrc/tally_kernels.h
@@ -4,8 +4,7 @@
 
 namespace pssbam {
 
-constexpr int TILED_THREADS = 256;
-constexpr int TILED_WAVES = TILED_THREADS / 64;
+constexpr int TILED_THREADS = 128;
 constexpr int TILED_ROWS = 32;
 constexpr int KMER_LDS_MAX_K = 4;
 constexpr uint32_t STAGE_SLACK = 64;
@@ -209,7 +208,7 @@
 struct __attribute__((packed, aligned(4))) Tri { uint32_t v[3]; };
 
 constexpr uint32_t TILED_MAX_T = 128;
-static_assert(TILED_MAX_T * 2 == TILED_THREADS, "CODES maps one (read, end) pair to each thread");
+static_assert(TILED_MAX_T == TILED_THREADS, "the decode round maps one read to each thread");
 
 __device__ __forceinline__ void stage_tile_dma(const uint8_t *recs, uint64_t recs_limit, const uint32_t *tile_offs,
                                                uint32_t count, uint32_t pieces, uint8_t *stage, uint32_t tid) {
@@ -249,6 +248,15 @@
     bool kfail = false;
     if (DO_KMER && (gpl.fk5 || gpl.fk3)) kfail = tally_kmer_record<LDS_KMER>(P, gpl, lds_kmer);
     return record_events(DO_PSS, DO_KMER, gpl, kfail);
+}
+
+__device__ __forceinline__ uint32_t lane_fetch(uint32_t v, uint32_t byte_addr) {
+    return (uint32_t)__builtin_amdgcn_ds_bpermute((int)byte_addr, (int)v);
+}
+__device__ __forceinline__ int64_t kmer_window_rel(bool rev, uint32_t Lk, int K, uint32_t which) {
+    const int64_t ok = K / 2, ik = K - K / 2;
+    if (!rev) return which ? (int64_t)Lk - ik : -ok;
+    return which ? -ok + (ik - ok) : (int64_t)Lk - ok;
 }
 
 enum PlaneSel { PLANES_NONE = 0, PLANES_RG, PLANES_LEN, PLANES_REF };
@@ -343,7 +351,7 @@
     const uint32_t ablate = P.ablate;
 
     const uint32_t tid = threadIdx.x;
-    const uint32_t lane = tid & 63u, wave = tid >> 6;
+    const uint32_t lane = tid & 63u, wave = __builtin_amdgcn_readfirstlane(tid >> 6);
     const int N = P.N;
     const uint32_t n_pos = (uint32_t)N + 2u;
     const uint32_t row_base = LATER_PASS ? P.row_base : 0u;
@@ -373,17 +381,22 @@
         n_tiles = min(all_tiles, (xcd + 1u) * per);
     }
     uint32_t tile = tile0;
-    uint32_t off_a = 0;
+    uint32_t off_a = 0, off_b = 0;
     const uint32_t TOFF = TILED_MAX_T + 4u;
     auto load_offsets = [&](uint32_t t) {
         const uint32_t r0 = t * T;
         if (tid <= T && r0 + tid <= n_recs) off_a = P.offs[r0 + tid];
+        if (tid + TILED_THREADS <= T && r0 + tid + TILED_THREADS <= n_recs) off_b = P.offs[r0 + tid + TILED_THREADS];
+    };
+    auto store_offsets = [&](uint32_t *dst) {
+        if (tid <= T) dst[tid] = off_a;
+        if (tid + TILED_THREADS <= T) dst[tid + TILED_THREADS] = off_b;
     };
     auto tile_count = [&](uint32_t t) { return min(T, n_recs - t * T); };
     __syncthreads();
     if (tile < n_tiles) {
         load_offsets(tile);
-        if (tid <= T) toffs[tid] = off_a;
+        store_offsets(toffs);
         __syncthreads();
         stage_tile_dma(P.recs, recs_limit, toffs, tile_count(tile), pieces, stage, tid);
         if (tile + tstride < n_tiles) load_offsets(tile + tstride);
@@ -397,137 +410,167 @@
         const uint32_t next = tile + tstride;
 
         asm volatile("s_waitcnt vmcnt(0)" ::: "memory");
-        if (next < n_tiles && tid <= T) toffs[(par ^ 1u) * TOFF + tid] = off_a;
+        if (next < n_tiles) store_offsets(toffs + (par ^ 1u) * TOFF);
         __syncthreads();
 
-        const uint32_t j = tid >> 1, e = tid & 1u;
-        const bool lane_on = tid < 2u * T && !(ablate & 4u);
-        const bool in_tile = lane_on && j < count;
+        const uint32_t jd = wave * 64u + lane;
+        const bool in_tile = jd < count && !(ablate & 4u);
         uint32_t o0 = 0, o1 = 0;
-        if (in_tile) { o0 = cur_offs[j]; o1 = cur_offs[j + 1]; }
+        if (in_tile) { o0 = cur_offs[jd]; o1 = cur_offs[jd + 1]; }
         const uint32_t avail = pieces * 16u - (o0 & 15u);
         const bool hdr_ok = in_tile && o1 - o0 >= 36u && avail >= 48u;
-        LdsBytes src{stage, hdr_ok ? j * pieces * 16u + (o0 & 15u) : 0u};
+        LdsBytes src{stage, hdr_ok ? jd * pieces * 16u + (o0 & 15u) : 0u};
         const RecHdr h = decode_hdr_lds(src, hdr_ok ? o1 - o0 : 0u);
         const uint32_t needed = (PLANES == PLANES_RG || P.rg) ? o1 - o0 : MASKQ ? h.aux_off : h.qual_off + 1u;
         const bool in_stage = hdr_ok && needed <= avail;
-        Plan pl = plan_head<DO_PSS, DO_KMER>(P, src, h, RefsLdsCached{refs_lds, P.ref_info, n_ref_cached, (uint32_t)P.n_ref});
-        if (!in_stage) { pl.status = RS_LIVE; pl.live = pl.pss_cand = pl.fk5 = pl.fk3 = false; }
-        const bool cand = DO_PSS && pl.pss_cand;
-        const bool rcand = REGIONS && (pl.pss_cand || pl.fk5 || pl.fk3);
-        uint4 rdesc = make_uint4(0u, 0u, 0u, 0u);
+        Plan pd = plan_head<DO_PSS, DO_KMER>(P, src, h, RefsLdsCached{refs_lds, P.ref_info, n_ref_cached, (uint32_t)P.n_ref});
+        if (!in_stage) { pd.status = RS_LIVE; pd.live = pd.pss_cand = pd.fk5 = pd.fk3 = false; }
         if constexpr (REGIONS) {
-            if (rcand) rdesc = P.region_info[region_ref_index(P, h)];
-        }
-        uint32_t gq[5] = {0u, 0u, 0u, 0u, 0u};
-        uint32_t gsh = 0u;
-        uint32_t nb_front = 4u, nb_behind = 4u;
-        if (cand) {
-            const uint64_t ga = pl.gbase + (uint64_t)pl.s + (e ? (uint64_t)pl.L - 30ull - row_base : (uint64_t)row_base - 2ull);
-            const uint32_t *pg = P.genome4 + (ga >> 3);
-            if (!(ablate & 128u)) {
-                const Quad q0 = *(const Quad *)pg;
-#pragma unroll
-                for (int k = 0; k < 4; k++) gq[k] = q0.v[k];
-                gq[4] = pg[4];
-                if constexpr (SITE) nb_front = P.genome4[(ga - 1ull) >> 3] >> (4u * (uint32_t)((ga - 1ull) & 7ull));
-            }
-            gsh = 4u * (uint32_t)(ga & 7ull);
-        }
-        uint32_t cx = 0u;
-        if (cand && !pass0) {
-            const uint64_t pc = pl.gbase + (uint64_t)pl.s + (e ? (uint64_t)pl.L : (uint64_t)-1ll);
-            cx = (P.genome4[pc >> 3] >> (4u * (uint32_t)(pc & 7ull))) & 15u;
-        }
-        const int32_t n0 = e ? (int32_t)pl.L - 30 - (int32_t)row_base : (int32_t)row_base - 2;
-        uint32_t rr[6];
-#pragma unroll
-        for (int k = 0; k < 6; k++) rr[k] = 0u;
-        uint32_t ssh = 0u;
-        if (cand) {
-            const int32_t n0a = min(n0, (int32_t)h.l_seq);
-            const uint32_t sa = src.off + (uint32_t)((int32_t)h.seq_off + (n0a >> 1));
-            const uint32_t *qs = (const uint32_t *)(stage + (sa & ~3u));
-            ssh = sa & 3u;
-#pragma unroll
-            for (int k = 0; k < 6; k++) rr[k] = qs[k];
-        }
-        uint32_t qq[MASKQ ? 9 : 1];
-        uint32_t qsh = 0u;
-        if constexpr (MASKQ) {
-#pragma unroll
-            for (int k = 0; k < 9; k++) qq[k] = 0u;
-            if (cand) {
-                const int32_t n0q = min(n0, (int32_t)h.l_seq);
-                const uint32_t qa = src.off + (uint32_t)((int32_t)h.qual_off + n0q);
-                const uint32_t *qp = (const uint32_t *)(stage + (qa & ~3u));
-                qsh = qa & 3u;
-#pragma unroll
-                for (int k = 0; k < 9; k++) qq[k] = qp[k];
-            }
-        }
-        const uint32_t kwhich = e ^ (pl.rev ? 1u : 0u);
-        bool kmer_try = DO_KMER && (kwhich ? pl.fk3 : pl.fk5) && !(ablate & 16u);
-        uint32_t kw[3] = {0u, 0u, 0u};
-        uint32_t ksh = 0u;
-        if (kmer_try) {
-            int64_t w5, w3;
-            kmer_windows(pl, P.K, w5, w3);
-            const uint64_t ka = pl.gbase + (uint64_t)(kwhich ? w3 : w5);
-            const Tri kq = *(const Tri *)(P.genome4 + (ka >> 3));
-#pragma unroll
-            for (int k = 0; k < 3; k++) kw[k] = kq.v[k];
-            ksh = 4u * (uint32_t)(ka & 7ull);
-        }
-        RegionQuery rq{};
-        if constexpr (REGIONS) {
-            if (rcand) region_grid_load(P, h, rdesc, rq);
-        }
-        uint32_t kplane = 0u;
+            if (pd.pss_cand || pd.fk5 || pd.fk3) {
+                RegionQuery rq;
+                region_grid_load(P, h, P.region_info[region_ref_index(P, h)], rq);
+                if (!region_resolve(P, rq)) pd.pss_cand = pd.fk5 = pd.fk3 = false;
+            }
+        }
+        uint32_t kplane_d = 0u;
         if constexpr (KPLANES) {
-            if (e == 0u && (pl.fk5 || pl.fk3)) kplane = record_plane<PLANES, true>(src, h, pl, *gk);
-            const uint32_t left = (uint32_t)__shfl_xor((int)kplane, 1);
-            if (e) kplane = left;
+            if (pd.fk5 || pd.fk3) kplane_d = record_plane<PLANES, true>(src, h, pd, *gk);
         }
         if constexpr (GROUPED && !KPLANES) {
-            if (in_tile && e == 0u) {
-                const uint32_t slot = cand ? record_plane<PLANES>(src, h, pl, *gk) - gk->plane0 : gk->n_slots;
-                grp_lds[j] = slot < gk->n_slots ? slot : gk->n_slots;
-            }
-        }
-        uint32_t ev_over = 0u;
-        if (in_tile && !in_stage && e == 0u) {
+            if (in_tile) {
+                const uint32_t slot = pd.pss_cand ? record_plane<PLANES>(src, h, pd, *gk) - gk->plane0 : gk->n_slots;
+                grp_lds[jd] = slot < gk->n_slots ? slot : gk->n_slots;
+            }
+        }
+        if (in_tile && !in_stage) {
+            uint32_t ev_over;
             if constexpr (KPLANES) ev_over = tally_overflow_record_kmer_planes<PLANES, LDS_KMER, REGIONS>(kernarg, gk, o0, o1, lds_kmer);
             else if constexpr (GROUPED) ev_over = tally_overflow_record_planes<PLANES, MASKQ, REGIONS>(kernarg, gk, o0, o1, table);
             else ev_over = tally_overflow_record<DO_PSS, DO_KMER, LDS_KMER, MASKQ, REGIONS, HIST, SITE>(kernarg, o0, o1, table, lds_kmer, hist_lds, site_lds);
-            if (pass0) atomicAdd(&lds_delta[ST_SLOW_PATH], 1);
-        }
-        uint32_t W[4];
-#pragma unroll
-        for (int m = 0; m < 4; m++) W[m] = __builtin_amdgcn_alignbit(gq[m + 1], gq[m], gsh);
-#pragma unroll
-        for (int k = 0; k < 2; k++) kw[k] = __builtin_amdgcn_alignbit(kw[k + 1], kw[k], ksh);
-#pragma unroll
-        for (int m = 0; m < 4; m++) asm volatile("" : "+v"(W[m]));
-        asm volatile("" : "+v"(cx));
-        if constexpr (SITE) {
-            nb_front &= 15u;
-            nb_behind = (gq[4] >> gsh) & 15u;
-            asm volatile("" : "+v"(nb_front));
-            asm volatile("" : "+v"(nb_behind));
-        }
-        if (DO_KMER) {
-#pragma unroll
-            for (int k = 0; k < 2; k++) asm volatile("" : "+v"(kw[k]));
-        }
-        if constexpr (MASKQ) {
-#pragma unroll
-            for (int k = 0; k < 9; k++) asm volatile("" : "+v"(qq[k]));
-        }
-        if constexpr (REGIONS) {
-            if (rcand && !region_resolve(P, rq)) {
-                pl.pss_cand = pl.fk5 = pl.fk3 = false;
-                kmer_try = false;
+            if (pass0) {
+                book_events(DO_PSS, DO_KMER, ev_over, lds_delta);
+                atomicAdd(&lds_delta[ST_SLOW_PATH], 1);
+            }
+        }
+        const uint64_t gs_d = pd.gbase + (uint64_t)pd.s;
+        const uint32_t meta_d = ((pd.pss_cand ? src.off + h.seq_off : 0u) & 0x3FFFFu) | ((pd.flag & 0xD1u) << 18) | (pd.status << 26) |
+                                (pd.pss_cand ? 1u << 28 : 0u) | (pd.fk5 ? 1u << 29 : 0u) | (pd.fk3 ? 1u << 30 : 0u) | (in_stage ? 1u << 31 : 0u);
+
+        const uint32_t e = lane & 1u;
+        struct Round {
+            uint32_t W[4], cx, nb_front, nb_behind;
+            uint32_t rr[6], ssh;
+            uint32_t qq[MASKQ ? 9 : 1], qsh;
+            uint32_t kw[2], kwhich, kplane;
+            uint32_t L, l_seq, meta;
+            int32_t n0;
+            bool on, cand, kmer_try;
+        } R[2];
+#pragma unroll
+        for (int hh = 0; hh < 2; hh++) {
+            Round &r = R[hh];
+            r.on = wave * 64u + (uint32_t)hh * 32u < count && !(ablate & 4u);
+            r.cand = r.kmer_try = false;
+            if (!r.on) continue;
+            const uint32_t sl = ((uint32_t)hh * 32u + (lane >> 1)) << 2;
+            const uint64_t gs = (uint64_t)lane_fetch((uint32_t)gs_d, sl) | ((uint64_t)lane_fetch((uint32_t)(gs_d >> 32), sl) << 32);
+            r.L = lane_fetch(pd.L, sl);
+            r.l_seq = lane_fetch(h.l_seq, sl);
+            r.meta = lane_fetch(meta_d, sl);
+            const bool rev = (r.meta & (FL_REVERSE << 18)) != 0;
+            const bool cand = DO_PSS && ((r.meta >> 28) & 1u);
+            r.cand = cand;
+            uint32_t gq[5] = {0u, 0u, 0u, 0u, 0u};
+            uint32_t gsh = 0u;
+            r.nb_front = r.nb_behind = 4u;
+            if (cand) {
+                const uint64_t ga = gs + (e ? (uint64_t)r.L - 30ull - row_base : (uint64_t)row_base - 2ull);
+                const uint32_t *pg = P.genome4 + (ga >> 3);
+                if (!(ablate & 128u)) {
+                    const Quad q0 = *(const Quad *)pg;
+#pragma unroll
+                    for (int k = 0; k < 4; k++) gq[k] = q0.v[k];
+                    gq[4] = pg[4];
+                    if constexpr (SITE) r.nb_front = P.genome4[(ga - 1ull) >> 3] >> (4u * (uint32_t)((ga - 1ull) & 7ull));
+                }
+                gsh = 4u * (uint32_t)(ga & 7ull);
+            }
+            r.cx = 0u;
+            if (cand && !pass0) {
+                const uint64_t pc = gs + (e ? (uint64_t)r.L : (uint64_t)-1ll);
+                r.cx = (P.genome4[pc >> 3] >> (4u * (uint32_t)(pc & 7ull))) & 15u;
+            }
+            r.n0 = e ? (int32_t)r.L - 30 - (int32_t)row_base : (int32_t)row_base - 2;
+#pragma unroll
+            for (int k = 0; k < 6; k++) r.rr[k] = 0u;
+            r.ssh = 0u;
+            const uint32_t soff = r.meta & 0x3FFFFu;
+            if (cand) {
+                const int32_t n0a = min(r.n0, (int32_t)r.l_seq);
+                const uint32_t sa = soff + (uint32_t)(n0a >> 1);
+                const uint32_t *qs = (const uint32_t *)(stage + (sa & ~3u));
+                r.ssh = sa & 3u;
+#pragma unroll
+                for (int k = 0; k < 6; k++) r.rr[k] = qs[k];
+            }
+            r.qsh = 0u;
+            if constexpr (MASKQ) {
+#pragma unroll
+                for (int k = 0; k < 9; k++) r.qq[k] = 0u;
+                if (cand) {
+                    const int32_t n0q = min(r.n0, (int32_t)r.l_seq);
+                    const uint32_t qa = soff + ((r.l_seq + 1u) >> 1) + (uint32_t)n0q;
+                    const uint32_t *qp = (const uint32_t *)(stage + (qa & ~3u));
+                    r.qsh = qa & 3u;
+#pragma unroll
+                    for (int k = 0; k < 9; k++) r.qq[k] = qp[k];
+                }
+            }
+            r.kwhich = e ^ (rev ? 1u : 0u);
+            r.kmer_try = DO_KMER && ((r.meta >> (r.kwhich ? 30 : 29)) & 1u) && !(ablate & 16u);
+            r.kplane = 0u;
+            uint32_t kw[3] = {0u, 0u, 0u};
+            uint32_t ksh = 0u;
+            if constexpr (DO_KMER) {
+                const uint32_t Lk = lane_fetch(pd.Lk, sl);
+                if constexpr (KPLANES) r.kplane = lane_fetch(kplane_d, sl);
+                if (r.kmer_try) {
+                    const uint64_t ka = gs + (uint64_t)kmer_window_rel(rev, Lk, P.K, r.kwhich);
+                    const Tri kq = *(const Tri *)(P.genome4 + (ka >> 3));
+#pragma unroll
+                    for (int k = 0; k < 3; k++) kw[k] = kq.v[k];
+                    ksh = 4u * (uint32_t)(ka & 7ull);
+                }
+            }
+#pragma unroll
+            for (int m = 0; m < 4; m++) r.W[m] = __builtin_amdgcn_alignbit(gq[m + 1], gq[m], gsh);
+#pragma unroll
+            for (int k = 0; k < 2; k++) r.kw[k] = __builtin_amdgcn_alignbit(kw[k + 1], kw[k], ksh);
+            if constexpr (SITE) {
+                r.nb_front &= 15u;
+                r.nb_behind = (gq[4] >> gsh) & 15u;
+            }
+        }
+#pragma unroll
+        for (int hh = 0; hh < 2; hh++) {
+            Round &r = R[hh];
+            if (!r.on) continue;
+#pragma unroll
+            for (int m = 0; m < 4; m++) asm volatile("" : "+v"(r.W[m]));
+            asm volatile("" : "+v"(r.cx));
+            if constexpr (SITE) {
+                asm volatile("" : "+v"(r.nb_front));
+                asm volatile("" : "+v"(r.nb_behind));
+            }
+            if (DO_KMER) {
+#pragma unroll
+                for (int k = 0; k < 2; k++) asm volatile("" : "+v"(r.kw[k]));
+            }
+#pragma unroll
+            for (int k = 0; k < 6; k++) asm volatile("" : "+v"(r.rr[k]));
+            if constexpr (MASKQ) {
+#pragma unroll
+                for (int k = 0; k < 9; k++) asm volatile("" : "+v"(r.qq[k]));
             }
         }
         __syncthreads();
@@ -537,8 +580,28 @@
             if (next + tstride < n_tiles) load_offsets(next + tstride);
         }
 
-        {
-            const uint32_t own1 = !pass0 ? cx : e ? (W[3] >> 24) & 15u : (W[0] >> 4) & 15u;
+#pragma unroll
+        for (int hh = 0; hh < 2; hh++) {
+            Round &r = R[hh];
+            if (!r.on) continue;
+            const uint32_t j = wave * 64u + (uint32_t)hh * 32u + (lane >> 1);
+            const bool cand = r.cand, kmer_try = r.kmer_try;
+            const uint32_t kwhich = r.kwhich;
+            const int32_t n0 = r.n0;
+            const uint32_t *W = r.W, *rr = r.rr, *kw = r.kw;
+            const uint32_t ssh = r.ssh, nb_front = r.nb_front, nb_behind = r.nb_behind;
+            const bool staged = (r.meta >> 31) != 0;
+            Plan pl;
+            pl.flag = (r.meta >> 18) & 0xD1u;
+            pl.rev = (pl.flag & FL_REVERSE) != 0;
+            pl.status = (r.meta >> 26) & 3u;
+            pl.live = staged && pl.status == RS_LIVE;
+            pl.pss_cand = ((r.meta >> 28) & 1u) != 0;
+            pl.fk5 = ((r.meta >> 29) & 1u) != 0;
+            pl.fk3 = ((r.meta >> 30) & 1u) != 0;
+            pl.pss_fwd = pl.pss_rev = false;
+            pl.L = r.L;
+            const uint32_t own1 = !pass0 ? r.cx : e ? (W[3] >> 24) & 15u : (W[0] >> 4) & 15u;
             const uint32_t other1 = (uint32_t)__shfl_xor((int)own1, 1);
             if (DO_PSS) plan_finish_pss_packed(P.acgt_ctx, pl, e ? other1 : own1, e ? own1 : other1);
             uint32_t code_w[8];
@@ -569,14 +632,14 @@
                     const uint32_t q4 = P.min_bq * 0x01010101u;
                     uint32_t Qb[8];
 #pragma unroll
-                    for (int k = 0; k < 8; k++) Qb[k] = __builtin_amdgcn_alignbyte(qq[k + 1], qq[k], qsh);
+                    for (int k = 0; k < 8; k++) Qb[k] = __builtin_amdgcn_alignbyte(r.qq[k + 1], r.qq[k], r.qsh);
 #pragma unroll
                     for (int m = 0; m < 4; m++) {
                         RE[m] |= base_quality_mask(__builtin_amdgcn_perm(Qb[2 * m + 1], Qb[2 * m], 0x06040200u), q4);
                         RO[m] |= base_quality_mask(__builtin_amdgcn_perm(Qb[2 * m + 1], Qb[2 * m], 0x07050301u), q4);
                     }
                 }
-                const int32_t have_s = (int32_t)h.l_seq - n0;
+                const int32_t have_s = (int32_t)r.l_seq - n0;
                 const uint32_t have = have_s <= 0 ? 0u : have_s >= 32 ? 32u : (uint32_t)have_s;
                 if (__any(have < (e && pass0 ? 30u : 32u))) {
 #pragma unroll
@@ -636,12 +699,12 @@
                 }
                 kmer_ok = bad == 0u;
                 if (kmer_ok && !(ablate & 8u)) {
-                    if constexpr (KPLANES) kmer_plane_add<LDS_KMER>(P, *gk, kplane, kwhich, bin, lds_kmer);
+                    if constexpr (KPLANES) kmer_plane_add<LDS_KMER>(P, *gk, r.kplane, kwhich, bin, lds_kmer);
                     else if (LDS_KMER) atomicAdd(&lds_kmer[(kwhich ? (1u << (2 * P.K)) : 0u) + bin], 1u);
                     else atomicAdd(&P.counters[(kwhich ? P.off_k3 : P.off_k5) + bin], 1ull);
                 }
             }
-            if (lane_on && !KPLANES) {
+            if constexpr (!KPLANES) {
                 uint4 *dst = (uint4 *)(sheet + j * 64u + e * 32u);
                 dst[0] = make_uint4(code_w[0], code_w[1], code_w[2], code_w[3]);
                 dst[1] = make_uint4(code_w[4], code_w[5], code_w[6], code_w[7]);
@@ -652,7 +715,7 @@
                 const int bad_other = __shfl_xor(bad, 1);
                 kfail = (bad | bad_other) != 0;
             }
-            if (e == 0u && pass0) book_events(DO_PSS, DO_KMER, in_stage ? record_events(DO_PSS, DO_KMER, pl, kfail) : ev_over, lds_delta);
+            if (e == 0u && pass0 && staged) book_events(DO_PSS, DO_KMER, record_events(DO_PSS, DO_KMER, pl, kfail), lds_delta);
             if constexpr (HIST) hist_wave_add(P, hist_lds, e == 0u, pl.L, pl.pss_fwd, pl.pss_rev);
         }
 
@@ -660,7 +723,7 @@
             const uint32_t e = lane >> 5, b = lane & 31u;
             const uint32_t wpos = (b & 24u) + 2u * (b & 3u) + ((b >> 2) & 1u);
             const uint32_t row = e ? 31u - wpos : wpos;
-            const uint32_t j0 = min(count, wave * 32u), j1 = min(count, j0 + 32u);
+            const uint32_t j0 = min(count, wave * 64u), j1 = min(count, j0 + 64u);
             if (GROUPED && row < n_live) {
                 const uint32_t trash_off = (gk->n_slots - 1u) * GROUP_PLANE_WORDS;
                 uint32_t j = j0;
@@ -782,7 +845,7 @@
     return record_events(true, DO_KMER, gpl, kfail);
 }
 
-template <bool DO_KMER, bool LDS_KMER, int DECODE_REPS = 1, bool PLAN_ONCE = false>
+template <bool DO_KMER, bool LDS_KMER>
 __device__ __forceinline__ void tally_compact_body(const TallyParams &P, const TallyParams *kernarg,
                                                    uint8_t *__restrict__ stage, uint8_t *__restrict__ sheet,
                                                    uint32_t *__restrict__ table, uint32_t *__restrict__ toffs,
@@ -794,7 +857,7 @@
     const uint32_t pieces = P.prefix_pieces;
     const uint32_t recs_limit32 = (uint32_t)(((P.recs_bytes + 15ull) & ~15ull) - 16ull);
     const uint32_t tid = threadIdx.x;
-    const uint32_t lane = tid & 63u, wave = tid >> 6;
+    const uint32_t lane = tid & 63u, wave = __builtin_amdgcn_readfirstlane(tid >> 6);
 
     uint32_t up_tab = 0u, dn_tab = 0u;
 #pragma unroll
@@ -807,7 +870,7 @@
     }
 
     for (uint32_t i = tid; i < COMPACT_TABLE_WORDS; i += TILED_THREADS) table[i] = 0u;
-    if (tid < CTX_WORDS) ctx_rep[tid] = 0u;
+    for (uint32_t i = tid; i < CTX_WORDS; i += TILED_THREADS) ctx_rep[i] = 0u;
     if (LDS_KMER)
         for (uint32_t i = tid; i < 2u * (1u << (2 * P.K)); i += TILED_THREADS) lds_kmer[i] = 0u;
     if (tid < ST_USED) lds_delta[tid] = 0;
@@ -818,17 +881,22 @@
     const uint32_t all_tiles = (n_recs + T - 1u) / T;
     uint32_t tile = blockIdx.x;
     const uint32_t tstride = gridDim.x, n_tiles = all_tiles;
-    uint32_t off_a = 0;
+    uint32_t off_a = 0, off_b = 0;
     const uint32_t TOFF = TILED_MAX_T + 4u;
     auto load_offsets = [&](uint32_t t) {
         const uint32_t r0 = t * T;
         if (tid <= T && r0 + tid <= n_recs) off_a = P.offs[r0 + tid];
+        if (tid + TILED_THREADS <= T && r0 + tid + TILED_THREADS <= n_recs) off_b = P.offs[r0 + tid + TILED_THREADS];
+    };
+    auto store_offsets = [&](uint32_t *dst) {
+        if (tid <= T) dst[tid] = off_a;
+        if (tid + TILED_THREADS <= T) dst[tid + TILED_THREADS] = off_b;
     };
     auto tile_count = [&](uint32_t t) { return min(T, n_recs - t * T); };
     __syncthreads();
     if (tile < n_tiles) {
         load_offsets(tile);
-        if (tid <= T) toffs[tid] = off_a;
+        store_offsets(toffs);
         __syncthreads();
         stage_tile_dma32(P.recs, recs_limit32, toffs, tile_count(tile), pieces, stage, tid);
         if (tile + tstride < n_tiles) load_offsets(tile + tstride);
@@ -842,120 +910,101 @@
         const uint32_t next = tile + tstride;
 
         asm volatile("s_waitcnt vmcnt(0)" ::: "memory");
-        if (next < n_tiles && tid <= T) toffs[(par ^ 1u) * TOFF + tid] = off_a;
+        if (next < n_tiles) store_offsets(toffs + (par ^ 1u) * TOFF);
         __syncthreads();
 
-        const uint32_t j = tid >> 1, e = tid & 1u;
-        const bool lane_on = tid < 2u * T;
-        Plan pl;
-        uint32_t l_seq = 0, soff = 0;
-        bool in_stage = false;
-        if constexpr (PLAN_ONCE) {
-            uint4 *plan_lds = (uint4 *)sheet;
-            if (tid < T) {
-                const bool in_t = tid < count;
-                uint32_t o0 = 0, o1 = 0;
-                if (in_t) { o0 = cur_offs[tid]; o1 = cur_offs[tid + 1]; }
-                const uint32_t avail = pieces * 16u - (o0 & 15u);
-                const bool hdr_ok = in_t && o1 - o0 >= 36u && avail >= 48u;
-                LdsBytes src{stage, hdr_ok ? tid * pieces * 16u + (o0 & 15u) : 0u};
-                const RecHdr h = decode_hdr_lds32(src, hdr_ok ? o1 - o0 : 0u);
-                const bool staged = hdr_ok && h.qual_off + 1u <= avail;
-                Plan p1 = plan_head<true, DO_KMER, false>(P, src, h, RefsLdsCached{refs_lds, P.ref_info, n_ref_cached, (uint32_t)P.n_ref});
-                if (!staged) { p1.status = RS_LIVE; p1.live = p1.pss_cand = p1.fk5 = p1.fk3 = false; }
-                if (in_t && !staged) ovf_list[atomicAdd(ovf_n, 1u)] = tid;
-                const uint32_t bits = (p1.flag & 0xFFFFu) | (p1.status << 16) | (p1.live ? 1u << 18 : 0u) | (p1.pss_cand ? 1u << 19 : 0u) |
-                                      (p1.fk5 ? 1u << 20 : 0u) | (p1.fk3 ? 1u << 21 : 0u) | (staged ? 1u << 22 : 0u);
-                plan_lds[2u * tid] = make_uint4((uint32_t)p1.gbase, (uint32_t)(p1.gbase >> 32), (uint32_t)p1.s, p1.L);
-                plan_lds[2u * tid + 1u] = make_uint4(h.l_seq, src.off + h.seq_off, bits, p1.Lk);
-            }
-            __syncthreads();
-            const uint4 qa = plan_lds[2u * j], qb = plan_lds[2u * j + 1u];
-            pl.gbase = (uint64_t)qa.x | ((uint64_t)qa.y << 32);
-            pl.s = (int32_t)qa.z;
-            pl.L = qa.w;
-            l_seq = qb.x;
-            soff = qb.y;
-            pl.flag = qb.z & 0xFFFFu;
-            pl.status = (qb.z >> 16) & 3u;
-            pl.live = lane_on && ((qb.z >> 18) & 1u);
-            pl.pss_cand = lane_on && ((qb.z >> 19) & 1u);
-            pl.fk5 = lane_on && ((qb.z >> 20) & 1u);
-            pl.fk3 = lane_on && ((qb.z >> 21) & 1u);
-            in_stage = lane_on && ((qb.z >> 22) & 1u);
-            pl.Lk = qb.w;
-            pl.rev = (pl.flag & FL_REVERSE) != 0;
-            pl.pss_fwd = pl.pss_rev = false;
-        } else {
-        const bool in_tile = lane_on && j < count;
+        const uint32_t jd = wave * 64u + lane;
+        const bool in_tile = jd < count;
         uint32_t o0 = 0, o1 = 0;
-        if (in_tile) { o0 = cur_offs[j]; o1 = cur_offs[j + 1]; }
+        if (in_tile) { o0 = cur_offs[jd]; o1 = cur_offs[jd + 1]; }
         const uint32_t avail = pieces * 16u - (o0 & 15u);
         const bool hdr_ok = in_tile && o1 - o0 >= 36u && avail >= 48u;
-        LdsBytes src{stage, hdr_ok ? j * pieces * 16u + (o0 & 15u) : 0u};
+        LdsBytes src{stage, hdr_ok ? jd * pieces * 16u + (o0 & 15u) : 0u};
         const RecHdr h = decode_hdr_lds32(src, hdr_ok ? o1 - o0 : 0u);
         const uint32_t needed = h.qual_off + 1u;
-        in_stage = hdr_ok && needed <= avail;
-        pl = plan_head<true, DO_KMER, false>(P, src, h, RefsLdsCached{refs_lds, P.ref_info, n_ref_cached, (uint32_t)P.n_ref});
-        if constexpr (DECODE_REPS > 1) {
-            uint32_t off2 = src.off;
-            asm volatile("" : "+v"(off2));
-            const LdsBytes src2{stage, off2};
-            const RecHdr h2 = decode_hdr_lds32(src2, hdr_ok ? o1 - o0 : 0u);
-            const Plan p2 = plan_head<true, DO_KMER, false>(P, src2, h2, RefsLdsCached{refs_lds, P.ref_info, n_ref_cached, (uint32_t)P.n_ref});
-            const uint32_t sink = (uint32_t)p2.s ^ p2.L ^ p2.flag ^ (uint32_t)p2.gbase ^ (uint32_t)(p2.gbase >> 32) ^ p2.status ^ (p2.pss_cand ? 1u : 0u) ^
-                                  (p2.rev ? 2u : 0u) ^ (p2.fk5 ? 4u : 0u) ^ (p2.fk3 ? 8u : 0u) ^ h2.seq_off ^ h2.qual_off;
-            asm volatile("" ::"v"(sink));
-        }
-        if (!in_stage) { pl.status = RS_LIVE; pl.live = pl.pss_cand = pl.fk5 = pl.fk3 = false; }
-        l_seq = h.l_seq;
-        soff = src.off + h.seq_off;
-        if (in_tile && !in_stage && e == 0u) ovf_list[atomicAdd(ovf_n, 1u)] = j;
-        }
-        const bool cand = pl.pss_cand;
-        uint32_t gq[4] = {0u, 0u, 0u, 0u};
-        uint32_t gsh = 0u;
-        if (cand) {
-            const uint64_t ga = pl.gbase + (uint64_t)(int64_t)((int32_t)pl.s + (e ? (int32_t)pl.L - 16 : -2));
-            const Quad q0 = *(const Quad *)(P.genome4 + (ga >> 3));
-#pragma unroll
-            for (int k = 0; k < 4; k++) gq[k] = q0.v[k];
-            gsh = 4u * (uint32_t)(ga & 7ull);
-        }
-        const int32_t n0 = e ? (int32_t)pl.L - 16 : 0;
-        uint32_t rr[3] = {0u, 0u, 0u};
-        uint32_t ssh = 0u;
-        if (cand) {
-            const int32_t n0a = min(n0, (int32_t)l_seq);
-            const uint32_t sa = soff + (uint32_t)(n0a >> 1);
-            const uint32_t *qs = (const uint32_t *)(stage + (sa & ~3u));
-            ssh = sa & 3u;
-#pragma unroll
-            for (int k = 0; k < 3; k++) rr[k] = qs[k];
-        }
-        const uint32_t kwhich = e ^ (pl.rev ? 1u : 0u);
-        const bool kmer_try = DO_KMER && (kwhich ? pl.fk3 : pl.fk5);
-        uint32_t kw[3] = {0u, 0u, 0u};
-        uint32_t ksh = 0u;
-        if (kmer_try) {
-            int64_t w5, w3;
-            kmer_windows(pl, P.K, w5, w3);
-            const uint64_t ka = pl.gbase + (uint64_t)(kwhich ? w3 : w5);
-            const Tri kq = *(const Tri *)(P.genome4 + (ka >> 3));
-#pragma unroll
-            for (int k = 0; k < 3; k++) kw[k] = kq.v[k];
-            ksh = 4u * (uint32_t)(ka & 7ull);
-        }
-        uint32_t A[3];
-#pragma unroll
-        for (int m = 0; m < 3; m++) A[m] = __builtin_amdgcn_alignbit(gq[m + 1], gq[m], gsh);
-#pragma unroll
-        for (int k = 0; k < 2; k++) kw[k] = __builtin_amdgcn_alignbit(kw[k + 1], kw[k], ksh);
-#pragma unroll
-        for (int m = 0; m < 3; m++) asm volatile("" : "+v"(A[m]));
-        if (DO_KMER) {
-#pragma unroll
-            for (int k = 0; k < 2; k++) asm volatile("" : "+v"(kw[k]));
+        const bool in_stage = hdr_ok && needed <= avail;
+        Plan pd = plan_head<true, DO_KMER, false>(P, src, h, RefsLdsCached{refs_lds, P.ref_info, n_ref_cached, (uint32_t)P.n_ref});
+        if (!in_stage) { pd.status = RS_LIVE; pd.live = pd.pss_cand = pd.fk5 = pd.fk3 = false; }
+        if (in_tile && !in_stage) ovf_list[atomicAdd(ovf_n, 1u)] = jd;
+        const uint64_t gs_d = pd.gbase + (uint64_t)(int64_t)pd.s;
+        const uint32_t meta_d = ((pd.pss_cand ? src.off + h.seq_off : 0u) & 0x3FFFFu) | ((pd.flag & 0xD1u) << 18) | (pd.status << 26) |
+                                (pd.pss_cand ? 1u << 28 : 0u) | (pd.fk5 ? 1u << 29 : 0u) | (pd.fk3 ? 1u << 30 : 0u) | (in_stage ? 1u << 31 : 0u);
+
+        const uint32_t e = lane & 1u;
+        struct Round {
+            uint32_t A[3];
+            uint32_t rr[3], ssh;
+            uint32_t kw[2], kwhich;
+            uint32_t L, l_seq, meta;
+            int32_t n0;
+            bool on, cand, kmer_try;
+        } R[2];
+#pragma unroll
+        for (int hh = 0; hh < 2; hh++) {
+            Round &r = R[hh];
+            r.on = wave * 64u + (uint32_t)hh * 32u < count;
+            r.cand = r.kmer_try = false;
+            if (!r.on) continue;
+            const uint32_t sl = ((uint32_t)hh * 32u + (lane >> 1)) << 2;
+            const uint64_t gs = (uint64_t)lane_fetch((uint32_t)gs_d, sl) | ((uint64_t)lane_fetch((uint32_t)(gs_d >> 32), sl) << 32);
+            r.L = lane_fetch(pd.L, sl);
+            r.l_seq = lane_fetch(h.l_seq, sl);
+            r.meta = lane_fetch(meta_d, sl);
+            const bool rev = (r.meta & (FL_REVERSE << 18)) != 0;
+            const bool cand = ((r.meta >> 28) & 1u) != 0;
+            r.cand = cand;
+            uint32_t gq[4] = {0u, 0u, 0u, 0u};
+            uint32_t gsh = 0u;
+            if (cand) {
+                const uint64_t ga = gs + (uint64_t)(int64_t)(e ? (int32_t)r.L - 16 : -2);
+                const Quad q0 = *(const Quad *)(P.genome4 + (ga >> 3));
+#pragma unroll
+                for (int k = 0; k < 4; k++) gq[k] = q0.v[k];
+                gsh = 4u * (uint32_t)(ga & 7ull);
+            }
+            r.n0 = e ? (int32_t)r.L - 16 : 0;
+#pragma unroll
+            for (int k = 0; k < 3; k++) r.rr[k] = 0u;
+            r.ssh = 0u;
+            if (cand) {
+                const int32_t n0a = min(r.n0, (int32_t)r.l_seq);
+                const uint32_t sa = (r.meta & 0x3FFFFu) + (uint32_t)(n0a >> 1);
+                const uint32_t *qs = (const uint32_t *)(stage + (sa & ~3u));
+                r.ssh = sa & 3u;
+#pragma unroll
+                for (int k = 0; k < 3; k++) r.rr[k] = qs[k];
+            }
+            r.kwhich = e ^ (rev ? 1u : 0u);
+            r.kmer_try = DO_KMER && ((r.meta >> (r.kwhich ? 30 : 29)) & 1u);
+            uint32_t kw[3] = {0u, 0u, 0u};
+            uint32_t ksh = 0u;
+            if constexpr (DO_KMER) {
+                const uint32_t Lk = lane_fetch(pd.Lk, sl);
+                if (r.kmer_try) {
+                    const uint64_t ka = gs + (uint64_t)kmer_window_rel(rev, Lk, P.K, r.kwhich);
+                    const Tri kq = *(const Tri *)(P.genome4 + (ka >> 3));
+#pragma unroll
+                    for (int k = 0; k < 3; k++) kw[k] = kq.v[k];
+                    ksh = 4u * (uint32_t)(ka & 7ull);
+                }
+            }
+#pragma unroll
+            for (int m = 0; m < 3; m++) r.A[m] = __builtin_amdgcn_alignbit(gq[m + 1], gq[m], gsh);
+#pragma unroll
+            for (int k = 0; k < 2; k++) r.kw[k] = __builtin_amdgcn_alignbit(kw[k + 1], kw[k], ksh);
+        }
+#pragma unroll
+        for (int hh = 0; hh < 2; hh++) {
+            Round &r = R[hh];
+            if (!r.on) continue;
+#pragma unroll
+            for (int m = 0; m < 3; m++) asm volatile("" : "+v"(r.A[m]));
+            if (DO_KMER) {
+#pragma unroll
+                for (int k = 0; k < 2; k++) asm volatile("" : "+v"(r.kw[k]));
+            }
+#pragma unroll
+            for (int k = 0; k < 3; k++) asm volatile("" : "+v"(r.rr[k]));
         }
         __syncthreads();
 
@@ -964,7 +1013,25 @@
             if (next + tstride < n_tiles) load_offsets(next + tstride);
         }
 
-        {
+#pragma unroll
+        for (int hh = 0; hh < 2; hh++) {
+            Round &r = R[hh];
+            if (!r.on) continue;
+            const uint32_t j = wave * 64u + (uint32_t)hh * 32u + (lane >> 1);
+            const uint32_t *A = r.A, *rr = r.rr, *kw = r.kw;
+            const uint32_t ssh = r.ssh, kwhich = r.kwhich, l_seq = r.l_seq;
+            const int32_t n0 = r.n0;
+            const bool cand = r.cand, kmer_try = r.kmer_try;
+            const bool staged = (r.meta >> 31) != 0;
+            Plan pl;
+            pl.flag = (r.meta >> 18) & 0xD1u;
+            pl.rev = (pl.flag & FL_REVERSE) != 0;
+            pl.status = (r.meta >> 26) & 3u;
+            pl.live = staged && pl.status == RS_LIVE;
+            pl.pss_cand = cand;
+            pl.fk5 = ((r.meta >> 29) & 1u) != 0;
+            pl.fk3 = ((r.meta >> 30) & 1u) != 0;
+            pl.pss_fwd = pl.pss_rev = false;
             const uint32_t cx = e ? A[2] : A[0];
             const uint32_t c_lo = cx & 15u, c_hi = (cx >> 4) & 15u;
             const uint32_t own1 = e ? c_lo : c_hi, own2 = e ? c_hi : c_lo;
@@ -1046,15 +1113,14 @@
                     else atomicAdd(&P.counters[(kwhich ? P.off_k3 : P.off_k5) + bin], 1ull);
                 }
             }
-            if (lane_on)
-                *(uint4 *)(sheet + j * 32u + e * 16u) = make_uint4(code_w[0], code_w[1], code_w[2], code_w[3]);
+            *(uint4 *)(sheet + j * 32u + e * 16u) = make_uint4(code_w[0], code_w[1], code_w[2], code_w[3]);
             bool kfail = false;
             if (DO_KMER) {
                 const int bad = (kmer_try && !kmer_ok) ? 1 : 0;
                 const int bad_other = __shfl_xor(bad, 1);
                 kfail = (bad | bad_other) != 0;
             }
-            if (e == 0u && in_stage) book_events(true, DO_KMER, record_events(true, DO_KMER, pl, kfail), lds_delta);
+            if (e == 0u && staged) book_events(true, DO_KMER, record_events(true, DO_KMER, pl, kfail), lds_delta);
         }
 
         {
@@ -1062,7 +1128,7 @@
             const uint32_t w = (b & 8u) + 2u * (b & 3u) + ((b >> 2) & 1u);
             const uint32_t posn = ee ? 15u - w : w;
             const uint32_t slot = ee * 16u + posn;
-            const uint32_t j0 = min(count, wave * 32u), j1 = min(count, j0 + 32u);
+            const uint32_t j0 = min(count, wave * 64u), j1 = min(count, j0 + 64u);
             if (posn < (uint32_t)P.N) {
                 const uint32_t rd = lane >> 5;
                 uint32_t jj = j0;
@@ -1111,7 +1177,7 @@
     if (tid < 16u) mine[SCRATCH_DELTA + tid] = tid < (uint32_t)ST_USED ? (uint32_t)lds_delta[tid] : 0u;
 }
 
-template <bool DO_KMER, bool LDS_KMER, bool PLAN_ONCE = false>
+template <bool DO_KMER, bool LDS_KMER>
 __global__ void __launch_bounds__(TILED_THREADS) tally_compact(const TallyParams P) {
     extern __shared__ __attribute__((aligned(16))) uint8_t stage[];
     __shared__ __attribute__((aligned(16))) uint8_t sheet[TILED_MAX_T * 32u];
@@ -1123,23 +1189,8 @@
     __shared__ uint32_t ctx_rep[CTX_WORDS];
     __shared__ uint32_t ovf_list[TILED_MAX_T + 1];
     const TallyParams *kernarg = (const TallyParams *)__builtin_amdgcn_kernarg_segment_ptr();
-    tally_compact_body<DO_KMER, LDS_KMER, 1, PLAN_ONCE>(P, kernarg, stage, sheet, table, toffs, lds_kmer, lds_delta, refs_lds, ctx_rep, ovf_list,
-                                                        ovf_list + TILED_MAX_T);
-}
-
-__global__ void __launch_bounds__(TILED_THREADS) tally_compact_decode_twice(const TallyParams P) {
-    extern __shared__ __attribute__((aligned(16))) uint8_t stage[];
-    __shared__ __attribute__((aligned(16))) uint8_t sheet[TILED_MAX_T * 32u];
-    __shared__ uint32_t table[COMPACT_TABLE_WORDS];
-    __shared__ uint32_t toffs[2u * (TILED_MAX_T + 4u)];
-    __shared__ uint32_t lds_kmer[1u];
-    __shared__ int32_t lds_delta[ST_USED];
-    __shared__ uint4 refs_lds[REF_LDS_ENTRIES + 1];
-    __shared__ uint32_t ctx_rep[CTX_WORDS];
-    __shared__ uint32_t ovf_list[TILED_MAX_T + 1];
-    const TallyParams *kernarg = (const TallyParams *)__builtin_amdgcn_kernarg_segment_ptr();
-    tally_compact_body<false, false, 2>(P, kernarg, stage, sheet, table, toffs, lds_kmer, lds_delta, refs_lds, ctx_rep, ovf_list,
-                                        ovf_list + TILED_MAX_T);
+    tally_compact_body<DO_KMER, LDS_KMER>(P, kernarg, stage, sheet, table, toffs, lds_kmer, lds_delta, refs_lds, ctx_rep, ovf_list,
+                                          ovf_list + TILED_MAX_T);
 }
 
 constexpr uint32_t REDUCE_GROUPS = 32;
```

New measurement: 19.97 billion. -15.8%, worse.
